# mariohsouto/ProxSDP.jl

Measured on AMD Instinct MI355X. Metric: PDHG iterations/sec at target rank ~ sqrt(n), Max-Cut SDP n=4000 (tol 1e-4 options), higher is better.
Workload: dtype f64

## Files before the change

### include/proxsdp_hip.h

```cpp
#ifndef PROXSDP_HIP_H
#define PROXSDP_HIP_H

#include <stdint.h>

#ifdef __cplusplus
extern "C" {
#endif

#define PROXSDP_HIP_ABI_VERSION 10

#define PROXSDP_E_INVALID  (-1)
#define PROXSDP_E_HIP      (-2)
#define PROXSDP_E_NOMEM    (-3)
#define PROXSDP_E_UNSUPP   (-4)
#define PROXSDP_E_INTERNAL (-5)
#define PROXSDP_E_COMM_ABORTED (-6)

#define PROXSDP_STATUS_NOT_CALLED       0
#define PROXSDP_STATUS_OPTIMAL          1
#define PROXSDP_STATUS_TIME_LIMIT       2
#define PROXSDP_STATUS_ITERATION_LIMIT  3
#define PROXSDP_STATUS_INFEAS_OR_UNBND  4
#define PROXSDP_STATUS_DUAL_INFEASIBLE  5
#define PROXSDP_STATUS_INFEASIBLE       6

typedef struct proxsdp_csc {
    int64_t nrows;
    int64_t ncols;
    const int64_t* colptr;
    const int64_t* rowval;
    const double*  nzval;
} proxsdp_csc;

typedef struct proxsdp_problem {
    int64_t n;
    int64_t p;
    int64_t m;
    proxsdp_csc A;
    proxsdp_csc G;
    const double* b;
    const double* h;
    const double* c;
    int64_t n_psd;
    const int64_t* psd_ptr;
    const int64_t* psd_idx;
    int64_t n_soc;
    const int64_t* soc_ptr;
    const int64_t* soc_idx;
    int32_t index_base;
    int32_t reserved0;
    const double* eig_resid;
    void* reduce_ctx;
    int (*reduce_fn)(void* ctx, double* sums, int32_t nsum, double* maxs, int32_t nmax);
    const double* M_dense;
    int32_t M_dense_on_device;
    int32_t reserved1;
    int64_t n_coupling;
    const int64_t* coupling_rows;
    const int32_t* coupling_owned;
    int (*reduce_vec_fn)(void* ctx, double* buf, int64_t len, int32_t on_device);
    int32_t reduce_vec_on_device;
    int32_t reserved2;
    void* nccl_comm;
    int64_t reserved3;
} proxsdp_problem;

typedef struct proxsdp_options {
    int64_t struct_size;
    int32_t log_verbose;  int32_t log_freq;
    int32_t timer_verbose; int32_t timer_file; int32_t disable_julia_logger;
    int32_t warn_on_limit; int32_t extended_log; int32_t extended_log2; int32_t log_repeat_header;
    int32_t pad0;
    double  time_limit;
    double tol_gap, tol_feasibility, tol_feasibility_dual, tol_primal, tol_dual, tol_psd, tol_soc;
    int32_t check_dual_feas; int32_t check_dual_feas_freq;
    double  max_obj; int32_t min_iter_max_obj; int32_t pad1;
    int32_t min_iter_time_infeas; int32_t pad2;
    double infeas_gap_tol, infeas_limit_gap_tol, infeas_stable_gap_tol,
           infeas_feasibility_tol, infeas_stable_feasibility_tol;
    int32_t certificate_search; int32_t pad3;
    double certificate_obj_tol, certificate_fail_tol;
    double min_beta, max_beta, initial_beta;
    double initial_adapt_level, adapt_decay; int32_t adapt_window; int32_t pad4;
    int32_t convergence_window; int32_t convergence_check;
    int64_t max_iter; int64_t min_iter; int64_t divergence_min_update;
    int64_t max_iter_lp; int64_t max_iter_conic; int64_t max_iter_local;
    int32_t advanced_initialization; int32_t line_search_flag;
    int32_t max_linsearch_steps; int32_t pad5;
    double delta, initial_theta, linsearch_decay;
    int32_t full_eig_decomp; int32_t max_target_rank_krylov_eigs;
    int32_t min_size_krylov_eigs; int32_t warm_start_eig;
    int32_t rank_increment; int32_t rank_increment_factor;
    int32_t eigsolver; int32_t eigsolver_min_lanczos; int64_t eigsolver_resid_seed;
    double  arpack_tol; int32_t arpack_resid_init; int32_t arpack_reset_resid; int64_t arpack_max_iter;
    int32_t krylovkit_reset_resid; int32_t krylovkit_resid_init;
    double  krylovkit_tol; int32_t krylovkit_max_iter; int32_t krylovkit_eager; int32_t krylovkit_verbose;
    int32_t reduce_rank; int32_t rank_slack; int32_t pad6;
    int64_t full_eig_freq; int64_t full_eig_len;
    int32_t equilibration; int32_t equilibration_iters;
    double  equilibration_lb, equilibration_ub, equilibration_limit;
    int32_t equilibration_force; int32_t approx_norm;
    int32_t device_id;
    int32_t trace_capacity;
    int32_t profile_symv_every;
    int32_t support_path;
    int32_t lanczos_operator;
    int32_t initial_target_rank;
    int32_t full_eig_lanczos;
    int32_t lanczos_cycle_kernel;
    int32_t lanczos_warm_start;
    int32_t reconstruct_mfma;
    int32_t small_block_batch;
    int32_t full_eig_sign;
    int32_t psd_sign_engine;
    int32_t full_eig_lanczos_verify;
    double  full_eig_lanczos_posres;
    int32_t full_eig_lanczos_kdim10;
    int32_t sign_small_tile_max;
    int32_t host_eig_threads;
    int32_t block_threads;
    int32_t host_eig_merge;
    int32_t block_batch;
    int32_t rocsolver_warmup;
    int32_t debug_fail_iteration;
    int32_t host_wait_spin;
    int32_t sign_start_row;
    int32_t general_batch;
    int32_t full_eig_lanczos_certify;
    int32_t host_merge_threads;
    int32_t reserved_i[1];
    double  full_eig_lanczos_tol;
    double  reserved_d[1];
    int32_t equilibration_reference_aliasing;
    int32_t reserved_i3[2];
    int32_t block_batch_groups;
    int32_t lanczos_wide_krylov;
    int32_t reserved_i2[7];
    double  full_eig_lanczos_warm_pow;
    double  reserved_d2[3];
} proxsdp_options;

#define PROXSDP_TRACE_COLS 14

typedef struct proxsdp_stats {
    int64_t lanczos_matvecs;
    int64_t lanczos_restarts;
    int64_t lanczos_calls;
    int64_t full_eigs;
    int64_t krylov_fallbacks;
    int64_t linesearch_trials;
    int64_t symv_launches;
    int64_t symv_profiled;
    double  symv_profiled_ms;
    double  symv_bytes;
    double  algorithmic_bytes;
    double  init_time;
    double  loop_time;
    double  exit_time;
    double  t_primal, t_psd, t_linesearch, t_residual;
    int64_t dense_passes;
    double  dense_ms;
    int64_t fop_projections;
    int64_t exit_matvecs;
    double  host_eig_time;
    int64_t host_eigs;
    int64_t device_eigs;
    int64_t batched_small_eigs;
    int64_t mfma_reconstructions;
    int64_t orth_profiled;
    double  orth_profiled_ms;
    double  full_eig_solver_ms;
    double  full_eig_recon_ms;
    int64_t cycle_launches;
    int64_t full_eigs_lanczos;
    int64_t cycle_steps;
    double  cycle_ms;
    int64_t warm_starts;
    int64_t full_eigs_sign;
    int64_t sign_products;
    int64_t sign_engine_projections;
    int64_t sign_engine_rejected;
    int64_t sign_engine_checks;
    int64_t sign_engine_mismatches;
    int64_t full_eigs_lanczos_checks;
    int64_t full_eigs_lanczos_mismatches;
    int64_t batched_block_steps;
    int64_t rccl_reductions;
    int64_t batched_profiled_blocks;
    int64_t host_eig_merges;
    double  host_eig_overlap_time;
    int64_t sign_short_pass;
    int64_t sign_short_fail;
    int64_t full_eigs_lanczos_certified;
    int64_t full_eigs_lanczos_cert_failed;
    int64_t cert_matvecs;
    int64_t dense_truncated_projections;
    int64_t wide_krylov_projections;
    int64_t reserved_s[4];
    int64_t dense_setup_passes;
    int64_t dense_sigma_steps;
} proxsdp_stats;
#define PROXSDP_STATS_SHARDED_GENERAL_ITERATIONS 0

typedef struct proxsdp_result {
    int32_t status;
    int32_t certificate_found;
    int32_t primal_feasible_user_tol;
    int32_t dual_feasible_user_tol;
    int32_t result_count;
    int32_t final_rank;
    int64_t iter;
    double  primal_residual;
    double  dual_residual;
    double  objval, dual_objval, gap, time;
    double  dual_feasibility;
    double* primal;
    double* dual_cone;
    double* dual_eq;
    double* dual_in;
    double* slack_eq;
    double* slack_in;
    double* trace;
    int64_t trace_rows;
    char    status_string[256];
    proxsdp_stats stats;
} proxsdp_result;

#define PROXSDP_STATE_NHIST 7
typedef struct proxsdp_state {
    int64_t struct_size;
    int64_t iteration;
    int64_t n, Q, n_psd;
    int64_t hist_len;
    double* x;
    double* y;
    double* Mty;
    double* Mx;
    int64_t* target_rank;
    int64_t* current_rank;
    double* min_eig;
    double* hist;
    double scal[16];
    int64_t ints[8];
} proxsdp_state;

int  proxsdp_hip_abi_version(void);
void proxsdp_hip_default_options(proxsdp_options* opt);
int  proxsdp_hip_set_option(proxsdp_options* opt, const char* name, double value);
int  proxsdp_hip_get_option(const proxsdp_options* opt, const char* name, double* value);
int  proxsdp_hip_solve(const proxsdp_problem* prob, const proxsdp_options* opt,
                       proxsdp_result* res);
int  proxsdp_hip_solve_ex(const proxsdp_problem* prob, const proxsdp_options* opt, proxsdp_result* res,
                          const proxsdp_state* resume, proxsdp_state* capture);
const char* proxsdp_hip_last_error(void);
int  proxsdp_hip_device_count(void);

int  proxsdp_hip_solve_sharded(const proxsdp_problem* prob, const proxsdp_options* opt,
                               int32_t n_shards, const int32_t* device_ids,
                               const int32_t* psd_owner, const int32_t* soc_owner, const int32_t* free_owner,
                               proxsdp_result* res, proxsdp_stats* shard_stats);

#define PROXSDP_FACTOR_NONE 0
#define PROXSDP_FACTOR_RITZ 1
#define PROXSDP_FACTOR_EIG  2
typedef struct proxsdp_psd_factors {
    int64_t struct_size;
    int64_t n_psd;
    const int64_t* cap;
    const int64_t* vec_ptr;
    const int64_t* val_ptr;
    double*  vectors;
    double*  values;
    int64_t* rank;
    int64_t* rank_found;
    int32_t* source;
    double*  resid;
    double*  xnorm;
} proxsdp_psd_factors;
int  proxsdp_hip_solve_factored(const proxsdp_problem* prob, const proxsdp_options* opt, proxsdp_result* res,
                                proxsdp_psd_factors* fac);

typedef struct proxsdp_start {
    int64_t struct_size;
// ... 150 lines not shown
```

### proxsdp.jl_amd/binding.py

```python
import ctypes as C
import os
import pathlib
import re

import numpy as np
import scipy.sparse as sp

_HERE = pathlib.Path(__file__).resolve().parent
LIB_PATH = _HERE / "libproxsdp_hip.so"
HEADER_PATH = _HERE.parent / "include" / "proxsdp_hip.h"

TRACE_COLS = 14
TRACE_NAMES = ("iter", "prim_obj", "dual_obj", "gap", "feas", "prim_res", "dual_res",
               "primal_step", "beta", "theta", "target_rank", "trials", "elapsed", "matvecs")


class LibraryNotBuilt(RuntimeError):
    pass


class ProxSDPHipError(RuntimeError):
    def __init__(self, code, msg):
        super().__init__(f"libproxsdp_hip error {code}: {msg}")
        self.code = code


i32, i64, f64 = C.c_int32, C.c_int64, C.c_double
pi64 = C.POINTER(C.c_int64)
pf64 = C.POINTER(C.c_double)


class CSC(C.Structure):
    _fields_ = [("nrows", i64), ("ncols", i64), ("colptr", pi64), ("rowval", pi64), ("nzval", pf64)]


class Problem(C.Structure):
    _fields_ = [("n", i64), ("p", i64), ("m", i64), ("A", CSC), ("G", CSC),
                ("b", pf64), ("h", pf64), ("c", pf64),
                ("n_psd", i64), ("psd_ptr", pi64), ("psd_idx", pi64),
                ("n_soc", i64), ("soc_ptr", pi64), ("soc_idx", pi64),
                ("index_base", i32), ("reserved0", i32), ("eig_resid", pf64),
                ("reduce_ctx", C.c_void_p), ("reduce_fn", C.c_void_p),
                ("M_dense", C.c_void_p), ("M_dense_on_device", i32), ("reserved1", i32),
                ("n_coupling", i64), ("coupling_rows", pi64), ("coupling_owned", C.POINTER(i32)),
                ("reduce_vec_fn", C.c_void_p), ("reduce_vec_on_device", i32), ("reserved2", i32),
                ("nccl_comm", C.c_void_p), ("reserved3", i64)]


REDUCE_FN = C.CFUNCTYPE(C.c_int, C.c_void_p, pf64, i32, pf64, i32)
REDUCE_VEC_FN = C.CFUNCTYPE(C.c_int, C.c_void_p, C.c_void_p, i64, i32)


def _opt_fields():
    F = []
    a = lambda name, t: F.append((name, t))
    a("struct_size", i64)
    for nme in ("log_verbose", "log_freq", "timer_verbose", "timer_file", "disable_julia_logger",
                "warn_on_limit", "extended_log", "extended_log2", "log_repeat_header", "pad0"):
        a(nme, i32)
    a("time_limit", f64)
    for nme in ("tol_gap", "tol_feasibility", "tol_feasibility_dual", "tol_primal", "tol_dual",
                "tol_psd", "tol_soc"):
        a(nme, f64)
    a("check_dual_feas", i32); a("check_dual_feas_freq", i32)
    a("max_obj", f64); a("min_iter_max_obj", i32); a("pad1", i32)
    a("min_iter_time_infeas", i32); a("pad2", i32)
    for nme in ("infeas_gap_tol", "infeas_limit_gap_tol", "infeas_stable_gap_tol",
                "infeas_feasibility_tol", "infeas_stable_feasibility_tol"):
        a(nme, f64)
    a("certificate_search", i32); a("pad3", i32)
    a("certificate_obj_tol", f64); a("certificate_fail_tol", f64)
    a("min_beta", f64); a("max_beta", f64); a("initial_beta", f64)
    a("initial_adapt_level", f64); a("adapt_decay", f64); a("adapt_window", i32); a("pad4", i32)
    a("convergence_window", i32); a("convergence_check", i32)
    for nme in ("max_iter", "min_iter", "divergence_min_update", "max_iter_lp", "max_iter_conic",
                "max_iter_local"):
        a(nme, i64)
    a("advanced_initialization", i32); a("line_search_flag", i32)
    a("max_linsearch_steps", i32); a("pad5", i32)
    a("delta", f64); a("initial_theta", f64); a("linsearch_decay", f64)
    a("full_eig_decomp", i32); a("max_target_rank_krylov_eigs", i32)
    a("min_size_krylov_eigs", i32); a("warm_start_eig", i32)
    a("rank_increment", i32); a("rank_increment_factor", i32)
    a("eigsolver", i32); a("eigsolver_min_lanczos", i32); a("eigsolver_resid_seed", i64)
    a("arpack_tol", f64); a("arpack_resid_init", i32); a("arpack_reset_resid", i32); a("arpack_max_iter", i64)
    a("krylovkit_reset_resid", i32); a("krylovkit_resid_init", i32)
    a("krylovkit_tol", f64); a("krylovkit_max_iter", i32); a("krylovkit_eager", i32); a("krylovkit_verbose", i32)
    a("reduce_rank", i32); a("rank_slack", i32); a("pad6", i32)
    a("full_eig_freq", i64); a("full_eig_len", i64)
    a("equilibration", i32); a("equilibration_iters", i32)
    a("equilibration_lb", f64); a("equilibration_ub", f64); a("equilibration_limit", f64)
    a("equilibration_force", i32); a("approx_norm", i32)
    a("device_id", i32); a("trace_capacity", i32); a("profile_symv_every", i32); a("support_path", i32)
    a("lanczos_operator", i32); a("initial_target_rank", i32)
    a("full_eig_lanczos", i32); a("lanczos_cycle_kernel", i32); a("lanczos_warm_start", i32)
    a("reconstruct_mfma", i32); a("small_block_batch", i32); a("full_eig_sign", i32); a("psd_sign_engine", i32)
    a("full_eig_lanczos_verify", i32); a("full_eig_lanczos_posres", f64); a("full_eig_lanczos_kdim10", i32)
    a("sign_small_tile_max", i32); a("host_eig_threads", i32); a("block_threads", i32)
    a("host_eig_merge", i32); a("block_batch", i32); a("rocsolver_warmup", i32); a("debug_fail_iteration", i32); a("host_wait_spin", i32)
    a("sign_start_row", i32); a("general_batch", i32); a("full_eig_lanczos_certify", i32); a("host_merge_threads", i32); a("reserved_i", i32 * 1)
    a("full_eig_lanczos_tol", f64); a("reserved_d", f64 * 1)
    a("equilibration_reference_aliasing", i32); a("reserved_i3", i32 * 2)
    a("block_batch_groups", i32); a("lanczos_wide_krylov", i32); a("reserved_i2", i32 * 7); a("full_eig_lanczos_warm_pow", f64); a("reserved_d2", f64 * 3)
    return F


class Options(C.Structure):
    _fields_ = _opt_fields()


class Stats(C.Structure):
    _fields_ = [("lanczos_matvecs", i64), ("lanczos_restarts", i64), ("lanczos_calls", i64),
                ("full_eigs", i64), ("krylov_fallbacks", i64), ("linesearch_trials", i64),
                ("symv_launches", i64), ("symv_profiled", i64), ("symv_profiled_ms", f64),
                ("symv_bytes", f64), ("algorithmic_bytes", f64), ("init_time", f64),
                ("loop_time", f64), ("exit_time", f64), ("t_primal", f64), ("t_psd", f64),
                ("t_linesearch", f64), ("t_residual", f64), ("dense_passes", i64), ("dense_ms", f64), ("fop_projections", i64), ("exit_matvecs", i64),
                ("host_eig_time", f64), ("host_eigs", i64), ("device_eigs", i64), ("batched_small_eigs", i64),
                ("mfma_reconstructions", i64), ("orth_profiled", i64), ("orth_profiled_ms", f64),
                ("full_eig_solver_ms", f64), ("full_eig_recon_ms", f64), ("cycle_launches", i64),
                ("full_eigs_lanczos", i64), ("cycle_steps", i64), ("cycle_ms", f64), ("warm_starts", i64),
                ("full_eigs_sign", i64), ("sign_products", i64),
                ("sign_engine_projections", i64), ("sign_engine_rejected", i64),
                ("sign_engine_checks", i64), ("sign_engine_mismatches", i64),
                ("full_eigs_lanczos_checks", i64), ("full_eigs_lanczos_mismatches", i64),
                ("batched_block_steps", i64), ("rccl_reductions", i64),
                ("batched_profiled_blocks", i64), ("host_eig_merges", i64),
                ("host_eig_overlap_time", f64), ("sign_short_pass", i64), ("sign_short_fail", i64),
                ("full_eigs_lanczos_certified", i64), ("full_eigs_lanczos_cert_failed", i64), ("cert_matvecs", i64),
                ("dense_truncated_projections", i64), ("wide_krylov_projections", i64), ("reserved_s", i64 * 4),
                ("dense_setup_passes", i64), ("dense_sigma_steps", i64)]


class Result(C.Structure):
    _fields_ = [("status", i32), ("certificate_found", i32), ("primal_feasible_user_tol", i32),
                ("dual_feasible_user_tol", i32), ("result_count", i32), ("final_rank", i32),
                ("iter", i64), ("primal_residual", f64), ("dual_residual", f64),
                ("objval", f64), ("dual_objval", f64), ("gap", f64), ("time", f64),
                ("dual_feasibility", f64),
                ("primal", pf64), ("dual_cone", pf64), ("dual_eq", pf64), ("dual_in", pf64),
                ("slack_eq", pf64), ("slack_in", pf64), ("trace", pf64), ("trace_rows", i64),
                ("status_string", C.c_char * 256), ("stats", Stats)]


STATS_RESERVED_SLOTS = {"sharded_general_iterations": 0}

STATE_NHIST = 7
STATE_HIST_NAMES = ("dual_gap", "prim_obj", "dual_obj", "feasibility", "primal_residual", "dual_residual", "comb_residual")
STATE_SCAL_NAMES = ("primal_step", "primal_step_old", "dual_step", "beta", "theta", "adapt_level",
                    "equa_feasibility", "ineq_feasibility", "dual_feasibility")


class State(C.Structure):
    _fields_ = [("struct_size", i64), ("iteration", i64), ("n", i64), ("Q", i64), ("n_psd", i64), ("hist_len", i64),
                ("x", pf64), ("y", pf64), ("Mty", pf64), ("Mx", pf64),
                ("target_rank", pi64), ("current_rank", pi64), ("min_eig", pf64), ("hist", pf64),
                ("scal", f64 * 16), ("ints", i64 * 8)]


class ShardIO(C.Structure):
    _fields_ = ([("struct_size", i64)] +
                [(k, i64) for k in ("n", "p", "m", "nnz_A", "nnz_G", "n_coupling", "n_psd", "len_psd", "n_soc", "len_soc", "len_eig")] +
                [("vars", pi64), ("rows_eq", pi64), ("rows_in", pi64), ("coupling_rows", pi64), ("coupling_owned", C.POINTER(i32)),
                 ("A_colptr", pi64), ("A_rowval", pi64), ("A_nzval", pf64), ("G_colptr", pi64), ("G_rowval", pi64), ("G_nzval", pf64),
                 ("b", pf64), ("h", pf64), ("c", pf64),
                 ("psd_ids", pi64), ("psd_ptr", pi64), ("psd_idx", pi64), ("soc_ids", pi64), ("soc_ptr", pi64), ("soc_idx", pi64), ("eig_resid", pf64)])


class PsdFactors(C.Structure):
    _fields_ = [("struct_size", i64), ("n_psd", i64), ("cap", pi64), ("vec_ptr", pi64), ("val_ptr", pi64),
                ("vectors", pf64), ("values", pf64), ("rank", pi64), ("rank_found", pi64), ("source", C.POINTER(i32)),
                ("resid", pf64), ("xnorm", pf64)]


class Start(C.Structure):
    _fields_ = [("struct_size", i64), ("primal", pf64), ("dual_eq", pf64), ("dual_in", pf64), ("n_psd", i64),
                ("rank", pi64), ("vec_ptr", pi64), ("val_ptr", pi64), ("vectors", pf64), ("values", pf64),
                ("target_rank", pi64), ("primal_step", f64), ("beta", f64)]


FACTOR_NONE, FACTOR_RITZ, FACTOR_EIG = 0, 1, 2
FACTOR_SOURCE_NAMES = {FACTOR_NONE: "NONE", FACTOR_RITZ: "RITZ", FACTOR_EIG: "EIG"}


_lib = None


def header_symbols():
    txt = HEADER_PATH.read_text()
    txt = re.sub(r"/\*.*?\*/", "", txt, flags=re.S)
    return sorted(set(re.findall(r"\b(proxsdp_(?:hip|host)_\w+)\s*\(", txt)))


def lib():
    global _lib
    if _lib is not None:
        return _lib
    if not LIB_PATH.exists():
        raise LibraryNotBuilt(
            f"{LIB_PATH} is missing: run `python -c 'import __graft_entry__ as g; g.build()'` "
            "(or `make -C proxsdp.jl_amd/csrc`).  There is no CPU fallback.")
    import sys
    if "torch" in sys.modules:
        try:
            tc = sys.modules["torch"].cuda
            if tc.is_available():
                tc.init()
        except Exception:
            pass
    L = C.CDLL(str(LIB_PATH))
    L.proxsdp_hip_abi_version.restype = C.c_int
    L.proxsdp_hip_last_error.restype = C.c_char_p
    L.proxsdp_hip_default_options.argtypes = [C.POINTER(Options)]
    L.proxsdp_hip_default_options.restype = None
    L.proxsdp_hip_set_option.argtypes = [C.POINTER(Options), C.c_char_p, f64]
    L.proxsdp_hip_get_option.argtypes = [C.POINTER(Options), C.c_char_p, pf64]
    L.proxsdp_hip_solve.argtypes = [C.POINTER(Problem), C.POINTER(Options), C.POINTER(Result)]
    L.proxsdp_hip_solve_ex.argtypes = [C.POINTER(Problem), C.POINTER(Options), C.POINTER(Result),
                                       C.POINTER(State), C.POINTER(State)]
    L.proxsdp_hip_solve_factored.argtypes = [C.POINTER(Problem), C.POINTER(Options), C.POINTER(Result),
                                             C.POINTER(PsdFactors)]
    L.proxsdp_hip_solve_from.argtypes = [C.POINTER(Problem), C.POINTER(Options), C.POINTER(Result),
                                         C.POINTER(Start), C.POINTER(PsdFactors)]
    L.proxsdp_hip_start_point.argtypes = [C.POINTER(Problem), C.POINTER(Options), C.POINTER(Start), C.POINTER(State)]
    L.proxsdp_hip_factor_residual.argtypes = [pf64, i64, pf64, i64, pf64, i32, pf64, pf64]
    L.proxsdp_hip_factor_residual_kernel.argtypes = [pf64, i64, pf64, i64, pf64, i32, pf64, pf64, i32, pf64]
    L.proxsdp_hip_psd_project.argtypes = [pf64, i64, i32, i32, C.POINTER(Options), pf64, pf64,
                                          C.POINTER(i32), pf64, pi64, C.POINTER(i32), C.POINTER(i32)]
    L.proxsdp_hip_eigsolve.argtypes = [pf64, i64, i32, C.POINTER(Options), pf64, i32, pf64, pf64,
                                       C.POINTER(i32), C.POINTER(i32), pi64, C.POINTER(i32)]
    L.proxsdp_hip_symv_packed.argtypes = [pf64, i64, pf64, pf64, i32, pf64]
    L.proxsdp_hip_reconstruct.argtypes = [pf64, pf64, i64, i32, pf64, i32, pf64]
    L.proxsdp_hip_reconstruct_kernel.argtypes = [pf64, pf64, i64, i32, i32, pf64, i32, pf64]
    L.proxsdp_hip_full_eig_kernel.argtypes = [pf64, i64, i32, pf64, i32, pf64, C.POINTER(i32), C.POINTER(i64)]
    L.proxsdp_hip_spmv.argtypes = [C.POINTER(CSC), i32, i32, pf64, pf64]
    L.proxsdp_host_symeig.argtypes = [i32, pf64, pf64]
    L.proxsdp_host_start_vector.argtypes = [i64, i64, i32, pf64]
    L.proxsdp_host_preprocess.argtypes = [C.POINTER(Problem), pi64, pi64, pf64, pf64]
    L.proxsdp_hip_dense_scaling.argtypes = [C.POINTER(Problem), C.POINTER(Options), pf64, pf64, pf64, pf64, C.POINTER(i32)]
    L.proxsdp_host_equilibrate_rowsums.argtypes = [pf64, i64, i64, C.POINTER(Options), pf64, pf64]
    L.proxsdp_hip_sym_product.argtypes = [C.POINTER(SymProductIO)]
    L.proxsdp_hip_sign_unpack.argtypes = [pf64, i64, f64, pf64, pf64]
    L.proxsdp_hip_solve_sharded.argtypes = [C.POINTER(Problem), C.POINTER(Options), i32, C.POINTER(i32), C.POINTER(i32),
                                            C.POINTER(i32), C.POINTER(i32), C.POINTER(Result), C.POINTER(Stats)]
    L.proxsdp_host_split_shard.argtypes = [C.POINTER(Problem), i32, C.POINTER(i32), C.POINTER(i32), C.POINTER(i32), i32,
                                           C.POINTER(ShardIO)]
    L.proxsdp_host_group_reduce.argtypes = [i32, i32, i32, i32, pf64, i32, i32, f64, pf64, C.POINTER(i32), C.POINTER(i32)]
    L.proxsdp_hip_coupling_sum.argtypes = [pf64, i32, i64, pi64, pf64, i64, pf64]
    L.proxsdp_hip_rccl_unique_id.argtypes = [C.c_void_p]
    L.proxsdp_hip_rccl_comm_init.argtypes = [i32, C.c_void_p, i32, i32, C.POINTER(C.c_void_p)]
    L.proxsdp_hip_rccl_comm_destroy.argtypes = [C.c_void_p]
    if L.proxsdp_hip_abi_version() != 10:
        raise ProxSDPHipError(-1, "ABI version mismatch")
# ... 854 lines not shown
```

### proxsdp.jl_amd/csrc/host_util.hpp

```cpp
#pragma once
#include <atomic>
#include <chrono>
#include <cmath>
#include <condition_variable>
#include <cstdint>
#include <cstdlib>
#include <cstring>
#include <cstddef>
#include <functional>
#include <mutex>
#include <thread>
#include <vector>
#include <algorithm>
#if defined(__x86_64__)
#include <immintrin.h>
#endif
#include "../../include/proxsdp_hip.h"
#include "host_eig_merge.hpp"

namespace proxsdp {

inline uint64_t splitmix64(uint64_t z) {
    z += 0x9E3779B97F4A7C15ull;
    z = (z ^ (z >> 30)) * 0xBF58476D1CE4E5B9ull;
// ... 376 lines not shown
        std::function<void(int)> f = fn;
        job_.store(&f, std::memory_order_relaxed);
        njobs_.store(n, std::memory_order_relaxed);
        done_.store(0, std::memory_order_relaxed);
        gen_ = (gen_ + 1) & 0xffffffffull;
        if (gen_ == 0) gen_ = 1;
        const uint64_t g = gen_;
        ticket_.store(g << 32, std::memory_order_release);
        work(g);
        while (done_.load(std::memory_order_acquire) < n) {
#if defined(__x86_64__)
            _mm_pause();
#endif
        }
    }
private:
    void work(uint64_t g) {
        for (;;) {
            uint64_t t = ticket_.load(std::memory_order_acquire);
            if ((t >> 32) != g) return;
            const int i = (int)(t & 0xffffffffu);
            if (i >= njobs_.load(std::memory_order_relaxed)) return;
            if (!ticket_.compare_exchange_weak(t, t + 1, std::memory_order_acq_rel, std::memory_order_acquire)) continue;
            (*job_.load(std::memory_order_relaxed))(i);
            done_.fetch_add(1, std::memory_order_acq_rel);
        }
    }
    void loop() {
        uint64_t seen = 0;
        for (;;) {
            {
                std::unique_lock<std::mutex> lk(mu_);
                cv_.wait(lk, [&]() { return stop_.load() || armed_.load(std::memory_order_acquire); });
                if (stop_.load()) return;
            }
            while (armed_.load(std::memory_order_acquire) && !stop_.load(std::memory_order_relaxed)) {
                const uint64_t g = ticket_.load(std::memory_order_acquire) >> 32;
                if (g != seen) { seen = g; work(g); }
                else {
#if defined(__x86_64__)
                    _mm_pause();
#endif
                }
            }
        }
    }
    std::vector<std::thread> th_;
    std::mutex mu_;
    std::condition_variable cv_;
    std::atomic<bool> armed_{false}, stop_{false};
    uint64_t gen_ = 0;
    std::atomic<uint64_t> ticket_{0};
    std::atomic<int> done_{0}, njobs_{0};
    std::atomic<const std::function<void(int)>*> job_{nullptr};
};

struct SplitEig {
    Rank1Merge M;
    std::vector<double> Q1, d1, Q2, d2, e2;
    int k1 = 0, K = 0;
    double beta = 0.0;
    bool have_first = false;
    int first(int k1_, int m, const double* D, const double* f, const double* al, const double* be) {
        k1 = k1_; have_first = false;
        if (k1 < 1 || (m > 0 && k1 != m + 1)) return 1;
        beta = be[k1 - 1];
        if (!(beta == beta) || beta == 0.0) return 1;
        Q1.assign((size_t)k1 * k1, 0.0); d1.assign(k1, 0.0);
        int rc;
        if (m == 0) {
            for (int j = 0; j < k1; ++j) {
                Q1[(size_t)j * k1 + j] = al[j];
                if (j + 1 < k1) { Q1[(size_t)j * k1 + j + 1] = be[j]; Q1[(size_t)(j + 1) * k1 + j] = be[j]; }
            }
            Q1[(size_t)(k1 - 1) * k1 + (k1 - 1)] -= std::fabs(beta);
            rc = symeig_dense(k1, Q1.data(), d1.data(), true, 0);
        } else {
            for (int j = 0; j < m; ++j) {
                Q1[(size_t)j * k1 + j] = D[j];
                Q1[(size_t)j * k1 + m] = f[j]; Q1[(size_t)m * k1 + j] = f[j];
            }
            Q1[(size_t)m * k1 + m] = al[m] - std::fabs(beta);
            rc = symeig_dense(k1, Q1.data(), d1.data(), false, 0);
        }
        have_first = (rc == 0);
        return rc;
    }
    int second(int K_, const double* al, const double* be) {
        K = K_;
        const int k2 = K - k1;
        if (!have_first || k2 < 1) return 1;
        Q2.assign((size_t)k2 * k2, 0.0); d2.assign(k2, 0.0);
        for (int j = 0; j < k2; ++j) {
            Q2[(size_t)j * k2 + j] = al[k1 + j];
            if (j + 1 < k2) { Q2[(size_t)j * k2 + j + 1] = be[k1 + j]; Q2[(size_t)(j + 1) * k2 + j] = be[k1 + j]; }
        }
        Q2[0] -= std::fabs(beta);
        if (symeig_dense(k2, Q2.data(), d2.data(), true, 0) != 0) return 1;
        M.build(k1, k2, Q1.data(), d1.data(), Q2.data(), d2.data(), beta);
        return 0;
    }
};

enum OptType { OT_I32, OT_I64, OT_F64 };
struct OptEntry { const char* name; OptType type; size_t offset; };

#define PX_OPT(name, type) { #name, type, offsetof(proxsdp_options, name) }
inline const std::vector<OptEntry>& option_table() {
    static const std::vector<OptEntry> t = {
        PX_OPT(log_verbose, OT_I32), PX_OPT(log_freq, OT_I32), PX_OPT(timer_verbose, OT_I32),
        PX_OPT(timer_file, OT_I32), PX_OPT(disable_julia_logger, OT_I32), PX_OPT(warn_on_limit, OT_I32),
        PX_OPT(extended_log, OT_I32), PX_OPT(extended_log2, OT_I32), PX_OPT(log_repeat_header, OT_I32),
        PX_OPT(time_limit, OT_F64),
        PX_OPT(tol_gap, OT_F64), PX_OPT(tol_feasibility, OT_F64), PX_OPT(tol_feasibility_dual, OT_F64),
        PX_OPT(tol_primal, OT_F64), PX_OPT(tol_dual, OT_F64), PX_OPT(tol_psd, OT_F64), PX_OPT(tol_soc, OT_F64),
        PX_OPT(check_dual_feas, OT_I32), PX_OPT(check_dual_feas_freq, OT_I32),
        PX_OPT(max_obj, OT_F64), PX_OPT(min_iter_max_obj, OT_I32),
        PX_OPT(min_iter_time_infeas, OT_I32), PX_OPT(infeas_gap_tol, OT_F64),
        PX_OPT(infeas_limit_gap_tol, OT_F64), PX_OPT(infeas_stable_gap_tol, OT_F64),
        PX_OPT(infeas_feasibility_tol, OT_F64), PX_OPT(infeas_stable_feasibility_tol, OT_F64),
        PX_OPT(certificate_search, OT_I32), PX_OPT(certificate_obj_tol, OT_F64), PX_OPT(certificate_fail_tol, OT_F64),
        PX_OPT(min_beta, OT_F64), PX_OPT(max_beta, OT_F64), PX_OPT(initial_beta, OT_F64),
        PX_OPT(initial_adapt_level, OT_F64), PX_OPT(adapt_decay, OT_F64), PX_OPT(adapt_window, OT_I32),
        PX_OPT(convergence_window, OT_I32), PX_OPT(convergence_check, OT_I32),
        PX_OPT(max_iter, OT_I64), PX_OPT(min_iter, OT_I64), PX_OPT(divergence_min_update, OT_I64),
        PX_OPT(max_iter_lp, OT_I64), PX_OPT(max_iter_conic, OT_I64), PX_OPT(max_iter_local, OT_I64),
        PX_OPT(advanced_initialization, OT_I32), PX_OPT(line_search_flag, OT_I32),
        PX_OPT(max_linsearch_steps, OT_I32), PX_OPT(delta, OT_F64), PX_OPT(initial_theta, OT_F64),
        PX_OPT(linsearch_decay, OT_F64),
        PX_OPT(full_eig_decomp, OT_I32), PX_OPT(max_target_rank_krylov_eigs, OT_I32),
        PX_OPT(min_size_krylov_eigs, OT_I32), PX_OPT(warm_start_eig, OT_I32),
        PX_OPT(rank_increment, OT_I32), PX_OPT(rank_increment_factor, OT_I32),
        PX_OPT(eigsolver, OT_I32), PX_OPT(eigsolver_min_lanczos, OT_I32), PX_OPT(eigsolver_resid_seed, OT_I64),
        PX_OPT(arpack_tol, OT_F64), PX_OPT(arpack_resid_init, OT_I32), PX_OPT(arpack_reset_resid, OT_I32),
        PX_OPT(arpack_max_iter, OT_I64),
        PX_OPT(krylovkit_reset_resid, OT_I32), PX_OPT(krylovkit_resid_init, OT_I32),
        PX_OPT(krylovkit_tol, OT_F64), PX_OPT(krylovkit_max_iter, OT_I32), PX_OPT(krylovkit_eager, OT_I32),
        PX_OPT(krylovkit_verbose, OT_I32),
        PX_OPT(reduce_rank, OT_I32), PX_OPT(rank_slack, OT_I32),
        PX_OPT(full_eig_freq, OT_I64), PX_OPT(full_eig_len, OT_I64),
        PX_OPT(equilibration, OT_I32), PX_OPT(equilibration_iters, OT_I32),
        PX_OPT(equilibration_lb, OT_F64), PX_OPT(equilibration_ub, OT_F64), PX_OPT(equilibration_limit, OT_F64),
        PX_OPT(equilibration_force, OT_I32), PX_OPT(approx_norm, OT_I32),
        PX_OPT(device_id, OT_I32), PX_OPT(trace_capacity, OT_I32), PX_OPT(profile_symv_every, OT_I32),
        PX_OPT(support_path, OT_I32), PX_OPT(lanczos_operator, OT_I32), PX_OPT(initial_target_rank, OT_I32),
        PX_OPT(full_eig_lanczos, OT_I32), PX_OPT(lanczos_cycle_kernel, OT_I32), PX_OPT(lanczos_warm_start, OT_I32),
        PX_OPT(reconstruct_mfma, OT_I32), PX_OPT(small_block_batch, OT_I32), PX_OPT(full_eig_sign, OT_I32), PX_OPT(psd_sign_engine, OT_I32),
        PX_OPT(full_eig_lanczos_verify, OT_I32), PX_OPT(full_eig_lanczos_posres, OT_F64), PX_OPT(full_eig_lanczos_kdim10, OT_I32),
        PX_OPT(sign_small_tile_max, OT_I32), PX_OPT(host_eig_threads, OT_I32), PX_OPT(block_threads, OT_I32),
        PX_OPT(host_eig_merge, OT_I32), PX_OPT(block_batch, OT_I32),
        PX_OPT(rocsolver_warmup, OT_I32), PX_OPT(debug_fail_iteration, OT_I32), PX_OPT(host_wait_spin, OT_I32), PX_OPT(sign_start_row, OT_I32), PX_OPT(general_batch, OT_I32),
        PX_OPT(full_eig_lanczos_certify, OT_I32), PX_OPT(full_eig_lanczos_tol, OT_F64), PX_OPT(host_merge_threads, OT_I32),
        PX_OPT(equilibration_reference_aliasing, OT_I32), PX_OPT(block_batch_groups, OT_I32), PX_OPT(full_eig_lanczos_warm_pow, OT_F64),
        PX_OPT(lanczos_wide_krylov, OT_I32),
    };
    return t;
}
#undef PX_OPT

inline void default_options(proxsdp_options* o) {
    std::memset(o, 0, sizeof(*o));
    o->struct_size = (int64_t)sizeof(*o);
    o->log_verbose = 0; o->log_freq = 1000; o->disable_julia_logger = 1;
    o->time_limit = 360000.0;
    o->tol_gap = 1e-4; o->tol_feasibility = 1e-4; o->tol_feasibility_dual = 1e-4;
    o->tol_primal = 1e-4; o->tol_dual = 1e-4; o->tol_psd = 1e-7; o->tol_soc = 1e-7;
    o->check_dual_feas = 0; o->check_dual_feas_freq = 1000;
    o->max_obj = 1e20; o->min_iter_max_obj = 10;
    o->min_iter_time_infeas = 1000; o->infeas_gap_tol = 1e-4; o->infeas_limit_gap_tol = 1e-1;
    o->infeas_stable_gap_tol = 1e-4; o->infeas_feasibility_tol = 1e-4;
    o->infeas_stable_feasibility_tol = 1e-8;
    o->certificate_search = 1; o->certificate_obj_tol = 1e-1; o->certificate_fail_tol = 1e-8;
    o->min_beta = 1e-5; o->max_beta = 1e5; o->initial_beta = 1.0;
    o->initial_adapt_level = 0.9; o->adapt_decay = 0.8; o->adapt_window = 50;
    o->convergence_window = 200; o->convergence_check = 50;
    o->max_iter = 0; o->min_iter = 40; o->divergence_min_update = 50;
    o->max_iter_lp = 10000000; o->max_iter_conic = 1000000; o->max_iter_local = 0;
    o->advanced_initialization = 1; o->line_search_flag = 1; o->max_linsearch_steps = 5000;
    o->delta = 0.9999; o->initial_theta = 1.0; o->linsearch_decay = 0.75;
    o->full_eig_decomp = 0; o->max_target_rank_krylov_eigs = 16; o->min_size_krylov_eigs = 100;
    o->warm_start_eig = 1; o->rank_increment = 1; o->rank_increment_factor = 1;
    o->eigsolver = 2; o->eigsolver_min_lanczos = 25; o->eigsolver_resid_seed = 1234;
    o->arpack_tol = 1e-10; o->arpack_resid_init = 3; o->arpack_reset_resid = 1; o->arpack_max_iter = 10000;
    o->krylovkit_reset_resid = 0; o->krylovkit_resid_init = 3; o->krylovkit_tol = 1e-12;
    o->krylovkit_max_iter = 100; o->krylovkit_eager = 0; o->krylovkit_verbose = 0;
    o->reduce_rank = 0; o->rank_slack = 3; o->full_eig_freq = 10000000; o->full_eig_len = 0;
    o->equilibration = 0; o->equilibration_iters = 1000; o->equilibration_lb = -10.0;
    o->equilibration_ub = 10.0; o->equilibration_limit = 0.9; o->equilibration_force = 0;
    o->approx_norm = 1;
    o->device_id = 0; o->trace_capacity = 0; o->profile_symv_every = 0; o->support_path = -1;
    o->lanczos_operator = -1; o->initial_target_rank = 2;
    o->full_eig_lanczos = -1; o->lanczos_cycle_kernel = -1; o->lanczos_warm_start = 0; o->reconstruct_mfma = -1;
    o->small_block_batch = -1; o->full_eig_sign = -1; o->psd_sign_engine = -1;
    o->full_eig_lanczos_verify = -1; o->full_eig_lanczos_posres = 1e-6; o->full_eig_lanczos_kdim10 = 30;
    o->sign_small_tile_max = 3072; o->host_eig_threads = 0; o->block_threads = -1;
    o->host_eig_merge = -1; o->block_batch = -1; o->rocsolver_warmup = 0; o->host_wait_spin = -1; o->sign_start_row = -1; o->general_batch = -1;
    o->full_eig_lanczos_certify = -1; o->full_eig_lanczos_tol = 0.0; o->host_merge_threads = -1;
    o->equilibration_reference_aliasing = 1; o->block_batch_groups = -1; o->full_eig_lanczos_warm_pow = 1.0;
    o->lanczos_wide_krylov = 0;
}

inline int set_option(proxsdp_options* o, const char* name, double v) {
    for (const auto& e : option_table()) {
        if (std::strcmp(e.name, name) == 0) {
            char* base = reinterpret_cast<char*>(o) + e.offset;
            if (e.type == OT_I32) *reinterpret_cast<int32_t*>(base) = (int32_t)std::llround(v);
            else if (e.type == OT_I64) *reinterpret_cast<int64_t*>(base) = (int64_t)std::llround(v);
            else *reinterpret_cast<double*>(base) = v;
            return 0;
        }
    }
    return PROXSDP_E_INVALID;
}
inline int get_option(const proxsdp_options* o, const char* name, double* v) {
    for (const auto& e : option_table()) {
        if (std::strcmp(e.name, name) == 0) {
            const char* base = reinterpret_cast<const char*>(o) + e.offset;
            if (e.type == OT_I32) *v = (double)*reinterpret_cast<const int32_t*>(base);
            else if (e.type == OT_I64) *v = (double)*reinterpret_cast<const int64_t*>(base);
            else *v = *reinterpret_cast<const double*>(base);
            return 0;
        }
    }
    return PROXSDP_E_INVALID;
}

}
```

### proxsdp.jl_amd/csrc/kernels.hip.hpp

```cpp
#pragma once
#include <hip/hip_runtime.h>
#include <cstdint>

namespace proxsdp {
namespace dev {

constexpr int WAVE = 64;
constexpr int TILE = 64;
constexpr int TPB = 256;
constexpr int NWAVE = TPB / WAVE;
constexpr int CPW = TILE / NWAVE;
constexpr double INV_SQRT2 = 0.70710678118654752440;
constexpr double SQRT2 = 1.41421356237309504880;

#ifdef PX_TIMELINE
constexpr int TL_WG = 160, TL_SLOTS = 8, TL_K = 260;
__device__ unsigned long long g_tl[2][TL_K][TL_WG][TL_SLOTS];
#define PX_TL(kind, k, slot)                                                                                   \
    do {                                                                                                       \
        if (threadIdx.x == 0 && (int)blockIdx.x < ::proxsdp::dev::TL_WG && (k) >= 0 && (k) < ::proxsdp::dev::TL_K) { \
            asm volatile("" ::: "memory");                                                                     \
            ::proxsdp::dev::g_tl[kind][k][blockIdx.x][slot] = wall_clock64();                                    \
            asm volatile("" ::: "memory");                                                                     \
        }                                                                                                      \
// ... 498 lines not shown
        if (lane < 16 && jc <= k) hpart_out[(long long)blockIdx.x * KLD + jc] = hs;
    }
    PX_TL(1, k, 6);
}
template <int NCH, int NCHP>
__global__ void __launch_bounds__(TPB)
k_lz_orth(const double* __restrict__ Ppart, int nt, int npad, const double* __restrict__ V, int ldv, int k,
          double* __restrict__ wbuf, const double* __restrict__ hred, double* __restrict__ hpart_out, int pld,
          double* __restrict__ hsum_out, const LanczosCtl* __restrict__ ctl,
          const double* __restrict__ alphas, const double* __restrict__ betas,
          const double* __restrict__ Apart, int napart, int first, const double* __restrict__ arrow, int keep,
          FopArgs fo) {
    lz_orth_body<NCH, NCHP>(Ppart, nt, npad, V, ldv, k, wbuf, hred, hpart_out, pld, hsum_out, ctl, alphas, betas, Apart,
                            napart, first, arrow, keep, fo);
}

template <int NCH>
__device__ __forceinline__ void lz_finish_body(const double* __restrict__ wbuf, double* __restrict__ V, int ldv, int k,
                                               const double* __restrict__ hpart_in, int pld,
                                               const double* __restrict__ h1, double* __restrict__ alphas,
                                               double* __restrict__ betas, LanczosCtl* __restrict__ ctl,
                                               double tol, int use_carry, int g,
                                               double* __restrict__ s_h, double* __restrict__ s_d,
                                               double* __restrict__ s_beta, double* __restrict__ hred,
                                               int nprod ) {
    constexpr int NC = 16 * NCH;
    __shared__ double s_p[NWAVE * 4 * 64 * NCH];
    const int lane = threadIdx.x & 63;
    const int wv = __builtin_amdgcn_readfirstlane((int)(threadIdx.x >> 6));
    const int kk = k + 1;
    const int i = g * LZ_ROWS + lane;
    PX_TL(0, k + 1, 0);
    const int stop = ctl->stop;
    double hp[16][NCH];
#pragma unroll
    for (int u = 0; u < 16; ++u) {
        const long long rec = (long long)min(wv + NWAVE * u, pld - 1) * KLD;
#pragma unroll
        for (int ch = 0; ch < NCH; ++ch)
            hp[u][ch] = ((ch == 0 || 64 * ch < kk) && (wv + NWAVE * u < nprod || pld > WAVE))
                            ? hpart_in[rec + 64 * ch + lane] : 0.0;
    }
    double vr[NC];
#pragma unroll
    for (int c0 = 0; c0 < NC; c0 += 4) {
        if (wv + 4 * c0 <= k) {
#pragma unroll
            for (int c = c0; c < c0 + 4; ++c) vr[c] = V[(long long)min(wv + 4 * c, k) * ldv + i];
        } else {
#pragma unroll
            for (int c = c0; c < c0 + 4; ++c) vr[c] = 0.0;
        }
    }
    double hn = hpart_in[(long long)pld * KLD + min(lane, pld - 1)];
    const double w0 = wbuf[i];
    const double h1k = h1[k];
    const double carry = use_carry ? ctl->carry : 0.0;
    if (stop) return;
    PX_TL(0, k + 1, 1);
    PX_TL_DRAIN();
    PX_TL(0, k + 1, 2);
#pragma unroll
    for (int ch = 0; ch < NCH; ++ch) {
        double pr[16], q4[4];
#pragma unroll
        for (int u = 0; u < 16; ++u) {
            pr[u] = hp[u][ch];
            if (64 * ch < kk)
                for (int q = wv + NWAVE * u + WAVE; q < pld; q += WAVE) pr[u] += hpart_in[(long long)q * KLD + 64 * ch + lane];
        }
        tree_in_wave(pr, q4);
#pragma unroll
        for (int a = 0; a < 4; ++a) s_p[(wv * 4 + a) * (64 * NCH) + 64 * ch + lane] = q4[a];
    }
    if (wv == 0) {
        if (lane >= pld) hn = 0.0;
        else for (int q = lane + WAVE; q < pld; q += WAVE) hn += hpart_in[(long long)pld * KLD + q];
        hn = wave_sum(hn);
        if (lane == 0) s_h[4 * NC] = hn;
    }
    __syncthreads();
    if ((int)threadIdx.x < 64 * NCH) {
        const int j = threadIdx.x;
        const double hj = tree_across(s_p, 64 * NCH, j);
        s_h[j] = (j < kk) ? hj : 0.0;
    }
    __syncthreads();
    PX_TL(0, k + 1, 3);
    double hh = 0.0;
    for (int j = lane; j < kk; j += WAVE) hh += s_h[j] * s_h[j];
    hh = wave_sum(hh);
    const double beta = sqrt(fmax(s_h[4 * NC] - hh, 0.0));
    double hq[NC];
#pragma unroll
    for (int c = 0; c < NC; ++c) hq[c] = s_h[wv + 4 * c];
    double d0 = 0.0, d1 = 0.0;
#pragma unroll
    for (int c = 0; c < NC; c += 2) {
        d0 += vr[c] * hq[c];
        d1 += vr[c + 1] * hq[c + 1];
    }
    s_d[wv * LZ_ROWS + lane] = d0 + d1;
    if (g == 0 && (int)threadIdx.x < kk) hred[threadIdx.x] = s_h[threadIdx.x];
    if (g == 0 && threadIdx.x == 0) {
        alphas[k] = h1k + s_h[k] - carry;
        betas[k] = beta;
        ctl->carry = s_h[k];
        if (beta <= tol) { ctl->kstop = k + 1; ctl->stop = 1; }
    }
    if (beta <= tol) return;
    __syncthreads();
    PX_TL(0, k + 1, 4);
    if (wv == 0) {
        const double wi = w0 - ((s_d[lane] + s_d[LZ_ROWS + lane]) + (s_d[2 * LZ_ROWS + lane] + s_d[3 * LZ_ROWS + lane]));
        V[(long long)(k + 1) * ldv + i] = wi / beta;
    }
    PX_TL(0, k + 1, 5);
    (void)s_beta;
}

template <int NCH>
__global__ void __launch_bounds__(TPB)
k_lz_measure(const double* __restrict__ wbuf, const double* __restrict__ V, int ldv, int k,
             double* __restrict__ hpart_out, int pld, LanczosCtl* __restrict__ ctl) {
    constexpr int NC = 16 * NCH;
    const int lane = threadIdx.x & 63;
    const int wv = __builtin_amdgcn_readfirstlane((int)(threadIdx.x >> 6));
    const int i = blockIdx.x * LZ_ROWS + lane;
    const double wp = wbuf[i];
    double vr[NC];
#pragma unroll
    for (int c = 0; c < NC; ++c) vr[c] = (wv + 4 * c <= k) ? V[(long long)(wv + 4 * c) * ldv + i] : 0.0;
    if (blockIdx.x == 0 && threadIdx.x == 0) { ctl->stop = 0; ctl->kstop = 0; ctl->carry = 0.0; }
    if (wv == 0) {
        const double r = wave_sum(wp * wp);
        if (lane == 0) hpart_out[(long long)pld * KLD + blockIdx.x] = r;
    }
#pragma unroll
    for (int ch = 0; ch < NCH; ++ch) {
        double t[16];
#pragma unroll
        for (int c = 0; c < 16; ++c) t[c] = vr[16 * ch + c] * wp;
        const double hs = fold16_all(t, lane);
        const int jc = wv + 4 * (16 * ch + lane);
        if (lane < 16 && jc <= k) hpart_out[(long long)blockIdx.x * KLD + jc] = hs;
    }
}

template <int NCH>
__global__ void __launch_bounds__(TPB)
k_lz_finish(const double* __restrict__ wbuf, int n, double* __restrict__ V, int ldv, int k,
            const double* __restrict__ hpart_in, int pld, const double* __restrict__ h1,
            double* __restrict__ alphas, double* __restrict__ betas, LanczosCtl* __restrict__ ctl, double tol,
            int use_carry, double* __restrict__ hred) {
    __shared__ double s_h[64 * NCH + 1];
    __shared__ double s_d[NWAVE * LZ_ROWS];
    __shared__ double s_beta;
    lz_finish_body<NCH>(wbuf, V, ldv, k, hpart_in, pld, h1, alphas, betas, ctl, tol, use_carry, blockIdx.x, s_h, s_d, &s_beta, hred,
                        (int)gridDim.x);
}

template <int NCH>
__global__ void __launch_bounds__(TPB)
k_symv_finish(const double* __restrict__ xp, int n, int nt, int npad, double* __restrict__ Ppart,
              const double* __restrict__ wbuf, double* __restrict__ V, int ldv, int k,
              const double* __restrict__ hpart_in, int pld, const double* __restrict__ h1,
              double* __restrict__ alphas, double* __restrict__ betas, LanczosCtl* __restrict__ ctl, double tol,
              int use_carry, double* __restrict__ Apart, double* __restrict__ hred) {
    __shared__ double s_a[2 * NWAVE * TILE];
    __shared__ double s_b[NWAVE * LZ_ROWS];
    __shared__ double s_beta;
    if ((int)blockIdx.x < nt)
        lz_finish_body<NCH>(wbuf, V, ldv, k, hpart_in, pld, h1, alphas, betas, ctl, tol, use_carry, blockIdx.x,
                            s_a, s_b, &s_beta, hred, nt);
    else if (ctl->stop) return;
    else
        symv_tiles(xp, n, npad, nt * (nt + 1) / 2, wbuf, Ppart, (int)blockIdx.x - nt, (int)gridDim.x - nt, s_a, s_b, Apart);
}

constexpr int LZB_MAX = 8;
struct LzBlk {
    const double* xp;
    double* Ppart; double* wbuf; double* V;
    double* hpart1; double* hpart2; double* hsum; double* alphas; double* betas;
    LanczosCtl* ctl;
    double* Apart; double* hred;
    const double* arrow; const double* resid;
    int k;
    int keep;
    int mode;
    int pad;
};
struct LzBatch {
    LzBlk b[LZB_MAX];
    int n, nt, npad, pld, napart, nb;
    double tol;
};
__global__ void __launch_bounds__(TPB)
k_lzb_begin(LzBatch B) {
    const LzBlk& b = B.b[blockIdx.z];
    if (b.mode == 0) return;
    const int i = blockIdx.x * TPB + threadIdx.x;
    if (i < B.npad) b.V[i] = b.resid[i];
    if (i == 0) { b.ctl->stop = 0; b.ctl->kstop = 0; b.ctl->carry = 0.0; }
}
__global__ void __launch_bounds__(TPB)
k_lzb_mv(LzBatch B, double* __restrict__ rec_out, int rec_doubles) {
    __shared__ double s_a[2 * NWAVE * TILE];
    __shared__ double s_b[NWAVE * LZ_ROWS];
    __shared__ double s_beta;
    const LzBlk& b = B.b[blockIdx.z];
    const int mode = b.mode;
    if (mode == 0) return;
    const int nt = B.nt;
    if ((int)blockIdx.x < nt) {
        if (mode == 1) return;
        const int kc = b.k - 1;
        lz_finish_body<1>(b.wbuf, b.V, B.npad, kc, (kc & 1) ? b.hpart2 : b.hpart1, B.pld, b.hsum, b.alphas, b.betas, b.ctl,
                          B.tol, kc > b.keep ? 1 : 0, blockIdx.x, s_a, s_b, &s_beta, b.hred, nt);
        if (mode == 3 && blockIdx.x == 0 && rec_out != nullptr) {
            __syncthreads();
            const double* src = b.alphas;
            for (int t = threadIdx.x; t < rec_doubles; t += TPB) rec_out[(long long)blockIdx.z * rec_doubles + t] = src[t];
        }
    } else {
        if (mode == 3 || b.ctl->stop) return;
        const double* v = (mode == 1) ? b.V + (long long)b.k * B.npad : b.wbuf;
        symv_tiles(b.xp, B.n, B.npad, nt * (nt + 1) / 2, v, b.Ppart, (int)blockIdx.x - nt, (int)gridDim.x - nt, s_a, s_b,
                   b.Apart);
    }
}
__global__ void __launch_bounds__(TPB)
k_lzb_orth(LzBatch B) {
    const LzBlk& b = B.b[blockIdx.z];
    if (b.mode == 0) return;
    FopArgs fo{};
    lz_orth_body<1, 0>(b.Ppart, B.nt, B.npad, b.V, B.npad, b.k, b.wbuf, b.hred, (b.k & 1) ? b.hpart2 : b.hpart1, B.pld,
                       b.hsum, b.ctl, b.alphas, b.betas, b.Apart, B.napart, b.k == b.keep ? 1 : 0, b.arrow, b.keep, fo);
}

struct EllOverflow {
    const int* wr_ptr;
    const int* wr_row;
    const int* wr_lo;
    const int* wr_hi;
    const int* ov_col;
    const int* ov_sidx;
};
template <int NCHP>
__device__ __forceinline__ void fop_body(const double* __restrict__ v, const double* __restrict__ Vp, int ldv, int rp,
                                         const int* __restrict__ ell_col, const int* __restrict__ ell_sidx, int ell_w,
                                         int npad, const double* __restrict__ esv, double* __restrict__ tpart, int pld,
                                         double* __restrict__ ebuf, double* __restrict__ apart, int g,
                                         double* __restrict__ s_e , const LanczosCtl* __restrict__ ctl,
                                         const EllOverflow& ov, int tlk = -1 ) {
    constexpr int NCP = 16 * NCHP;
    const int lane = threadIdx.x & 63;
    const int wv = __builtin_amdgcn_readfirstlane((int)(threadIdx.x >> 6));
    const int i = g * LZ_ROWS + lane;
    PX_TL(0, tlk, 0);
    const int stop = (ctl != nullptr) ? ctl->stop : 0;
    const double vi = v[i];
    double vrp[NCP];
#pragma unroll
    for (int c = 0; c < NCP; ++c) vrp[c] = Vp[(long long)min(wv + 4 * c, max(rp - 1, 0)) * ldv + i];
    int col0[4], sx0[4];
#pragma unroll
    for (int u = 0; u < 4; ++u) {
        const int k = min(wv + u * NWAVE, ell_w - 1);
        col0[u] = ell_col[(long long)k * npad + i];
        sx0[u] = (wv + u * NWAVE < ell_w) ? ell_sidx[(long long)k * npad + i] : -1;
    }
    if (stop) return;
    PX_TL(0, tlk, 1);
    double e = 0.0;
    for (int k0 = wv; k0 < ell_w; k0 += 4 * NWAVE) {
        int col[4], sx[4];
#pragma unroll
        for (int u = 0; u < 4; ++u) {
            if (k0 == wv) { col[u] = col0[u]; sx[u] = sx0[u]; continue; }
            const int k = min(k0 + u * NWAVE, ell_w - 1);
            col[u] = ell_col[(long long)k * npad + i];
            sx[u] = (k0 + u * NWAVE < ell_w) ? ell_sidx[(long long)k * npad + i] : -1;
        }
        double ev[4], xv[4];
#pragma unroll
        for (int u = 0; u < 4; ++u) { ev[u] = esv[max(sx[u], 0)]; xv[u] = v[col[u]]; }
#pragma unroll
        for (int u = 0; u < 4; ++u)
            if (sx[u] >= 0) e += ((col[u] == i) ? ev[u] : ev[u] * INV_SQRT2) * xv[u];
    }
    s_e[wv * LZ_ROWS + lane] = e;
    PX_TL(0, tlk, 2);
    if (ov.wr_ptr != nullptr) {
        const int q0 = ov.wr_ptr[g], q1 = ov.wr_ptr[g + 1];
        if (q1 > q0) {
            __shared__ double s_w[NWAVE];
            __syncthreads();
            for (int q = q0; q < q1; ++q) {
                const int rloc = ov.wr_row[q], grow = g * LZ_ROWS + rloc;
                double a = 0.0;
                for (int k = ov.wr_lo[q] + (int)threadIdx.x; k < ov.wr_hi[q]; k += TPB) {
                    const int col = ov.ov_col[k];
                    const double evk = esv[ov.ov_sidx[k]];
                    a += ((col == grow) ? evk : evk * INV_SQRT2) * v[col];
                }
                a = wave_sum(a);
                if (lane == 0) s_w[wv] = a;
                __syncthreads();
                if (threadIdx.x == 0) s_e[rloc] += (s_w[0] + s_w[1]) + (s_w[2] + s_w[3]);
                __syncthreads();
            }
// ... 263 lines not shown
            const int gjc = min(J * TILE + w * 16 + l4 + 4 * reg, n - 1);
#pragma unroll
            for (int b = 0; b < 4; ++b) {
                const int gic = min(I * TILE + b * 16 + l15, gjc);
                const long long idxc = (long long)gjc * (gjc + 1) / 2 + gic;
                xo[reg * 4 + b] = xold[idxc];
                mk[reg * 4 + b] = mask[(mask_off + idxc) >> 5];
            }
        }
    }
    fetch(0);
    stash(0);
    __syncthreads();
    int cur = 0;
    for (int k0 = 0; k0 < r; k0 += MF_KC) {
        const bool more = k0 + MF_KC < r;
        if (more) fetch(k0 + MF_KC);
#pragma unroll
        for (int q = 0; q < MF_KC / 4; ++q) {
            const double a = sA[cur][4 * q + l4][w * 16 + l15];
            double bv[4];
#pragma unroll
            for (int b = 0; b < 4; ++b) bv[b] = sB[cur][4 * q + l4][b * 16 + l15];
#pragma unroll
            for (int b = 0; b < 4; ++b) acc[b] = __builtin_amdgcn_mfma_f64_16x16x4f64(a, bv[b], acc[b], 0, 0, 0);
        }
        if (more) {
            stash(cur ^ 1);
            __syncthreads();
            cur ^= 1;
        }
    }
    double m0 = 0.0, m1 = 0.0;
#pragma unroll
    for (int reg = 0; reg < 4; ++reg) {
        const int gj = J * TILE + w * 16 + l4 + 4 * reg;
#pragma unroll
        for (int b = 0; b < 4; ++b) {
            const int gi = I * TILE + b * 16 + l15;
            if (gj < n && gi <= gj) {
                const long long idx = (long long)gj * (gj + 1) / 2 + gi;
                const double xn = ((gi == gj) ? 1.0 : SQRT2) * acc[b][reg];
                if (FUSE_RES) {
                    const double xov = xo[reg * 4 + b];
                    const long long gidx = mask_off + idx;
                    const bool on = (mk[reg * 4 + b] >> (gidx & 31)) & 1u;
                    if (!on) { m0 = fmax(m0, fabs(xn - xov)); m1 = fmax(m1, fabs(xov)); }
                }
                xp[idx] = xn;
            }
        }
    }
    if (FUSE_RES) {
        const double r0 = block_max(m0, s_red);
        const double r1 = block_max(m1, s_red);
        if (threadIdx.x == 0) { respart[blockIdx.x] = r0; respart[rstride + blockIdx.x] = r1; }
    }
}

__global__ void __launch_bounds__(TPB)
k_factor_residual(const double* __restrict__ xp, int n, const double* __restrict__ V, int ldv,
                  const double* __restrict__ lam, int r, double* __restrict__ part) {
    __shared__ double sA[2][MF_KC][MF_LD];
    __shared__ double sB[2][MF_KC][MF_LD];
    __shared__ double s_red[NWAVE];
    const int nt_ = (n + TILE - 1) / TILE;
    const int tile = xcd_tile(blockIdx.x, nt_ * (nt_ + 1) / 2);
    if (tile >= nt_ * (nt_ + 1) / 2) return;
    int I, J;
    tile_coords(tile, I, J);
    const int lane = threadIdx.x & 63;
    const int w = __builtin_amdgcn_readfirstlane((int)(threadIdx.x >> 6));
    const int l15 = lane & 15, l4 = lane >> 4;
    const int gja = J * TILE + lane, gib = I * TILE + lane;
    const bool ja_ok = gja < n, ib_ok = gib < n;
    const double* __restrict__ zA = V + (ja_ok ? gja : 0);
    const double* __restrict__ zB = V + (ib_ok ? gib : 0);
    constexpr int MF_U = MF_KC / NWAVE;
    double pa[MF_U], pb[MF_U];
    auto fetch = [&](int k0) {
#pragma unroll
        for (int u = 0; u < MF_U; ++u) {
            const int k = k0 + w + 4 * u;
            const bool kok = k < r;
            const long long ko = (long long)(kok ? k : 0) * ldv;
            pa[u] = (kok && ja_ok) ? zA[ko] * lam[k] : 0.0;
            pb[u] = (kok && ib_ok) ? zB[ko] : 0.0;
        }
    };
    auto stash = [&](int buf) {
#pragma unroll
        for (int u = 0; u < MF_U; ++u) { sA[buf][w + 4 * u][lane] = pa[u]; sB[buf][w + 4 * u][lane] = pb[u]; }
    };
    v4f64 acc[4];
#pragma unroll
    for (int b = 0; b < 4; ++b) acc[b] = (v4f64){0.0, 0.0, 0.0, 0.0};
    double xv[16];
#pragma unroll
    for (int reg = 0; reg < 4; ++reg) {
        const int gjc = min(J * TILE + w * 16 + l4 + 4 * reg, n - 1);
#pragma unroll
        for (int b = 0; b < 4; ++b) {
            const int gic = min(I * TILE + b * 16 + l15, gjc);
            xv[reg * 4 + b] = xp[(long long)gjc * (gjc + 1) / 2 + gic];
        }
    }
    fetch(0);
    stash(0);
    __syncthreads();
    int cur = 0;
    for (int k0 = 0; k0 < r; k0 += MF_KC) {
        const bool more = k0 + MF_KC < r;
        if (more) fetch(k0 + MF_KC);
#pragma unroll
        for (int q = 0; q < MF_KC / 4; ++q) {
            const double a = sA[cur][4 * q + l4][w * 16 + l15];
            double bv[4];
#pragma unroll
            for (int b = 0; b < 4; ++b) bv[b] = sB[cur][4 * q + l4][b * 16 + l15];
#pragma unroll
            for (int b = 0; b < 4; ++b) acc[b] = __builtin_amdgcn_mfma_f64_16x16x4f64(a, bv[b], acc[b], 0, 0, 0);
        }
        if (more) {
            stash(cur ^ 1);
            __syncthreads();
            cur ^= 1;
        }
    }
    double s0 = 0.0, s1 = 0.0;
#pragma unroll
    for (int reg = 0; reg < 4; ++reg) {
        const int gj = J * TILE + w * 16 + l4 + 4 * reg;
#pragma unroll
        for (int b = 0; b < 4; ++b) {
            const int gi = I * TILE + b * 16 + l15;
            if (gj < n && gi <= gj) {
                const double wt = (gi == gj) ? 1.0 : 2.0;
                const double x = xv[reg * 4 + b];
                const double d = x - acc[b][reg];
                s0 += wt * (d * d);
                s1 += wt * (x * x);
            }
        }
    }
    const double r0 = block_sum(s0, s_red);
    const double r1 = block_sum(s1, s_red);
    if (threadIdx.x == 0) { part[2 * tile] = r0; part[2 * tile + 1] = r1; }
}

constexpr int RM_LDV = TILE + 16;
constexpr int RM_CG = 16;
__global__ void __launch_bounds__(TPB)
k_lz_rotate_mfma(const double* __restrict__ V, int ldv, int K, const double* __restrict__ U, int ncols,
                 double* __restrict__ out, int ldo, int copy_src, int copy_dst) {
    extern __shared__ double s_mem[];
    const int Kp = (K + 3) & ~3;
    const int ldu = Kp + 2;
    double* s_V = s_mem;
    double* s_U = s_mem + (size_t)Kp * RM_LDV;
    const int lane = threadIdx.x & 63;
    const int w = __builtin_amdgcn_readfirstlane((int)(threadIdx.x >> 6));
    const int l15 = lane & 15, l4 = lane >> 4;
    const int i0 = blockIdx.x * LZ_ROWS;
    const int c0 = blockIdx.y * RM_CG;
    const int cn = min(RM_CG, ncols - c0);
    if (cn > 0) {
        double tu[RM_CG / NWAVE][2];
        for (int jb = 0; jb < Kp; jb += 2 * WAVE) {
#pragma unroll
            for (int u = 0; u < RM_CG / NWAVE; ++u)
#pragma unroll
                for (int h = 0; h < 2; ++h) {
                    const int c = w + NWAVE * u, j = jb + WAVE * h + lane;
                    tu[u][h] = (c < cn && j < K) ? U[(long long)(c0 + c) * K + j] : 0.0;
                }
#pragma unroll
            for (int u = 0; u < RM_CG / NWAVE; ++u)
#pragma unroll
                for (int h = 0; h < 2; ++h) {
                    const int c = w + NWAVE * u, j = jb + WAVE * h + lane;
                    if (j < Kp) s_U[c * ldu + j] = tu[u][h];
                }
        }
        for (int j0 = w; j0 < Kp; j0 += 16 * NWAVE) {
            double tv[16];
#pragma unroll
            for (int u = 0; u < 16; ++u) {
                const int j = j0 + NWAVE * u;
                tv[u] = (j < K) ? V[(long long)j * ldv + i0 + lane] : 0.0;
            }
#pragma unroll
            for (int u = 0; u < 16; ++u) {
                const int j = j0 + NWAVE * u;
                if (j < Kp) s_V[j * RM_LDV + lane] = tv[u];
            }
        }
        __syncthreads();
        v4f64 acc = (v4f64){0.0, 0.0, 0.0, 0.0};
        for (int q = 0; q < Kp / 4; ++q) {
            const double bv = s_V[(4 * q + l4) * RM_LDV + w * 16 + l15];
            const double av = s_U[l15 * ldu + 4 * q + l4];
            acc = __builtin_amdgcn_mfma_f64_16x16x4f64(av, bv, acc, 0, 0, 0);
        }
#pragma unroll
        for (int reg = 0; reg < 4; ++reg) {
            const int c = l4 + 4 * reg;
            if (c < cn) out[(long long)(c0 + c) * ldo + i0 + w * 16 + l15] = acc[reg];
        }
    }
    if (copy_src >= 0 && blockIdx.y == 0 && w == 0) out[(long long)copy_dst * ldo + i0 + lane] = V[(long long)copy_src * ldv + i0 + lane];
}

__global__ void __launch_bounds__(TPB)
k_small_psd_project(double* __restrict__ x, const long long* __restrict__ offs, const int* __restrict__ sides,
                    double tol_psd, int* __restrict__ rank_out, int* __restrict__ npos_out, int nmin, int nmax) {
    extern __shared__ __attribute__((aligned(16))) double sj_mem[];
    __shared__ double s_red[NWAVE];
    __shared__ int s_cnt[2];
    const int n = sides[blockIdx.x];
    if (n < nmin || n > nmax) return;
    double* __restrict__ xp = x + offs[blockIdx.x];
    const int ld = n | 1;
    double* A = sj_mem;
    double* V = A + n * ld;
    double* cs = V + n * ld;
    int* pq = (int*)(cs + 64);
    const int tid = threadIdx.x;
    for (int t = tid; t < n * n; t += TPB) {
        const int i = t % n, j = t / n;
        const int lo = min(i, j), hi = max(i, j);
        const double v = xp[(long long)hi * (hi + 1) / 2 + lo];
        A[i * ld + j] = (i == j) ? v : v * INV_SQRT2;
        V[i * ld + j] = (i == j) ? 1.0 : 0.0;
    }
    __syncthreads();
    const int m = n + (n & 1);
    const int np = m / 2;
    for (int sweep = 0; sweep < 40; ++sweep) {
        double off = 0.0, dg = 0.0;
        for (int t = tid; t < n * n; t += TPB) {
            const int i = t % n, j = t / n;
            const double v = A[i * ld + j];
            if (i == j) dg += v * v; else off += v * v;
        }
        const double offs_ = block_sum(off, s_red);
        if (tid == 0) cs[0] = offs_;
        __syncthreads();
        const double dgs = block_sum(dg, s_red);
        if (tid == 0) cs[1] = dgs;
        __syncthreads();
        if (cs[0] <= 1e-32 * cs[1] || cs[0] == 0.0) break;
        __syncthreads();
        for (int rd = 0; rd < m - 1; ++rd) {
            if (tid < np) {
                int p, q;
                if (tid == 0) { p = m - 1; q = rd; }
                else { p = (rd + tid) % (m - 1); q = (rd - tid + (m - 1)) % (m - 1); }
                if (p > q) { const int t = p; p = q; q = t; }
                double c = 1.0, s = 0.0;
                if (q < n) {
                    const double apq = A[p * ld + q];
                    if (apq != 0.0) {
                        const double tau = (A[q * ld + q] - A[p * ld + p]) / (2.0 * apq);
                        const double t = (tau >= 0.0 ? 1.0 : -1.0) / (fabs(tau) + sqrt(1.0 + tau * tau));
                        c = 1.0 / sqrt(1.0 + t * t);
                        s = t * c;
                    }
                } else { q = -1; }
                pq[tid] = p; pq[32 + tid] = q; cs[tid] = c; cs[32 + tid] = s;
            }
            __syncthreads();
            for (int t = tid; t < np * n; t += TPB) {
                const int i = t / n, k = t - i * n;
                const int p = pq[i], q = pq[32 + i];
                if (q >= 0) {
                    const double c = cs[i], s = cs[32 + i];
                    const double ap = A[p * ld + k], aq = A[q * ld + k];
                    A[p * ld + k] = c * ap - s * aq;
                    A[q * ld + k] = s * ap + c * aq;
                }
            }
            __syncthreads();
            for (int t = tid; t < np * n; t += TPB) {
                const int i = t / n, k = t - i * n;
                const int p = pq[i], q = pq[32 + i];
                if (q >= 0) {
                    const double c = cs[i], s = cs[32 + i];
                    const double ap = A[k * ld + p], aq = A[k * ld + q];
                    A[k * ld + p] = c * ap - s * aq;
                    A[k * ld + q] = s * ap + c * aq;
                    const double vp = V[k * ld + p], vq = V[k * ld + q];
                    V[k * ld + p] = c * vp - s * vq;
                    V[k * ld + q] = s * vp + c * vq;
                }
            }
            __syncthreads();
        }
    }
    if (tid == 0) { s_cnt[0] = 0; s_cnt[1] = 0; }
    __syncthreads();
    if (tid < n) {
        const double lamk = A[tid * ld + tid];
        cs[tid] = lamk > 0.0 ? lamk : 0.0;
        if (lamk > tol_psd) atomicAdd(&s_cnt[0], 1);
        if (lamk > 0.0) atomicAdd(&s_cnt[1], 1);
    }
    __syncthreads();
    const int N = n * (n + 1) / 2;
    for (int t = tid; t < N; t += TPB) {
        int j = (int)((sqrt(8.0 * (double)t + 1.0) - 1.0) * 0.5);
// ... 775 lines not shown
```

### proxsdp.jl_amd/csrc/pdhg_loop.hip.hpp

```cpp
#pragma once
#include "solver.hip.hpp"

namespace proxsdp {

constexpr int PSTRIDE = 2048;
constexpr int NQ = 16;

inline void Solver::spmv(const double* x, double* y) {
    spmv_sparse(x, y);
    if (P.dense()) dense_mv(x, y, true);
}
inline void Solver::spmv_sparse(const double* x, double* y) {
    if (P.Q == 0) return;
    if (csr_wave)
        hipLaunchKernelGGL(dev::k_spmv_csr_wave, dim3(ceil_div(P.Q, dev::NWAVE)), dim3(dev::TPB), 0, stream,
                           csr_ptr.p, csr_col.p, csr_val.p, x, y, (int)P.Q, LONG_ROW);
    else
        hipLaunchKernelGGL(dev::k_spmv_csr_thread, dim3(ceil_div(P.Q, dev::TPB)), dim3(dev::TPB), 0, stream,
                           csr_ptr.p, csr_col.p, csr_val.p, x, y, (int)P.Q, LONG_ROW);
    if (n_seg > 0) {
        hipLaunchKernelGGL(dev::k_spmv_csr_seg, dim3(n_seg), dim3(dev::TPB), 0, stream,
                           seg_lo_d.p, seg_hi_d.p, csr_col.p, csr_val.p, x, segpart_d.p);
        hipLaunchKernelGGL(dev::k_spmv_seg_fin, dim3(ceil_div(n_long, dev::TPB)), dim3(dev::TPB), 0, stream,
                           long_row_d.p, long_ptr_d.p, n_long, segpart_d.p, y);
    }
}
inline void Solver::setup_long_rows(const std::vector<int>& rp) {
    std::vector<int> lo, hi, rows, ptr{0};
    for (int64_t r = 0; r < P.Q; ++r) {
        if (rp[r + 1] - rp[r] <= LONG_ROW) continue;
        rows.push_back((int)r);
        for (int k = rp[r]; k < rp[r + 1]; k += dev::SPMV_SEG) { lo.push_back(k); hi.push_back(std::min(k + dev::SPMV_SEG, rp[r + 1])); }
        ptr.push_back((int)lo.size());
    }
    n_seg = (int)lo.size(); n_long = (int)rows.size();
    if (n_seg == 0) return;
    seg_lo_d.alloc(n_seg); seg_hi_d.alloc(n_seg); long_row_d.alloc(n_long); long_ptr_d.alloc(n_long + 1); segpart_d.alloc(n_seg);
    seg_lo_d.upload(lo.data(), n_seg, stream); seg_hi_d.upload(hi.data(), n_seg, stream);
    long_row_d.upload(rows.data(), n_long, stream); long_ptr_d.upload(ptr.data(), n_long + 1, stream);
    PX_HIP(hipStreamSynchronize(stream));
}

inline bool Solver::krylov_branch(int idx) const {
    return !opt.full_eig_decomp && target_rank[idx] <= opt.max_target_rank_krylov_eigs &&
           eig[idx].n > opt.min_size_krylov_eigs && (iter % opt.full_eig_freq) > opt.full_eig_len;
}
inline bool Solver::batch_eligible(int idx, bool fuse) const {
    const EigWork& W = eig[idx];
    if (opt.block_batch == 0 || !krylov_branch(idx)) return false;
    if (opt.eigsolver == 1 || opt.psd_sign_engine == 1 || opt.lanczos_warm_start > 0 || opt.krylovkit_eager)
        return false;
    if (fuse && use_support && opt.lanczos_operator != 0 && W.fop_ok && (W.have_factors || W.x_prev_sparse)) return false;
    return std::max(2 * (int)target_rank[idx] + 1, (int)opt.eigsolver_min_lanczos) <= 63;
}
inline void Solver::project_blocks(const std::vector<int>& blocks, const double* xin, double* xout, bool fuse) {
    std::vector<int> rest;
    std::vector<std::vector<int>> groups;
    if (opt.block_batch != 0 && blocks.size() >= 2) {
        std::vector<int> cand;
        for (int idx : blocks) (batch_eligible(idx, fuse) ? cand : rest).push_back(idx);
        std::stable_sort(cand.begin(), cand.end(), [this](int a, int b) { return eig[a].n < eig[b].n; });
        size_t i0 = 0;
        while (i0 < cand.size()) {
            size_t i1 = i0;
            while (i1 < cand.size() && eig[cand[i1]].n == eig[cand[i0]].n) ++i1;
            const size_t cnt = i1 - i0;
            if (cnt < 2) { rest.push_back(cand[i0]); i0 = i1; continue; }
            size_t ng = (cnt + dev::LZB_MAX - 1) / dev::LZB_MAX;
            const int want = opt.block_batch_groups < 0 ? 1 : (int)opt.block_batch_groups;
            if (parallel_blocks() && want >= 2 && cnt >= 4) ng = std::max<size_t>(ng, std::min<size_t>((size_t)want, cnt / 2));
            for (size_t q = 0; q < ng; ++q) {
                const size_t a = i0 + q * cnt / ng, b = i0 + (q + 1) * cnt / ng;
                groups.emplace_back(cand.begin() + a, cand.begin() + b);
            }
            i0 = i1;
        }
        std::sort(rest.begin(), rest.end());
    } else {
        rest = blocks;
    }
    if (batch_ctx.size() < groups.size()) {
        const size_t have = batch_ctx.size();
        batch_ctx.resize(groups.size());
        for (size_t q = have; q < groups.size(); ++q) batch_ctx[q].reset(new BatchCtx());
    }
    for (const std::vector<int>& g : groups) for (int idx : g) current_rank[idx] = 0;
    const int want_groups = opt.block_batch_groups < 0 ? 1 : (int)opt.block_batch_groups;
    bool leaders_have_streams = parallel_blocks() && groups.size() >= 2 && want_groups >= 2;
    for (const std::vector<int>& g : groups) leaders_have_streams = leaders_have_streams && eig[g[0]].stream != nullptr;
    if (leaders_have_streams) {
        std::vector<int> leaders;
        std::vector<int> slot_of(eig.size(), -1);
        for (size_t q = 0; q < groups.size(); ++q) { leaders.push_back(groups[q][0]); slot_of[groups[q][0]] = (int)q; }
        run_blocks(leaders, [this, xin, &groups, &slot_of](int leader) {
            const std::vector<int>& g = groups[slot_of[leader]];
            std::vector<int> nevs;
            for (int idx : g) nevs.push_back((int)target_rank[idx]);
            lanczos_batch(g, xin, nevs, slot_of[leader]);
        });
    } else {
        for (size_t q = 0; q < groups.size(); ++q) {
            std::vector<int> nevs;
            for (int idx : groups[q]) nevs.push_back((int)target_rank[idx]);
            lanczos_batch(groups[q], xin, nevs, (int)q);
        }
    }
    for (const std::vector<int>& g : groups)
        for (int idx : g) project_block(idx, xin, xout, fuse, true);
    if (!groups.empty()) merge_block_stats();
    if (!rest.empty()) run_blocks(rest, [this, xin, xout, fuse](int idx) { project_block(idx, xin, xout, fuse); });
}

inline void Solver::project_block(int idx, const double* xin, double* xout, bool fuse, bool lanczos_done) {
    EigWork& W = eig[idx];
    const double* xp = xin + P.blocks[idx].off;
    double* xo = xout + P.blocks[idx].off;
    current_rank[idx] = 0;
    W.ritz_ok = false;
    const bool krylov = lanczos_done || krylov_branch(idx);
    W.use_fop = !lanczos_done && fuse && use_support && opt.lanczos_operator != 0 && W.fop_ok && krylov &&
                (W.have_factors || W.x_prev_sparse) && !(opt.krylovkit_eager && opt.eigsolver != 1);
    if (std::max(2 * (int)target_rank[idx] + 1, (int)opt.eigsolver_min_lanczos) > dev::LZ_KMAX) W.use_fop = false;
    if (W.use_fop) {
        if (!W.have_factors) { W.F_r = 0; W.F_first = 0; }
        W.esv = esv_d.p + (W.have_factors ? 0 : ns);
    }
    if (!krylov) {
        const bool implicit = !opt.full_eig_decomp && (iter % opt.full_eig_freq) > opt.full_eig_len &&
                              W.n > opt.min_size_krylov_eigs;
        if (!implicit && opt.full_eig_lanczos != 1) {
            W.have_factors = false; W.x_prev_sparse = false; W.use_fop = false;
            full_eig_project(idx, xp, xo, fuse);
            return;
        }
        W.use_fop = fuse && use_support && opt.lanczos_operator != 0 && W.fop_ok && (W.have_factors || W.x_prev_sparse);
        if (W.use_fop) {
            if (!W.have_factors) { W.F_r = 0; W.F_first = 0; }
            W.esv = esv_d.p + (W.have_factors ? 0 : ns);
        }
        if (full_eig_by_lanczos(idx, xp, xo, fuse)) return;
        W.have_factors = false; W.x_prev_sparse = false; W.use_fop = false;
        full_eig_project(idx, xp, xo, fuse);
        return;
    }
    const bool used_fop = W.use_fop;
    const int nev = (int)target_rank[idx];
    if (!lanczos_done && !krylovdim_fits(nev)) {
        W.use_fop = false;
        truncated_project_dense(idx, xp, xo, fuse, nev);
        return;
    }
    if (!lanczos_done) {
        if (exact_projection_by_sign(idx, xp, xo, fuse, nev)) return;
        const double t_kry = opt.psd_sign_engine == 1 ? now_s() : 0.0;
        lanczos(W, xp, nev);
        if (opt.psd_sign_engine == 1 && W.converged) {
            const double ms = (now_s() - t_kry) * 1e3;
            W.kry_ms = W.kry_ms < 0 ? ms : 0.75 * W.kry_ms + 0.25 * ms;
        }
    }
    W.use_fop = false;
    if (used_fop) W.lst.fop_projections++;
    if (!W.converged) {
        W.lst.krylov_fallbacks++;
        W.have_factors = false; W.x_prev_sparse = false;
        full_eig_project(idx, xp, xo, fuse);
        return;
    }
    double mn = W.vals[0];
    for (double v : W.vals) mn = std::min(mn, v);
    min_eig[idx] = mn;
    int first = 0, npos = 0;
    if (opt.eigsolver == 1) {
        for (int i = 0; i < nev; ++i) if (W.vals[i] > 0.0) ++npos;
        first = nev - npos;
    } else {
        const int k = std::min(nev, W.converged_eigs);
        for (int i = 0; i < k; ++i) if (W.vals[i] > 0.0) ++npos;
    }
    current_rank[idx] += npos;
    W.last_npos = npos;
    if (npos > 0) W.lam.upload(W.vals.data() + first, npos, stream);
    launch_reconstruct(W, W.Z.p + (size_t)first * W.npad, W.npad, W.lam.p, npos, xo,
                       fuse ? xp : nullptr, fuse ? idx : -1);
    W.recon_r += npos;
    if (W.fop_ok) {
        std::swap(W.Z.p, W.F.p);
        W.F_first = first; W.F_r = npos;
        std::swap(W.lam.p, W.Flam.p);
        std::swap(W.lam.n, W.Flam.n);
        W.have_factors = true; W.x_prev_sparse = false;
    } else {
        W.ritz_first = first; W.ritz_r = npos; W.ritz_ok = true;
    }
    if (W.sign_check_pending) verify_sign_engine(idx, xo);
}

inline double sign_cost_model_ms(int ld) {
    static const int L[] = {128, 512, 1024, 1536, 2048, 3072, 4096};
    static const double T[] = {0.30, 0.60, 2.05, 4.8, 11.3, 31.2, 71.2};
    if (ld <= L[0]) return T[0];
    for (int i = 1; i < 7; ++i)
        if (ld <= L[i]) return T[i - 1] + (T[i] - T[i - 1]) * (double)(ld - L[i - 1]) / (L[i] - L[i - 1]);
    return T[6] * std::pow((double)ld / 4096.0, 3.0);
}
inline bool Solver::exact_projection_by_sign(int idx, const double* xp, double* xo, bool fuse, int nev) {
    if (opt.psd_sign_engine != 1) return false;
    EigWork& W = eig[idx];
    W.sign_check_pending = false;
    if (W.n < 33 || W.n > 16384) return false;
    if (W.kry_ms < 0.0 || W.last_npos < 0) return false;
    if (W.last_npos >= nev) return false;
    if (W.sign_backoff > 0) { --W.sign_backoff; return false; }
    const double est = W.sign_ms >= 0.0 ? W.sign_ms : sign_cost_model_ms(W.nt * dev::TILE);
    if (W.kry_ms < 1.5 * est) { W.sign_streak = 0; return false; }
    if (W.sign_streak >= 256) { W.sign_streak = 0; return false; }
    if (W.sign_disabled) return false;
    const bool inplace = xp == xo;
    if (W.sign_verified_left <= 0) {
        if (W.sg_out.n < (size_t)W.N) W.sg_out.alloc(W.N);
        const long long cr = current_rank[idx];
        const double me = min_eig[idx];
        const int lnp = W.last_npos;
        if (full_eig_by_sign(idx, xp, W.sg_out.p, false, true)) W.sign_check_pending = current_rank[idx] < nev;
        current_rank[idx] = cr; min_eig[idx] = me; W.last_npos = lnp;
        return false;
    }
    double* out = xo;
    if (inplace) {
        if (W.sg_out.n < (size_t)W.N) W.sg_out.alloc(W.N);
        out = W.sg_out.p;
    }
    const double t0 = now_s();
    if (!full_eig_by_sign(idx, xp, out, fuse, true)) return false;
    const double ms = (now_s() - t0) * 1e3;
    W.sign_ms = W.sign_ms < 0 ? ms : 0.75 * W.sign_ms + 0.25 * ms;
    const int npos = (int)current_rank[idx];
    if (npos >= nev) {
        W.lst.sign_engine_rejected++;
        current_rank[idx] = 0;
        W.sign_backoff = 32;
        return false;
    }
    if (inplace) PX_HIP(hipMemcpyAsync(xo, out, (size_t)W.N * sizeof(double), hipMemcpyDeviceToDevice, stream));
    W.lst.sign_engine_projections++;
    W.sign_streak++;
    W.sign_verified_left--;
    min_eig[idx] = 0.0;
    W.have_factors = false; W.x_prev_sparse = false; W.use_fop = false;
    return true;
}

inline void Solver::verify_sign_engine(int idx, const double* xo) {
    EigWork& W = eig[idx];
    W.sign_check_pending = false;
    if (W.sg_cmp.n < 2) W.sg_cmp.alloc(2);
    W.sg_cmp.zero(stream);
    hipLaunchKernelGGL(dev::k_maxdiff, dim3(grid_for(W.N)), dim3(dev::TPB), 0, stream, xo, (const double*)W.sg_out.p,
                       (long long)W.N, W.sg_cmp.p);
    double h[2] = {0.0, 0.0};
    W.sg_cmp.download(h, 2, stream);
    PX_HIP(hipStreamSynchronize(stream));
    W.lst.sign_engine_checks++;
    if (h[0] <= 1e-8 * std::max(h[1], 1e-300)) {
        W.sign_verified_left = 64;
    } else {
        W.sign_disabled = true;
        W.lst.sign_engine_mismatches++;
    }
}

inline bool Solver::full_eig_by_lanczos(int idx, const double* xp, double* xo, bool fuse) {
    EigWork& W = eig[idx];
    if (opt.full_eig_lanczos == 0 || opt.eigsolver == 1 || W.n <= opt.min_size_krylov_eigs) return false;
    if (W.last_npos < 0) return false;
    if (W.fel_disabled) return false;
    const int maxnev = std::min((std::min(W.cap, dev::MAXK - 4) - 2) / 2, W.n - 1);
    int g = W.last_npos + std::max(3, W.last_npos / 8);
    if (8 * W.last_npos > W.n) return false;
    const bool used_fop = W.use_fop;
    const int vk = opt.full_eig_lanczos_verify < 0 ? 256 : opt.full_eig_lanczos_verify;
    bool verify = vk > 0 && (W.fel_served % vk) == 0;
    long long ref_rank = 0;
    int ref_npos = 0;
    bool ref_sign = false;
    if (verify) {
        if (W.sg_out.n < (size_t)W.N) W.sg_out.alloc(W.N);
        const long long cr = current_rank[idx];
        const double me = min_eig[idx];
        const int lnp = W.last_npos;
        const bool hf = W.have_factors, xs = W.x_prev_sparse, uf = W.use_fop;
        const long long fe0 = W.lst.full_eigs, fs0 = W.lst.full_eigs_sign;
        full_eig_project(idx, xp, W.sg_out.p, false);
        ref_rank = current_rank[idx]; ref_npos = W.last_npos; ref_sign = W.lst.full_eigs_sign > fs0;
        current_rank[idx] = cr; min_eig[idx] = me; W.last_npos = lnp;
        W.have_factors = hf; W.x_prev_sparse = xs; W.use_fop = uf;
        W.lst.full_eigs = fe0; W.lst.full_eigs_sign = fs0;
    }
    auto use_reference_result = [&]() {
        W.fel_disabled = true;
        W.lst.full_eigs_lanczos_mismatches++;
        W.have_factors = false; W.x_prev_sparse = false; W.use_fop = false; W.ritz_ok = false;
        if (xp != xo) { full_eig_project(idx, xp, xo, fuse); return; }
        PX_HIP(hipMemcpyAsync(xo, W.sg_out.p, (size_t)W.N * sizeof(double), hipMemcpyDeviceToDevice, stream));
        W.lst.full_eigs++;
        if (ref_sign) W.lst.full_eigs_sign++;
        current_rank[idx] = ref_rank; min_eig[idx] = 0.0; W.last_npos = ref_npos;
    };
    for (int attempt = 0; attempt < 2; ++attempt) {
        if (g > maxnev || g < 1) break;
        lanczos(W, xp, g, true);
        if (!W.converged) {
            if (attempt == 0 && g < maxnev) { g = std::min(2 * g + 2, maxnev); continue; }
            break;
        }
        const int npos = W.count;
        W.fel_served++;
        if (npos + 2 + W.last_npos / 8 < W.last_npos) break;
        const int cert_m = opt.full_eig_lanczos_certify < 0 ? 10 : opt.full_eig_lanczos_certify;
        if (cert_m >= 2) {
            double theta = 0.0, cscale = 0.0;
            if (lanczos_certificate(W, xp, npos, cert_m, theta, cscale)) {
                const double posres = lanczos_posres();
                if (!(theta <= posres * cscale)) {
                    W.lst.full_eigs_lanczos_cert_failed++;
                    if (++W.fel_cert_fails >= 3) W.fel_disabled = true;
                    if (debug) std::fprintf(stderr, "[proxsdp] certificate failed: block %d iteration %lld theta %.3e scale %.3e npos %d\n",
                                            idx, (long long)iter, theta, cscale, npos);
                    break;
                }
                W.lst.full_eigs_lanczos_certified++;
            }
        }
        int rank = 0;
        for (int i = 0; i < npos; ++i) if (W.vals[i] > opt.tol_psd) ++rank;
        W.use_fop = false;
        if (used_fop) W.lst.fop_projections++;
// ... 1504 lines not shown
        if (nb > 0) {
            const BlockInfo& B0 = P.blocks[0];
            bb += (8.0 * (double)B0.N + 16.0 * (double)B0.n) * (double)lz_matvec_iter +
                  8.0 * (double)B0.n * (double)recon_r_iter;
        }
        st.algorithmic_bytes += bb;
    }
    if (res.trace && res.trace_rows < opt.trace_capacity) {
        double* row = res.trace + (size_t)res.trace_rows * PROXSDP_TRACE_COLS;
        row[0] = (double)k; row[1] = h_pobj.at(k); row[2] = h_dobj.at(k); row[3] = h_gap.at(k);
        row[4] = h_feas.at(k); row[5] = h_pres.at(k); row[6] = h_dres.at(k); row[7] = primal_step;
        row[8] = beta; row[9] = theta; row[10] = nb ? (double)target_rank[0] : 0.0; row[11] = (double)last_trials;
        row[12] = now_s() - loop_t0; row[13] = (double)lz_matvec_iter;
        res.trace_rows++;
    }
    if (opt.check_dual_feas && k % opt.check_dual_feas_freq == 0) {
        std::vector<double> cc(P.c_orig);
        if (stop_reason == 6) std::fill(cc.begin(), cc.end(), 0.0);
        update_dual_feasibility(cc);
    }
    if (opt.log_verbose && opt.log_freq > 0 && k % opt.log_freq == 0)
        std::printf("|%9lld| %+.4e %+.4e %.2e %.2e %.2e %.2e %4lld %8.2f\n", k, h_pobj.at(k), h_dobj.at(k),
                    h_gap.at(k), h_feas.at(k), h_pres.at(k), h_dres.at(k), nb ? target_rank[0] : 0,
                    now_s() - time0);
}

inline Solver::Loop Solver::after_iteration(long long k) {
    const int window = opt.convergence_window;
    const size_t nb = P.blocks.size();
    if (iter < certificate_search_min_iter) return Loop::next;

    if (opt.certificate_search && certificate_search) {
        if (stop_reason == 6) {
            if (h_dobj.at(k) > opt.certificate_obj_tol) {
                update_dual_feasibility(std::vector<double>(P.n, 0.0));
                if (dual_feasibility < opt.tol_feasibility_dual) {
                    certificate_found = true;
                    stop_reason_string += " [Dual ray found]";
                    return Loop::stop;
                }
            }
        } else {
            if (h_pobj.at(k) < -opt.certificate_obj_tol && h_feas.at(iter) < opt.tol_feasibility) {
                certificate_found = true;
                stop_reason_string += " [Primal ray found]";
                return Loop::stop;
            }
        }
        if ((h_pobj.at(k) < -opt.certificate_fail_tol && h_dobj.at(k) < -opt.certificate_fail_tol &&
             h_feas.at(iter) < -opt.certificate_fail_tol) || std::isnan(h_comb.at(k))) {
            stop_reason_string += " [Failed to find certificate]";
            return Loop::stop;
        }
    }

    rank_update += 1;
    if (h_gap.at(iter) <= opt.tol_gap && h_feas.at(iter) <= opt.tol_feasibility &&
        (!opt.check_dual_feas || dual_feasibility < opt.tol_feasibility_dual)) {
        if ((sharded() ? !g_not_converged_rank : convergedrank()) && soc_convergence() && iter > opt.min_iter) {
            if (!certificate_search) {
                stop_reason = 1;
                stop_reason_string = "Optimal solution found";
            } else {
                stop_reason_string += " [Failed to find certificate - type 2]";
            }
            return Loop::stop;
        } else if (rank_update > window) {
            update_cont += 1;
            if (update_cont > 0) {
                for (size_t idx = 0; idx < nb; ++idx) bump_rank((int)idx);
                rank_update = 0; update_cont = 0;
            }
        }
    } else if (k > window && h_comb.at(k - window) < h_comb.at(k) && rank_update > window) {
        update_cont += 1;
        if (update_cont > opt.divergence_min_update) {
            if (sharded() && g_any_below_full) { rank_update = 0; update_cont = 0; }
            for (size_t idx = 0; idx < nb; ++idx) {
                if (target_rank[idx] < P.blocks[idx].n) { rank_update = 0; update_cont = 0; }
                bump_rank((int)idx);
            }
        }
    } else if (h_pres.at(k) > opt.tol_primal && h_dres.at(k) < opt.tol_dual && k > window) {
        if (++ada_count > opt.adapt_window) {
            ada_count = 0;
            if (opt.line_search_flag) { beta *= (1.0 - adapt_level); primal_step /= std::sqrt(1.0 - adapt_level); }
            else { primal_step /= (1.0 - adapt_level); dual_step *= (1.0 - adapt_level); }
            adapt_level *= opt.adapt_decay;
        }
    } else if (h_pres.at(k) < opt.tol_primal && h_dres.at(k) > opt.tol_dual && k > window) {
        if (++ada_count > opt.adapt_window) {
            ada_count = 0;
            if (opt.line_search_flag) { beta /= (1.0 - adapt_level); primal_step *= std::sqrt(1.0 - adapt_level); }
            else { primal_step *= (1.0 - adapt_level); dual_step /= (1.0 - adapt_level); }
            adapt_level *= opt.adapt_decay;
        }
    }

    const double elapsed = sharded() ? g_elapsed : now_s() - time0;
    if (iter >= max_iter_local || elapsed >= time_limit) {
        if (iter > opt.min_iter_time_infeas && h_gap.max_abs_diff() < opt.infeas_stable_gap_tol &&
            h_gap.at(k) > opt.infeas_limit_gap_tol) {
            if (h_feas.at(iter) <= opt.tol_feasibility / 100) {
                if (declare(5, "Problem declared unbounded due to lack of improvement", Cert::dual_infeasible, true))
                    return Loop::stop;
            } else if (h_feas.at(iter) > opt.infeas_feasibility_tol) {
                if (declare(6, "Problem declared infeasible due to lack of improvement", Cert::infeasible, true))
                    return Loop::stop;
            }
        } else if (iter >= max_iter_local) {
            stop_reason = 3;
            stop_reason_string = "Iteration limit of " + std::to_string(max_iter_local) + " was hit";
        } else {
            stop_reason = 2;
            stop_reason_string = "Time limit hit, limit: " + std::to_string(time_limit) +
                                 " time: " + std::to_string(now_s() - time0);
        }
        if (iter >= max_iter_local || elapsed >= time_limit) return Loop::stop;
    }
    if (opt.certificate_search && certificate_search) return Loop::next;

    if ((iter > opt.min_iter_max_obj && h_dobj.at(k) > opt.max_obj) || std::isnan(h_dobj.at(k))) {
        if (declare(6, "Infeasible: |Dual objective| = " + std::to_string(h_dobj.at(k)) +
                       " > maximum allowed = " + std::to_string(opt.max_obj), Cert::infeasible))
            return Loop::stop;
    }
    if ((iter > opt.min_iter_max_obj && h_pobj.at(k) < -opt.max_obj) || std::isnan(h_pobj.at(k))) {
        if (declare(5, "Unbounded: |Primal objective| = " + std::to_string(h_pobj.at(k)) +
                       " > maximum allowed = " + std::to_string(opt.max_obj), Cert::dual_infeasible))
            return Loop::stop;
    }
    if (iter > opt.min_iter_max_obj && h_gap.at(k) > opt.infeas_limit_gap_tol &&
        h_feas.at(iter) > opt.infeas_feasibility_tol &&
        h_feas.max_abs_diff() < opt.infeas_stable_feasibility_tol) {
        if (declare(6, "Infeasible: feasibility stalled at " + std::to_string(h_feas.at(iter)), Cert::infeasible))
            return Loop::stop;
    }
    if (iter > opt.min_iter_max_obj && h_gap.at(k) > 1 - opt.infeas_gap_tol &&
        h_gap.max_abs_diff() < opt.infeas_stable_gap_tol) {
        if (std::fabs(h_dobj.at(k)) > std::fabs(h_pobj.at(k)) && h_feas.at(iter) > opt.infeas_feasibility_tol) {
            if (declare(6, "Infeasible: duality gap stalled at 100 % with |Dual objective| >> |Primal objective|", Cert::infeasible))
                return Loop::stop;
        } else if (std::fabs(h_pobj.at(k)) > std::fabs(h_dobj.at(k)) && h_feas.at(iter) <= opt.tol_feasibility) {
            if (declare(5, "Unbounded: duality gap stalled at 100 % with |Dual objective| << |Primal objective|", Cert::dual_infeasible))
                return Loop::stop;
        }
    }
    return Loop::next;
}

inline void Solver::finish() {
    PX_HIP(hipStreamSynchronize(stream));
    if (capture_state && capture_state->ints[3] == 0 && iter == capture_state->iteration) write_capture();
    for (EigWork& W : eig) harvest_full_eig_events(W);
    merge_block_stats();
    st.loop_time = now_s() - loop_t0;
    if (warm.joinable()) warm.join();

    if (opt.certificate_search && certificate_search) {
        if (certificate_found) {
            std::vector<double> cc(P.c_orig);
            if (stop_reason == 6) std::fill(cc.begin(), cc.end(), 0.0);
            cache_solution(cc);
        }
    } else {
        cache_solution(P.c_orig);
    }
    if (debug && dbg_lz[5] > 0)
        std::fprintf(stderr, "[proxsdp] single-block Lanczos: %.0f cycles; per cycle: wait for the GPU %.1f us | after-cycle host logic (eigensolve, "
                     "convergence, restart rotation staging) %.1f us; per projection: results (Ritz coefficients + rotation staging) %.1f us\n",
                     dbg_lz[5], 1e6 * dbg_lz[0] / dbg_lz[5], 1e6 * dbg_lz[1] / dbg_lz[5], 1e6 * dbg_lz[3] / std::max(1.0, (double)st.lanczos_calls));
    if (b1_dbg.p != nullptr) {
        long long t[8] = {0};
        b1_dbg.download(t, 8, stream);
        PX_HIP(hipStreamSynchronize(stream));
        if (t[4] > 0)
            std::fprintf(stderr, "[proxsdp] k_lz_block1: %lld launches, %lld steps; per launch: prologue %.2f us | step loop %.2f us (%.2f us per step) | "
                         "epilogue %.2f us\n", t[4], t[3], 0.01 * t[0] / t[4], 0.01 * t[1] / t[4], 0.01 * t[1] / std::max(1LL, t[3]), 0.01 * t[2] / t[4]);
    }
    if (debug && dbg_batch[4] > 0)
        std::fprintf(stderr, "[dbg] batched Lanczos: %.0f cycles; per cycle enqueue %.1f us, wait %.1f us, restart logic %.1f us, flush %.1f us\n",
                     dbg_batch[4], 1e6 * dbg_batch[0] / dbg_batch[4], 1e6 * dbg_batch[1] / dbg_batch[4],
                     1e6 * dbg_batch[2] / dbg_batch[4], 1e6 * dbg_batch[3] / dbg_batch[4]);
    res.stats = st;
}

inline void Solver::run() {
    const double t_init0 = now_s();
    check_run_options();
    init_parameters();
    reduce_global_constants();

    setup_device();
    setup_dense_scaling();
    b_host = P.b; h_host = P.h; c_host = P.c;
    start_host_helpers();
    alloc_iterate();
    upload_sparse_operator();
    classify_blocks();
    start_block_workers();
    setup_small_batch();
    setup_soc();
    if (P.dense()) opt.support_path = 0;
    setup_support();
    setup_dense();
    alloc_candidates();
    if (sharded() && use_support == shard_general)
        throw std::logic_error("block-sharded solve: the shard's vector path is not the one chosen for it");
    if (!initial_steps()) return;

    long long k_first = 1;
    if (resume_state) { apply_resume(); k_first = resume_state->iteration + 1; }
    if (start) apply_start();
    if (start_out) { write_start_point(); return; }
    if (capture_state) { check_state_shape(*capture_state, "capture"); capture_state->ints[3] = 0; }
    st.init_time = now_s() - t_init0;

    loop_t0 = now_s();
    const long long kmax = 2 * max_iter_local;
    for (long long k = k_first; k <= kmax; ++k) {
        if (capture_state && k == capture_state->iteration + 1 && k > k_first) write_capture();
        iterate(k);
        if (after_iteration(k) == Loop::stop) break;
    }
    finish();
}

}
```

### proxsdp.jl_amd/csrc/solver.hip.hpp

```cpp
#pragma once
#include <hip/hip_runtime.h>
#include <hip/hip_ext.h>
#include <array>
#include <memory>
#include <mutex>
#include <condition_variable>
#include <functional>
#include <exception>
#include <rocblas/rocblas.h>
#include <rocsolver/rocsolver.h>

#include <algorithm>
#include <chrono>
#include <cmath>
#include <cstdio>
#include <cstdlib>
#include <cstring>
#include <stdexcept>
#include <string>
#include <thread>
#include <tuple>
#include <type_traits>
#include <utility>
#include <vector>
// ... 10 lines not shown
#include "prep.hpp"

namespace proxsdp {

struct HipError : std::runtime_error { using std::runtime_error::runtime_error; };

#define PX_HIP(call)                                                                         \
    do {                                                                                     \
        hipError_t e_ = (call);                                                              \
        if (e_ != hipSuccess)                                                                \
            throw ::proxsdp::HipError(std::string(#call) + ": " + hipGetErrorString(e_) + " (" +       \
                           __FILE__ + ":" + std::to_string(__LINE__) + ")");                \
    } while (0)
#define PX_ROC(call)                                                                         \
    do {                                                                                     \
        rocblas_status s_ = (call);                                                          \
        if (s_ != rocblas_status_success)                                                    \
            throw ::proxsdp::HipError(std::string(#call) + ": rocblas status " + std::to_string((int)s_)); \
    } while (0)

template <typename T>
struct DevBuf {
    T* p = nullptr;
    size_t n = 0;
    DevBuf() = default;
    explicit DevBuf(size_t count) { alloc(count); }
    DevBuf(const DevBuf&) = delete;
    DevBuf& operator=(const DevBuf&) = delete;
    DevBuf(DevBuf&& o) noexcept : p(o.p), n(o.n) { o.p = nullptr; o.n = 0; }
    DevBuf& operator=(DevBuf&& o) noexcept {
        if (this != &o) { release(); p = o.p; n = o.n; o.p = nullptr; o.n = 0; }
        return *this;
    }
    ~DevBuf() { release(); }
    void alloc(size_t count) {
        release();
        n = count;
        if (count == 0) return;
        hipError_t e = hipMalloc(reinterpret_cast<void**>(&p), count * sizeof(T));
        if (e != hipSuccess) { p = nullptr; throw std::bad_alloc(); }
    }
    void release() { if (p) { (void)hipFree(p); p = nullptr; } n = 0; }
    void zero(hipStream_t s) { if (n) PX_HIP(hipMemsetAsync(p, 0, n * sizeof(T), s)); }
    void upload(const T* h, size_t count, hipStream_t s) {
        if (count) PX_HIP(hipMemcpyAsync(p, h, count * sizeof(T), hipMemcpyHostToDevice, s));
    }
    void download(T* h, size_t count, hipStream_t s) const {
        if (count) PX_HIP(hipMemcpyAsync(h, p, count * sizeof(T), hipMemcpyDeviceToHost, s));
    }
};

struct PinnedBuf {
    double* p = nullptr;
    PinnedBuf() = default;
    PinnedBuf(const PinnedBuf&) = delete;
    PinnedBuf& operator=(const PinnedBuf&) = delete;
    PinnedBuf(PinnedBuf&& o) noexcept : p(o.p) { o.p = nullptr; }
    PinnedBuf& operator=(PinnedBuf&& o) noexcept { if (this != &o) { release(); p = o.p; o.p = nullptr; } return *this; }
    ~PinnedBuf() { release(); }
    void alloc(size_t count, unsigned flags = hipHostMallocDefault) {
        release();
        if (hipHostMalloc((void**)&p, count * sizeof(double), flags) != hipSuccess) { p = nullptr; throw std::bad_alloc(); }
    }
    void release() { if (p) { (void)hipHostFree(p); p = nullptr; } }
};

template <typename H, typename Traits>
struct Owned {
    H h = nullptr;
    Owned() = default;
    Owned(const Owned&) = delete;
    Owned& operator=(const Owned&) = delete;
    Owned(Owned&& o) noexcept : h(o.h) { o.h = nullptr; }
    Owned& operator=(Owned&& o) noexcept { if (this != &o) { release(); h = o.h; o.h = nullptr; } return *this; }
    ~Owned() { release(); }
    void release() { if (h) { Traits::destroy(h); h = nullptr; } }
    operator H() const { return h; }
};
struct EventTraits { static void destroy(hipEvent_t e) { (void)hipEventDestroy(e); } };
struct StreamTraits { static void destroy(hipStream_t s) { (void)hipStreamDestroy(s); } };
struct BlasTraits { static void destroy(rocblas_handle b) { (void)rocblas_destroy_handle(b); } };
struct Event : Owned<hipEvent_t, EventTraits> {
    void create(unsigned flags = hipEventDefault) { if (!h) PX_HIP(hipEventCreateWithFlags(&h, flags)); }
};
struct Stream : Owned<hipStream_t, StreamTraits> {
    void create(unsigned flags = hipStreamDefault) { if (!h) PX_HIP(hipStreamCreateWithFlags(&h, flags)); }
};
struct BlasHandle : Owned<rocblas_handle, BlasTraits> {
    void create() { if (!h) PX_ROC(rocblas_create_handle(&h)); }
};

template <typename F>
inline double time_launches(hipStream_t s, int repeat, F&& launch) {
    Event a, b;
    a.create(); b.create();
    PX_HIP(hipEventRecord(a, s));
    for (int i = 0; i < repeat; ++i) launch();
    PX_HIP(hipEventRecord(b, s));
    PX_HIP(hipEventSynchronize(b));
    float t = 0.f;
    PX_HIP(hipEventElapsedTime(&t, a, b));
    return (double)t / repeat;
}

static inline double now_s() {
    return std::chrono::duration<double>(std::chrono::steady_clock::now().time_since_epoch()).count();
}
static inline int ceil_div(long long a, long long b) { return (int)((a + b - 1) / b); }
static inline int grid_for(long long n) {
    long long g = (n + dev::TPB - 1) / dev::TPB;
    return (int)std::max<long long>(1, std::min<long long>(g, 2048));
}
template <typename Query, typename GiveUp>
inline void poll_ready(Query query, GiveUp give_up) {
    for (unsigned spins = 0;; ++spins) {
        const hipError_t e = query();
        if (e == hipSuccess) return;
        if (e != hipErrorNotReady) PX_HIP(e);
        if ((spins & 0xfff) == 0xfff) give_up();
#if defined(__x86_64__)
        _mm_pause();
#endif
    }
}
}
#include "shard_comm.hip.hpp"
namespace proxsdp {

struct CircularVector {
    std::vector<double> v;
    int l = 0;
    void init(int len) { v.assign(len, 0.0); l = len; }
    double& at(long long i) { return v[(size_t)(((i - 1) % l + l) % l)]; }
    double max_abs_diff() const {
        double val = 0.0;
        for (int i = 0; i < l; ++i) val = std::max(val, std::fabs(v[i] - v[(i + l - 1) % l]));
        return val;
    }
};

struct EigEvents {
    std::vector<Event> e0, e1;
    size_t used = 0;
    std::pair<hipEvent_t, hipEvent_t> acquire() {
        if (used == e0.size()) {
            Event a, b;
            a.create(); b.create();
            e0.push_back(std::move(a)); e1.push_back(std::move(b));
        }
        ++used;
        return {e0[used - 1], e1[used - 1]};
    }
    void harvest(double& ms_sum, int64_t& count) {
        for (size_t s = 0; s < used; ++s) {
            float ms = 0.f;
            if (hipEventElapsedTime(&ms, e0[s], e1[s]) == hipSuccess) { ms_sum += ms; count++; }
        }
        used = 0;
    }
};

struct StreamRef {
    Stream main;
    static inline thread_local hipStream_t tl = nullptr;
    operator hipStream_t() const { return tl ? tl : main.h; }
};

struct LzRun {
    int nev = 0, krylovdim = 0, ld = 0;
    bool arpack = false, positive_part = false;
    double tol = 0.0, step_tol = 0.0;
    long long maxiter = 0;
    std::vector<double> T, Tw, D, U, f, al, be, Qa, da, ea;
    int howmany = 0, numiter = 1, converged = 0, K = 0, kfirst = 0, pos_count = -1, m_arrow = 0;
    bool pos_fail = false, presymv = false;
    double betaK = 0.0;
    const double* rec = nullptr;
    int rec_ld = 0;
    bool wide = false;
    SplitEig* splitp = nullptr;
    SplitEig& split_ref() { return *splitp; }
    bool split_ready = false;
    bool merge_active = false;
    std::vector<double> erow;
};

struct EigWork {
    int n = 0, nt = 0, npad = 0, nwg = 0, cap = 0, pld = 0;
    int64_t N = 0;
    DevBuf<double> V, Z;
    DevBuf<double> w, Ppart, hpart1, hpart2, hsum1, hred, U, lam, resid, Apart, arrow;
    DevBuf<double> resid2;
    int napart = 0;
    PinnedBuf arrow_host;
    const double* arrow_p = nullptr;
    DevBuf<double> rec;
    double* alphas_p = nullptr; double* betas_p = nullptr; dev::LanczosCtl* ctl_p = nullptr;
    PinnedBuf rec_pinned;
    double* rec_host = nullptr;
    static constexpr size_t REC_DOUBLES = 2 * dev::MAXK + sizeof(dev::LanczosCtl) / sizeof(double);
    static constexpr size_t USTAGE_DOUBLES = (size_t)dev::MAXK * dev::MAXK + 2 * dev::MAXK;
    size_t ustage_doubles = USTAGE_DOUBLES;
    bool wide = false;
    DevBuf<double> hpw1, hpw2, hsw1, hsw2, recw;
    PinnedBuf recw_pinned;
    dev::LanczosCtl* ctlw_p = nullptr;
    static constexpr size_t RECW_DOUBLES = 2 * dev::LZW_MAXK + sizeof(dev::LanczosCtl) / sizeof(double);
    DevBuf<double> A, D, E;
    DevBuf<rocblas_int> info;
    std::vector<double> resid_host;
    PinnedBuf Ustage[2];
    int ustage_next = 0;
    std::vector<double> vals;
    int count = 0, converged_eigs = 0, numiter = 0, prev_numiter = 1;
    bool converged = false;
    DevBuf<double> F, Flam, tpart, ebuf, apartf;
    DevBuf<int> ell_col, ell_sidx;
    DevBuf<int> wr_ptr, wr_row, wr_lo, wr_hi, ov_col, ov_sidx;
    dev::EllOverflow ov{};
    int ell_w = 0, F_first = 0, F_r = 0;
    bool fop_ok = false;
    bool have_factors = false;
    bool x_prev_sparse = true;
    bool use_fop = false;
    bool ritz_ok = false;
    int ritz_first = 0, ritz_r = 0;
    int last_npos = -1;
    PinnedBuf rec_early;
    SplitEig split;
    int batch_slot = 0;
    bool b1_defer = false;
    int b1_rot_K = 0;
    const double* b1_rot_U = nullptr;
    LzRun lzrun;
    long long fel_served = 0;
    bool fel_disabled = false;
    int fel_cert_fails = 0;
    DevBuf<double> warm_part;
    bool cye_pending = false;
    const double* esv = nullptr;
    proxsdp_stats lst{};
    long long mv_iter = 0, recon_r = 0;
    bool fe_pending = false;
    DevBuf<double> sgA, sgX, sgX2, sgY, sgQ, sg_part, sg_part2, sg_sc;
    PinnedBuf sg_host;
    int sg_ld = 0;
    int sg_npart = 0;
    int sg_row = -1, sg_ok = 16, sg_idle = 0, sg_hold = 0;
    bool sg_small = false;
    int sg_nt48 = 0;
    bool sg_pending = false;
    double kry_ms = -1.0, sign_ms = -1.0;
    int sign_streak = 0, sign_backoff = 0;
    int sign_verified_left = 0;
    bool sign_disabled = false, sign_check_pending = false;
    DevBuf<double> sg_cmp;
    DevBuf<double> sg_out;
    Stream stream;
    Event done;
    Stream side;
    Event ev_mid, ev_early;
    EigEvents ev, evo;
    Event fe[3];
    Event cye[2];
    Event sg_ev;
};
static_assert(std::is_nothrow_move_constructible<EigWork>::value, "eig.resize() moves workspaces");


static inline void count_matvecs(EigWork& W, long long c) {
    W.lst.symv_launches += c;
    W.lst.symv_bytes += (double)c * (8.0 * (double)W.N + 16.0 * (double)W.n);
}

static inline int lz_nch(int cols) { return (cols <= 64) ? 1 : (cols <= 128) ? 2 : (cols <= 192) ? 3 : 4; }
template <typename F>
static inline void with_nch(int cols, F&& f) {
    switch (lz_nch(cols)) {
        case 1: f(std::integral_constant<int, 1>{}); break;
        case 2: f(std::integral_constant<int, 2>{}); break;
        case 3: f(std::integral_constant<int, 3>{}); break;
        default: f(std::integral_constant<int, 4>{}); break;
    }
}

struct RotSink {
    struct Req { EigWork* W = nullptr; const double* V = nullptr; double* out = nullptr; int K = 0, ncols = 0, copy_src = -1,
                 copy_dst = 0, nextra = 0; bool valid = false; std::vector<double> data; };
    std::array<Req, dev::LZB_MAX> slot;
};

class Solver {
public:
    Solver(const proxsdp_problem& prob, const proxsdp_options& opt_in, proxsdp_result& res_out,
           ShardGroup* grp = nullptr, int grp_rank = 0)
        : opt(opt_in), res(res_out), time0(now_s()), P(prepare(prob, &opt_in, grp != nullptr || prob.reduce_fn != nullptr || prob.nccl_comm != nullptr)) {
        user_resid = prob.eig_resid;
        if (grp) comm.reset(new GroupComm(*grp, grp_rank, opt.host_wait_spin != 0));
        else if (prob.nccl_comm != nullptr) comm.reset(new RcclComm(prob.nccl_comm, st));
        else if (prob.reduce_fn != nullptr) comm.reset(new CallbackComm(prob));
        if (prob.n_coupling > 0) {
            if ((!prob.reduce_fn || !prob.reduce_vec_fn) && prob.nccl_comm == nullptr && grp == nullptr)
                throw std::invalid_argument("coupling rows need nccl_comm, or reduce_fn and reduce_vec_fn");
            if (!prob.coupling_rows || !prob.coupling_owned)
                throw std::invalid_argument("coupling rows need coupling_rows and coupling_owned");
            for (int64_t k = 0; k < prob.n_coupling; ++k) {
                const int64_t r = prob.coupling_rows[k];
                if (r < 0 || r >= prob.p + prob.m) throw std::invalid_argument("coupling row out of range");
                coup_rows.push_back((int)r);
                coup_owned.push_back(prob.coupling_owned[k] != 0);
            }
        }
    }
    Solver(const proxsdp_options& opt_in, proxsdp_result& res_out) : opt(opt_in), res(res_out) {
        time0 = now_s();
    }
    ~Solver() {
        if (warm.joinable()) warm.join();
        block_pool.reset();
    }
    void run();
    void check_run_options();
    void init_parameters();
    void reduce_global_constants();
    void start_host_helpers();
    void alloc_iterate_pairs();
    void alloc_iterate();
    void classify_blocks();
    void start_block_workers();
    void setup_small_batch();
    void setup_soc();
    bool initial_steps();
    enum class Loop { next, stop };
    void iterate(long long k);
    Loop after_iteration(long long k);
    void finish();
    enum class Cert { infeasible, dual_infeasible };
    bool declare(int reason, const std::string& str, Cert kind, bool at_limit = false);
    void cert_infeas();
    void cert_dual_infeas();
    void snapshot();
    void update_dual_feasibility(const std::vector<double>& cvec);
    double loop_t0 = 0;
    bool shard_general = false;

    void setup_device();
    void alloc_eigwork(EigWork& W, int n, int max_nev);
    void lanczos_start_vector(EigWork& W, const double* user);
    void lanczos(EigWork& W, const double* xp, int nev, bool positive_part = false);
    void lz_launch_step(EigWork& W, const double* xp, int k, int kfirst, double step_tol, bool& presymv);
    void lz_launch_finish(EigWork& W, int k, double tol, bool use_carry);
    void lz_launch_begin(EigWork& W, const double* start, dev::LanczosCtl* ctl);
    bool lanczos_certificate(EigWork& W, const double* xp, int npos, int msteps, double& theta_max, double& scale);
    void lanczos_batch(const std::vector<int>& blocks, const double* xbase, const std::vector<int>& nevs, int ctx_slot = 0);
    double dbg_batch[5] = {0, 0, 0, 0, 0};
    double dbg_lz[8] = {0, 0, 0, 0, 0, 0, 0, 0};
    static inline thread_local RotSink* rot_sink = nullptr;
    struct BatchCtx {
        DevBuf<double> U;
        PinnedBuf U_host, rec_host;
        std::unique_ptr<SpinPool> pool;
        Event ev;
    };
    std::vector<std::unique_ptr<BatchCtx>> batch_ctx;
    std::mutex batch_stats_mu;
    std::unique_ptr<SpinPool> merge_pool;
    ParFor merge_par;
    int merge_helpers() const { return opt.host_merge_threads < 0 ? 3 : std::min(15, (int)opt.host_merge_threads); }
    static constexpr size_t LZB_USTRIDE = 64 * 64 + 2 * dev::MAXK;
    void flush_rotations(RotSink& sink, BatchCtx& C);
    bool lz_init(EigWork& W, struct LzRun& R, int nev, bool positive_part);
    void lz_prepare_arrow(struct LzRun& R);
    bool lz_after_cycle(EigWork& W, struct LzRun& R, bool speculated);
    void lz_rayleigh(EigWork& W, struct LzRun& R, int K, double betaK, bool from_arrow, bool check_first);
    void lz_restart(EigWork& W, struct LzRun& R, int K, int keep, bool speculated);
    void lz_finish_run(EigWork& W, struct LzRun& R);
    void lanczos_eager(EigWork& W, const double* xp, int nev);
    void lzw_step(EigWork& W, const double* xp, int k, int kfirst, double step_tol, bool& presymv);
    void lz_merge_vectors(EigWork& W, struct LzRun& R, int ncols);
    bool lz_split_first(EigWork& W, struct LzRun& R, int k1);
    void full_eig_values(EigWork& W, const double* xp, double offscale, bool vectors, std::vector<double>& Dhost);
    void harvest_full_eig_events(EigWork& W);
    int block1_lds_cap = 0;
    DevBuf<long long> b1_dbg;
    bool block1_plan(const EigWork& W, int krylovdim, bool split_wanted) const;
    void launch_block1(EigWork& W, const double* xp, int kfirst, int krylovdim, double tol);
    bool sg48_ok = false;
    void launch_symv(EigWork& W, const double* xp, const double* v, bool use_ctl, dev::LanczosCtl* ctl = nullptr);
    void launch_symv_finish(EigWork& W, const double* xp, int kclose, double tol, bool use_carry);
    void launch_reconstruct(EigWork& W, const double* Z, int ldz, const double* lam, int r, double* xp_out,
                            const double* xp_old = nullptr, int blk = -1);
    proxsdp_psd_factors* factors_out = nullptr;
    DevBuf<double> fac_V, fac_lam, fac_part;
    void factor_residual(const double* xp, int n, const double* V, int ldv, const double* lam, int r,
                         double& resid2, double& xnorm2);
    void extract_factors(const std::vector<double>& x);
    void rotate(EigWork& W, int K, const std::vector<double>& U, int ldu, int ncols, double* out, int copy_src, int copy_dst,
                const double* extra, int nextra);

    void test_project(int idx, double* xp, int tr);
    void test_full_eig(const double* xin, double* xout) { current_rank.assign(1, 0); min_eig.assign(1, 0.0); full_eig_project(0, xin, xout, false); }
    long long test_rank() const { return current_rank.empty() ? 0 : current_rank[0]; }
    double test_min_eig() const { return min_eig.empty() ? 0.0 : min_eig[0]; }
    void test_spmv(bool transpose, const double* in, double* out);
    void test_trial_batch(proxsdp_trial_batch& t);
    void test_cone_tail(const double* x, int64_t n, const int64_t* so, const int32_t* sl, int nsoc,
                        const int64_t* oo, int none, double* x_soc, double* gap_in, double* gap_out,
                        double* x_clamp, double* mineig);
    void test_sym_product(proxsdp_sym_product& t);
    void test_sign_unpack(const double* packed, double sentinel, double* A, double* sc);

    bool debug = std::getenv("PROXSDP_HIP_DEBUG") != nullptr;
    proxsdp_options opt;
    proxsdp_result& res;
    double time0 = 0;
    Prep P;
    proxsdp_stats st{};
    const double* user_resid = nullptr;
    std::unique_ptr<ShardComm> comm;
    bool sharded() const { return comm != nullptr; }
    long long current_iteration() const { return iter; }
    std::exception_ptr shard_error;
    void reduce(std::vector<double>& sums, std::vector<double>& maxs) { if (comm) comm->reduce(stream, sums, maxs); }
    void reduce_vec_host(std::vector<double>& v) { if (!v.empty()) comm->reduce_vec_host(stream, v); }
    std::vector<int> coup_rows;
    std::vector<char> coup_owned;
    DevBuf<int> coup_rows_d;
    DevBuf<double> roww_d;
    void reduce_coupling(double* Mx_dev) {
        if (!coup_rows.empty()) comm->reduce_coupling(stream, Mx_dev, coup_rows_d.p, (int)coup_rows.size());
    }
    void wait_stream() {
        if (!comm || !comm->bounded_wait(stream)) wait_for_stream(stream, opt.host_wait_spin != 0);
    }
    const proxsdp_state* resume_state = nullptr;
    proxsdp_state* capture_state = nullptr;
    void check_state_shape(const proxsdp_state& s, const char* what) const;
    void apply_resume();
    void write_capture();
    const proxsdp_start* start = nullptr;
    proxsdp_state* start_out = nullptr;
    bool start_active = false;
    DevBuf<long long> start_ord_d;
    DevBuf<double> start_src_d, start_V, start_lam;
    void apply_start();
    void write_start_point();
    int ada_count = 0;
    void wait_event(hipEvent_t ev) {
        if (opt.host_wait_spin == 0) PX_HIP(hipEventSynchronize(ev));
        else poll_ready([&]() { return hipEventQuery(ev); }, []() {});
    }
    double g_n = 0, g_Q = 0, g_p = 0, g_m = 0, g_norm_b = 0, g_norm_h = 0, g_norm_c = 0, g_frob = 0;
    bool g_conic = false, g_not_converged_rank = false, g_any_below_full = false;
    double g_elapsed = 0;
    bool init_only = false;
    double sigma_max = 0.0;
    std::thread warm;
    std::mutex blas_mutex;
    std::unique_ptr<BlockPool> block_pool;
    bool parallel_blocks() const { return block_pool != nullptr; }
    void run_blocks(const std::vector<int>& blocks, const std::function<void(int)>& job);
    void merge_block_stats();
    void start_rocsolver_warmup();

private:
    DevBuf<double> xbuf[2], Mtybuf[2], ybuf[2], Mxbuf[2], c_d, bh_d, part, scal;
    DevBuf<int> csr_ptr, csr_col, csc_ptr, csc_row;
    DevBuf<double> csr_val, csc_val;
    DevBuf<long long> one_off, soc_off;
    DevBuf<int> soc_len;
    DevBuf<double> one_min, soc_gap_d;
    int xc = 0, mtyc = 0, yc = 0, mxc = 0;
    std::vector<int> one_blocks;
    std::vector<int> big_blocks;
    std::vector<int> small_blocks, large_blocks;
    DevBuf<long long> small_off;
    DevBuf<int> small_side, small_rank;
    PinnedBuf small_rank_host;
    int small_maxn = 0;
    int small_jacobi_max = 64;
    int small_sign_maxn = 0;
    int small_sign_cap = 0;
    bool zero_copy_small() const { return P.n <= (1 << 16); }
    bool small_pending = false;
    void project_small_blocks(double* x);
    void harvest_small_ranks();
    bool csr_wave = false;
    int rotate_lds_cap = 60 * 1024;
    int rotate_mfma_lds_cap = 0;
    static constexpr int LONG_ROW = 8192;
    DevBuf<int> seg_lo_d, seg_hi_d, long_row_d, long_ptr_d;
    DevBuf<double> segpart_d;
    int n_seg = 0, n_long = 0;
    void setup_long_rows(const std::vector<int>& rp);

    double theta = 1, beta = 1, adapt_level = 0.9, primal_step = 0, primal_step_old = 0, dual_step = 0;
    long long iter = 0;
    int rank_update = 0, update_cont = 0, stop_reason = 0;
    std::string stop_reason_string = "Not optimized";
    std::vector<long long> target_rank, current_rank;
    std::vector<double> min_eig;
    double dual_feasibility = -1.0;
    bool certificate_search = false, certificate_found = false;
    long long certificate_search_min_iter = 0;
    long long max_iter_local = 0;
    double time_limit = 0;
    int last_trials = 0;
    long long lz_matvec_iter = 0; long long recon_r_iter = 0;
    CircularVector h_gap, h_pobj, h_dobj, h_feas, h_pres, h_dres, h_comb;
    double equa_feasibility = 0, ineq_feasibility = 0;

    void primal_step_dev();
    void psd_projection(double* x);
    void project_block(int idx, const double* xin, double* xout, bool fuse, bool lanczos_done = false);
    void project_blocks(const std::vector<int>& blocks, const double* xin, double* xout, bool fuse);
    bool krylov_branch(int idx) const;
    bool batch_eligible(int idx, bool fuse) const;
    void setup_support();
    void setup_dense();
    std::vector<int> support_list() const;
    void upload_support(const std::vector<int>& supp);
    void upload_sparse_operator();
    void launch_clamp_scalars(double* x, int cnt);
    void launch_soc_project(double* x, int nsoc);
    void launch_soc_gap(const double* x, int nsoc);
    void launch_primal_update_S(double* x, double tau);
    void alloc_candidates();
    struct BatchShape {
        int gq, gx; long long cstride, ystride, mstride;
        const int* supp; long long cnt;
        const double* xold; const double* cv;
        double* mty_cur; double* mty_commit;
    };
    BatchShape batch_shape() const;
    void batch_evaluate(const dev::TrialBatch& tb, int nc, double xold_coef);
    void batch_mty(const dev::TrialBatch& tb, int nc);
    void batch_residuals(const dev::TrialBatch& tb, int nc, int c0, double xold_coef);
    const double* batch_read_back(int nc);
    const double* linesearch_and_residuals();
    void reduce_candidates(int nc);
    void record_residuals(const double* s);
    void dense_mv(const double* x, double* y, bool scaled);
    void dense_mtv(int nc, const double* Y, long long ystride, bool scaled, double* OUT, long long ostride,
                   const double* old, const double* addc, double* normpart, long long cstride, bool addback);
    void full_eig_project(int idx, const double* xp_in, double* xp_out, bool fuse);
    bool full_eig_by_lanczos(int idx, const double* xp_in, double* xp_out, bool fuse);
    bool full_eig_by_sign(int idx, const double* xp_in, double* xp_out, bool fuse, bool force = false);
    void truncated_project_dense(int idx, const double* xp_in, double* xp_out, bool fuse, int nev);
    double lanczos_posres() const {
        const double base = opt.full_eig_lanczos_posres > 0.0 ? opt.full_eig_lanczos_posres : 1e-6;
        const double tmin = std::min({opt.tol_gap, opt.tol_feasibility, opt.tol_primal, opt.tol_dual});
        return tmin > 0.0 ? std::min(base, 1e-2 * tmin) : base;
    }
    bool krylovdim_fits(int nev) const {
        const int kd = std::max(2 * nev + 1, (int)opt.eigsolver_min_lanczos);
        if (kd <= dev::LZ_KMAX) return true;
        return opt.lanczos_wide_krylov == 1 && kd <= dev::LZW_MAXK - 1 && !(opt.krylovkit_eager && opt.eigsolver != 1);
    }
    bool exact_projection_by_sign(int idx, const double* xp, double* xo, bool fuse, int nev);
    void verify_sign_engine(int idx, const double* xo);
    template <int EPI, bool FUSE>
    void sym_gemm(EigWork& W, const double* Pm, const double* Qm, double* T, const double* Y, double ca, double cb,
                  double cc, const double* dsc, double* part, double* xp_out, const double* xp_old, int blk);
    bool sign_tile48_fits(int n, int ld) const { return sg48_ok && ceil_div(n, dev::SG_T48) * dev::SG_T48 <= ld; }
    static int sym_gemm_grid(const EigWork& W, bool final_epi);
    void sign_choose_tiles(EigWork& W);
    void sign_unpack(EigWork& W, const double* xp_in, double* A, double* sc);
    void sign_scale(EigWork& W, double* sc);
    void spmv(const double* x, double* y);
    void spmv_sparse(const double* x, double* y);
    bool convergedrank() const;
    bool soc_convergence();
    double dual_feas_host(const std::vector<double>& y, const std::vector<double>& cvec,
                          std::vector<double>* dual_eq, std::vector<double>* dual_in, std::vector<double>* dual_cone);
    void cache_solution(const std::vector<double>& cvec);
    void certificate_parameters();
    void bump_rank(int idx);
    std::vector<double> b_host, h_host, c_host;
    bool have_snapshot = false;
    bool use_support = false;
    bool general_row_weights = false;
    int ns = 0, rstride = 0, n_res_wg = 0;
    std::vector<int> tile_base;
    DevBuf<int> supp_d;
    DevBuf<unsigned> mask_d;
    DevBuf<double> cS_d, xsave_d, MtyS_cur, respart_d;
    DevBuf<double> Ediag_d, Ddiag_d;
    DevBuf<double> esv_d;
    const double* Md = nullptr;
    DevBuf<double> Md_own, dmv_part;
    DevBuf<unsigned char> offdiag_d;
    int dmv_slices = 1, dmv_qpad = 0;
    static constexpr int DMV_ROWS = 8, DMV_UNR = 4;
    long long dense_passes_seen = 0;
    void upload_dense();
    void setup_dense_scaling();
    double spectral_norm_device();
    DevBuf<double> drow_d, dcol_d;
    double dense_frob2 = 0.0;
    size_t dense_ev_used = 0;
    void dense_ev_begin();
    void dense_ev_end();
    void dense_ev_harvest();
    DevBuf<double> ycand_d, Mtycand_d, bpart, bscal;
    std::vector<double> hbscal;
    PinnedBuf hscal_pin;

public:
    std::vector<EigWork> eig;
    StreamRef stream;
    BlasHandle blas;
    std::vector<std::pair<Event, Event>> dense_ev;
    Event ev_main;
};

inline void Solver::alloc_eigwork(EigWork& W, int n, int max_nev) {
    W.n = n;
    W.N = (int64_t)n * (n + 1) / 2;
    W.nt = ceil_div(n, dev::TILE);
    W.npad = W.nt * dev::TILE;
    W.nwg = ceil_div(n, dev::TPB);
    const int kd_want = std::max(2 * max_nev + 1, (int)opt.eigsolver_min_lanczos);
    W.wide = opt.lanczos_wide_krylov == 1 && kd_want > dev::LZ_KMAX;
    int kd = std::min(kd_want, W.wide ? dev::LZW_MAXK - 1 : dev::LZ_KMAX);
    W.cap = kd + 1;
    W.V.alloc((size_t)W.npad * W.cap);
    W.Z.alloc((size_t)W.npad * W.cap);
    W.w.alloc(W.npad);
    W.Ppart.alloc((size_t)W.nt * W.npad);
    W.pld = ceil_div(W.nt, dev::WAVE) * dev::WAVE;
    W.hpart1.alloc((size_t)W.pld * dev::MAXK);
    W.hpart2.alloc((size_t)W.pld * dev::MAXK);
    W.hpart1.zero(stream); W.hpart2.zero(stream);
    W.hsum1.alloc(dev::MAXK);
    W.hred.alloc(dev::MAXK); W.hred.zero(stream);
    W.napart = 8 * ceil_div(W.nt * (W.nt + 1) / 2, 8);
    W.Apart.alloc(W.napart); W.Apart.zero(stream);
    W.arrow.alloc(2 * dev::MAXK); W.arrow.zero(stream);
    W.arrow_host.alloc(2 * dev::MAXK);
    W.rec.alloc(EigWork::REC_DOUBLES);
    W.alphas_p = W.rec.p; W.betas_p = W.rec.p + dev::MAXK;
    W.ctl_p = reinterpret_cast<dev::LanczosCtl*>(W.rec.p + 2 * dev::MAXK);
    W.rec_pinned.alloc(EigWork::REC_DOUBLES);
    W.rec_host = W.rec_pinned.p;
    W.ustage_doubles = W.wide ? (size_t)dev::LZW_MAXK * dev::LZW_MAXK + 2 * dev::LZW_MAXK : EigWork::USTAGE_DOUBLES;
    W.U.alloc(W.ustage_doubles);
    W.Ustage[0].alloc(W.ustage_doubles); W.Ustage[1].alloc(W.ustage_doubles);
    if (W.wide) {
        if (W.nt > W.pld) throw std::logic_error("wide Lanczos: more producers than partial-dot records");
        const size_t hpw_doubles = dev::lzw_hpart_doubles(W.pld);
        W.hpw1.alloc(hpw_doubles); W.hpw2.alloc(hpw_doubles);
        W.hpw1.zero(stream); W.hpw2.zero(stream);
        W.hsw1.alloc(dev::KW + 1); W.hsw2.alloc(dev::KW + 1);
        W.hsw1.zero(stream); W.hsw2.zero(stream);
        W.recw.alloc(EigWork::RECW_DOUBLES); W.recw.zero(stream);
        W.ctlw_p = reinterpret_cast<dev::LanczosCtl*>(W.recw.p + 2 * dev::LZW_MAXK);
        W.recw_pinned.alloc(EigWork::RECW_DOUBLES);
    }
    W.arrow_p = W.arrow.p;
    W.lam.alloc(std::max(n, dev::MAXK));
    W.resid.alloc(W.npad);
    W.V.zero(stream); W.Z.zero(stream); W.w.zero(stream);
    W.hsum1.zero(stream); W.rec.zero(stream);
    W.resid.zero(stream);
}

inline void Solver::lanczos_start_vector(EigWork& W, const double* user) {
    W.resid_host.assign(W.npad, 0.0);
    if (user) std::copy(user, user + W.n, W.resid_host.begin());
    else start_vector(W.n, (uint64_t)opt.eigsolver_resid_seed,
                      opt.eigsolver == 1 ? opt.arpack_resid_init : opt.krylovkit_resid_init,
                      W.resid_host.data());
    double nr = norm2(W.resid_host.data(), W.n);
    if (!(nr > 0.0)) throw std::invalid_argument("Lanczos start vector has zero norm");
    for (int i = 0; i < W.n; ++i) W.resid_host[i] /= nr;
}

inline void Solver::setup_device() {
    int ndev = 0;
    PX_HIP(hipGetDeviceCount(&ndev));
    if (ndev <= 0) throw HipError("no HIP device available");
    if (opt.device_id < 0 || opt.device_id >= ndev) throw std::invalid_argument("device_id out of range");
    if (opt.lanczos_wide_krylov != 0 && opt.lanczos_wide_krylov != 1) throw std::invalid_argument("lanczos_wide_krylov must be 0 or 1");
    if (opt.lanczos_cycle_kernel == 1) opt.lanczos_cycle_kernel = 0;
    PX_HIP(hipSetDevice(opt.device_id));
    stream.main.create();
    rotate_lds_cap = 60 * 1024;
    for (int kb : {160, 156, 152, 144}) {
        if (hipFuncSetAttribute(reinterpret_cast<const void*>(dev::k_lz_rotate),
                                hipFuncAttributeMaxDynamicSharedMemorySize, kb * 1024) == hipSuccess) { rotate_lds_cap = kb * 1024; break; }
        (void)hipGetLastError();
    }
    (void)hipFuncSetAttribute(reinterpret_cast<const void*>(dev::k_lzb_rotate), hipFuncAttributeMaxDynamicSharedMemorySize, rotate_lds_cap);
    for (int kb : {156, 152, 144, 128, 96, 64}) {
        if (hipFuncSetAttribute(reinterpret_cast<const void*>(dev::k_lz_rotate_mfma),
                                hipFuncAttributeMaxDynamicSharedMemorySize, kb * 1024) == hipSuccess) { rotate_mfma_lds_cap = kb * 1024; break; }
        (void)hipGetLastError();
    }
    sg48_ok = true;
    for (const void* f : {reinterpret_cast<const void*>(dev::k_sym_gemm48<dev::SG_PLAIN, 4>), reinterpret_cast<const void*>(dev::k_sym_gemm48<dev::SG_POLY, 4>)})
        sg48_ok = sg48_ok && hipFuncSetAttribute(f, hipFuncAttributeMaxDynamicSharedMemorySize, (int)dev::sg48_lds_bytes(4)) == hipSuccess;
    if (!sg48_ok) (void)hipGetLastError();
    small_sign_cap = 0;
    for (int sd : {64, 56, 48, 40, 32, 24, 16}) {
        const size_t bytes = dev::small_sign_lds_bytes(sd);
        if (bytes <= 48 * 1024 || hipFuncSetAttribute(reinterpret_cast<const void*>(dev::k_small_sign_project),
                                                      hipFuncAttributeMaxDynamicSharedMemorySize, (int)bytes) == hipSuccess) {
            small_sign_cap = sd;
            break;
        }
        (void)hipGetLastError();
    }
    if (std::getenv("PROXSDP_HIP_DEBUG_B1") != nullptr) { b1_dbg.alloc(8); b1_dbg.zero(stream); }
    block1_lds_cap = 0;
    for (int kb : {160, 144, 128, 112, 96}) {
        bool ok = true;
        for (const void* f : {reinterpret_cast<const void*>(dev::k_lz_block1<1, false>), reinterpret_cast<const void*>(dev::k_lz_block1<2, false>),
                              reinterpret_cast<const void*>(dev::k_lz_block1<1, true>), reinterpret_cast<const void*>(dev::k_lz_block1<2, true>)})
            ok = ok && hipFuncSetAttribute(f, hipFuncAttributeMaxDynamicSharedMemorySize, kb * 1024) == hipSuccess;
        if (ok) { block1_lds_cap = kb * 1024; break; }
        (void)hipGetLastError();
    }
    blas.create();
    PX_ROC(rocblas_set_stream(blas, stream));
}

inline bool Solver::block1_plan(const EigWork& W, int krylovdim, bool split_wanted) const {
    if (!(opt.lanczos_cycle_kernel == 2 || opt.lanczos_cycle_kernel < 0) || block1_lds_cap == 0) return false;
    if (W.nt > dev::B1_MAXNT || krylovdim > dev::B1_KMAX || split_wanted || rot_sink != nullptr) return false;
    if (opt.lanczos_cycle_kernel < 0 && W.nt > dev::B1_NV) return false;
    if (W.use_fop && (W.F_r > 4 * dev::B1_NPV || W.ov.wr_ptr != nullptr || W.ell_w < 1)) return false;
    const dev::B1Lds L = dev::b1_lds_plan(W.nt, W.npad, W.use_fop, W.use_fop ? 0 : W.N, 0);
    return (size_t)L.total * sizeof(double) <= (size_t)block1_lds_cap;
}

inline void Solver::launch_block1(EigWork& W, const double* xp, int kfirst, int krylovdim, double tol) {
    dev::Block1Args a{};
    a.xp = xp; a.n = W.n; a.nt = W.nt; a.npad = W.npad;
    a.ldv = W.npad; a.kfirst = kfirst; a.kd = krylovdim; a.tol = tol;
    a.Vout = W.V.p;
    if (W.b1_rot_K > 0) {
        a.Vin = W.Z.p; a.U = W.b1_rot_U; a.rotK = W.b1_rot_K;
        W.b1_rot_K = 0;
    } else {
        a.Vin = W.V.p; a.U = nullptr; a.rotK = 0;
    }
    bool ell_lds = false;
    if (W.use_fop) {
        a.Vp = W.F.p + (size_t)W.F_first * W.npad; a.lam = W.Flam.p; a.rp = W.F_r;
        a.ell_col = W.ell_col.p; a.ell_sidx = W.ell_sidx.p; a.ell_w = W.ell_w; a.esv = W.esv;
        const dev::B1Lds Le = dev::b1_lds_plan(W.nt, W.npad, true, 0, W.ell_w);
        ell_lds = (size_t)Le.total * sizeof(double) <= (size_t)block1_lds_cap;
    }
    a.ell_in_lds = ell_lds ? 1 : 0;
    a.arrow = W.arrow_p;
    a.alphas = W.alphas_p; a.betas = W.betas_p; a.ctl = W.ctl_p;
    a.dbg = b1_dbg.p;
    const dev::B1Lds L = dev::b1_lds_plan(W.nt, W.npad, W.use_fop, W.use_fop ? 0 : W.N, ell_lds ? W.ell_w : 0);
    const size_t lds = (size_t)L.total * sizeof(double);
    const bool two = W.nt > dev::B1_NV;
    auto kern = W.use_fop ? (two ? dev::k_lz_block1<2, true> : dev::k_lz_block1<1, true>)
                          : (two ? dev::k_lz_block1<2, false> : dev::k_lz_block1<1, false>);
    const bool prof = opt.profile_symv_every > 0;
    if (prof) {
        W.cye[0].create(); W.cye[1].create();
        hipExtLaunchKernelGGL(kern, dim3(1), dim3(dev::B1_TPB), lds, stream, W.cye[0], W.cye[1], 0, a);
        W.cye_pending = true;
    } else {
        hipLaunchKernelGGL(kern, dim3(1), dim3(dev::B1_TPB), lds, stream, a);
    }
    W.lst.cycle_launches++;
    W.lst.cycle_steps += krylovdim - kfirst;
    count_matvecs(W, krylovdim - kfirst);
}

inline void Solver::start_rocsolver_warmup() {
    const int dev_id = opt.device_id;
    warm = std::thread([dev_id]() {
        if (hipSetDevice(dev_id) != hipSuccess) return;
        try {
            Stream s;
            BlasHandle h;
            s.create(); h.create();
            (void)rocblas_set_stream(h, s);
            double* buf = nullptr;
            rocblas_int* info = nullptr;
            const int n = 96;
            if (hipMalloc((void**)&buf, sizeof(double) * (n * n + 2 * n)) == hipSuccess &&
                hipMalloc((void**)&info, sizeof(rocblas_int)) == hipSuccess) {
                (void)hipMemsetAsync(buf, 0, sizeof(double) * (n * n + 2 * n), s);
                (void)rocsolver_dsyevd(h, rocblas_evect_original, rocblas_fill_upper, n, buf, n,
                                       buf + n * n, buf + n * n + n, info);
                (void)rocsolver_dsyevd(h, rocblas_evect_none, rocblas_fill_upper, n, buf, n,
                                       buf + n * n, buf + n * n + n, info);
                (void)hipStreamSynchronize(s);
            }
            if (buf) (void)hipFree(buf);
            if (info) (void)hipFree(info);
        } catch (...) {}
    });
}

template <typename K, typename... Args>
static inline void launch_prof(bool prof, hipEvent_t e0, hipEvent_t e1, K kern, dim3 grid, hipStream_t stream, Args... args) {
    if (prof) hipExtLaunchKernelGGL(kern, grid, dim3(dev::TPB), 0, stream, e0, e1, 0, args...);
    else hipLaunchKernelGGL(kern, grid, dim3(dev::TPB), 0, stream, args...);
}

inline void Solver::launch_symv(EigWork& W, const double* xp, const double* v, bool use_ctl, dev::LanczosCtl* ctl) {
    const int ntile = 8 * ceil_div(W.nt * (W.nt + 1) / 2, 8);
    const bool prof = opt.profile_symv_every > 0 && (W.lst.symv_launches % opt.profile_symv_every) == 0;
    hipEvent_t e0 = nullptr, e1 = nullptr;
    if (prof) std::tie(e0, e1) = W.ev.acquire();
    if (W.use_fop) {
        auto kern = (W.F_r <= 64) ? dev::k_fop<1> : dev::k_fop<2>;
        launch_prof(prof, e0, e1, kern, dim3(W.nt), stream,
                    v, (const double*)(W.F.p + (size_t)W.F_first * W.npad), W.npad, W.F_r,
                    (const int*)W.ell_col.p, (const int*)W.ell_sidx.p, W.ell_w, W.npad, W.esv, W.tpart.p, W.pld,
                    W.ebuf.p, W.apartf.p, (const dev::LanczosCtl*)(use_ctl ? W.ctl_p : nullptr), W.ov);
    } else {
        launch_prof(prof, e0, e1, dev::k_symv_packed, dim3(ntile), stream,
                    xp, W.n, W.nt, W.npad, v, W.Ppart.p, (const dev::LanczosCtl*)(use_ctl ? (ctl ? ctl : W.ctl_p) : nullptr), W.Apart.p);
    }
    count_matvecs(W, 1);
}

inline double* lz_hpart(EigWork& W, int k) {
    return (k & 1) ? W.hpart2.p : W.hpart1.p;
}

inline void Solver::launch_symv_finish(EigWork& W, const double* xp, int kclose, double tol, bool use_carry) {
    const int ntile = 8 * ceil_div(W.nt * (W.nt + 1) / 2, 8);
    const bool prof = opt.profile_symv_every > 0 && (W.lst.symv_launches % opt.profile_symv_every) == 0;
    hipEvent_t e0 = nullptr, e1 = nullptr;
    if (prof) std::tie(e0, e1) = W.ev.acquire();
    with_nch(kclose + 1, [&](auto nch) {
        constexpr int NCH = decltype(nch)::value;
        if (W.use_fop) {
            auto kern = (W.F_r <= 64) ? dev::k_fop_finish<1, NCH> : dev::k_fop_finish<2, NCH>;
            launch_prof(prof, e0, e1, kern, dim3(2 * W.nt), stream,
                        (const double*)W.w.p, W.V.p, W.npad, kclose, (const double*)lz_hpart(W, kclose), W.pld,
                        (const double*)W.hsum1.p, W.alphas_p, W.betas_p, W.ctl_p, tol, use_carry ? 1 : 0, W.nt,
                        (const double*)(W.F.p + (size_t)W.F_first * W.npad), W.F_r,
                        (const int*)W.ell_col.p, (const int*)W.ell_sidx.p, W.ell_w, W.npad, W.esv, W.tpart.p, W.ebuf.p,
                        W.apartf.p, W.hred.p, W.ov);
        } else {
            launch_prof(prof, e0, e1, dev::k_symv_finish<NCH>, dim3(W.nt + ntile), stream,
                        xp, W.n, W.nt, W.npad, W.Ppart.p, (const double*)W.w.p, W.V.p, W.npad, kclose,
                        (const double*)lz_hpart(W, kclose), W.pld, (const double*)W.hsum1.p, W.alphas_p, W.betas_p, W.ctl_p,
                        tol, use_carry ? 1 : 0, W.Apart.p, W.hred.p);
        }
    });
    count_matvecs(W, 1);
}

inline void Solver::lz_launch_finish(EigWork& W, int k, double tol, bool use_carry) {
    with_nch(k + 1, [&](auto nch) {
        hipLaunchKernelGGL(dev::k_lz_finish<decltype(nch)::value>, dim3(W.nt), dim3(dev::TPB), 0, stream,
                           (const double*)W.w.p, W.n, W.V.p, W.npad, k, (const double*)lz_hpart(W, k), W.pld,
                           (const double*)W.hsum1.p, W.alphas_p, W.betas_p, W.ctl_p, tol, use_carry ? 1 : 0, W.hred.p);
    });
}

inline void Solver::lz_launch_begin(EigWork& W, const double* start, dev::LanczosCtl* ctl) {
    hipLaunchKernelGGL(dev::k_lz_begin, dim3(ceil_div(W.npad, dev::TPB)), dim3(dev::TPB), 0, stream,
                       W.V.p, start, W.npad, ctl);
}

inline void Solver::launch_reconstruct(EigWork& W, const double* Z, int ldz, const double* lam, int r, double* xp_out,
                                       const double* xp_old, int blk) {
    const int ntile = 8 * ceil_div(W.nt * (W.nt + 1) / 2, 8);
    const bool mfma = opt.reconstruct_mfma == 1 || (opt.reconstruct_mfma < 0 && r >= 16);
    if (mfma) {
        W.lst.mfma_reconstructions++;
        if (use_support && xp_old != nullptr && blk >= 0)
            hipLaunchKernelGGL(dev::k_reconstruct_mfma<true>, dim3(ntile), dim3(dev::TPB), 0, stream,
                               Z, ldz, lam, r, W.n, xp_out, xp_old, mask_d.p, (long long)P.blocks[blk].off,
                               respart_d.p + tile_base[blk], rstride);
        else
            hipLaunchKernelGGL(dev::k_reconstruct_mfma<false>, dim3(ntile), dim3(dev::TPB), 0, stream,
                               Z, ldz, lam, r, W.n, xp_out, (const double*)nullptr, (const unsigned*)nullptr, 0LL,
                               (double*)nullptr, 0);
        return;
    }
    if (use_support && xp_old != nullptr && blk >= 0)
        hipLaunchKernelGGL(dev::k_reconstruct_packed<true>, dim3(ntile), dim3(dev::TPB), 0, stream,
                           Z, ldz, lam, r, W.n, xp_out, xp_old, mask_d.p, (long long)P.blocks[blk].off,
                           respart_d.p + tile_base[blk], rstride);
    else
        hipLaunchKernelGGL(dev::k_reconstruct_packed<false>, dim3(ntile), dim3(dev::TPB), 0, stream,
                           Z, ldz, lam, r, W.n, xp_out, (const double*)nullptr, (const unsigned*)nullptr, 0LL,
                           (double*)nullptr, 0);
}

inline void Solver::factor_residual(const double* xp, int n, const double* V, int ldv, const double* lam, int r,
                                    double& resid2, double& xnorm2) {
    const int nt = ceil_div(n, dev::TILE);
    const int tiles = nt * (nt + 1) / 2;
    if (fac_part.n < (size_t)2 * tiles) fac_part.alloc((size_t)2 * tiles);
    hipLaunchKernelGGL(dev::k_factor_residual, dim3(8 * ceil_div(tiles, 8)), dim3(dev::TPB), 0, stream,
                       xp, n, V, ldv, lam, r, fac_part.p);
    PX_HIP(hipGetLastError());
    std::vector<double> h((size_t)2 * tiles);
    fac_part.download(h.data(), h.size(), stream);
    PX_HIP(hipStreamSynchronize(stream));
    resid2 = 0.0; xnorm2 = 0.0;
    for (int t = 0; t < tiles; ++t) { resid2 += h[2 * t]; xnorm2 += h[2 * t + 1]; }
}

inline void Solver::rotate(EigWork& W, int K, const std::vector<double>& U, int ldu, int ncols,
                           double* out, int copy_src, int copy_dst, const double* extra, int nextra) {
    if (rot_sink != nullptr) {
        RotSink::Req& q = rot_sink->slot[W.batch_slot];
        q.W = &W; q.V = W.V.p; q.out = out; q.K = K; q.ncols = ncols; q.copy_src = copy_src; q.copy_dst = copy_dst;
        q.nextra = std::max(nextra, 0); q.valid = true;
        q.data.resize((size_t)K * std::max(ncols, 0) + (size_t)q.nextra);
        for (int c = 0; c < ncols; ++c)
            for (int j = 0; j < K; ++j) q.data[(size_t)c * K + j] = U[(size_t)c * ldu + j];
        for (int t = 0; t < q.nextra; ++t) q.data[(size_t)K * std::max(ncols, 0) + t] = extra[t];
        return;
    }
    double* tmp = W.Ustage[W.ustage_next].p;
    W.ustage_next ^= 1;
    if ((size_t)K * std::max(ncols, 1) + (size_t)std::max(nextra, 0) > W.ustage_doubles)
        throw std::logic_error("rotation staging buffer too small");
    for (int c = 0; c < ncols; ++c)
        for (int j = 0; j < K; ++j) tmp[(size_t)c * K + j] = U[(size_t)c * ldu + j];
    for (int q = 0; q < nextra; ++q) tmp[(size_t)K * ncols + q] = extra[q];
    if (W.b1_defer && nextra > 0 && K < 32 && copy_src == K && copy_dst == ncols && out == W.Z.p) {
        W.b1_rot_K = K; W.b1_rot_U = tmp;
        W.arrow_p = tmp + (size_t)K * ncols;
        return;
    }
    W.U.upload(tmp, (size_t)K * ncols + (size_t)std::max(nextra, 0), stream);
    if (nextra > 0) W.arrow_p = W.U.p + (size_t)K * ncols;
    if (W.lzrun.wide) {
        if (ncols > 0 || copy_src >= 0)
            hipLaunchKernelGGL(dev::k_lzw_rotate, dim3(W.nt, std::max(1, ceil_div(ncols, dev::LZW_RC))), dim3(dev::TPB), 0, stream,
                               (const double*)W.V.p, W.npad, K, (const double*)W.U.p, ncols, out, W.npad, copy_src, copy_dst);
        return;
    }
    {
        const int Kp = (K + 3) & ~3;
        const size_t lds_m = ((size_t)Kp * dev::RM_LDV + (size_t)dev::RM_CG * (Kp + 2)) * sizeof(double);
        if (K >= 32 && ncols >= 16 && (int)lds_m <= rotate_mfma_lds_cap) {
            hipLaunchKernelGGL(dev::k_lz_rotate_mfma, dim3(W.nt, ceil_div(ncols, dev::RM_CG)), dim3(dev::TPB), lds_m, stream,
                               (const double*)W.V.p, W.npad, K, (const double*)W.U.p, ncols, out, W.npad, copy_src, copy_dst);
            return;
        }
    }
    const int vbytes = K * (dev::LZ_ROWS + 1) * 8;
    const int maxcols = std::max(1, (rotate_lds_cap - vbytes) / (8 * K));
    int c0 = 0;
    do {
        const int cn = std::max(0, std::min(maxcols, ncols - c0));
        const bool last = (c0 + cn >= ncols);
        if (cn > 0 || (last && copy_src >= 0))
            hipLaunchKernelGGL(dev::k_lz_rotate, dim3(W.nt), dim3(dev::TPB), (size_t)K * cn * 8 + vbytes, stream,
                               W.V.p, W.npad, W.n, K, W.U.p + (size_t)c0 * K, K, cn,
                               out + (size_t)c0 * W.npad, W.npad, last ? copy_src : -1, copy_dst - c0);
        c0 += std::max(cn, 1);
    } while (c0 < ncols);
}

inline bool Solver::lz_init(EigWork& W, LzRun& R, int nev, bool positive_part) {
    R.nev = nev; R.positive_part = positive_part;
    W.b1_rot_K = 0; W.b1_rot_U = nullptr;
    R.arpack = (opt.eigsolver == 1);
    int krylovdim = std::max(2 * nev + 1, (int)opt.eigsolver_min_lanczos);
    if (positive_part) {
        const int mult10 = opt.full_eig_lanczos_kdim10 > 0 ? opt.full_eig_lanczos_kdim10 : 30;
        krylovdim = std::min(std::min(W.cap, dev::MAXK - 4) - 1, std::max(krylovdim, nev * mult10 / 10 + 8));
    }
    if (krylovdim + 1 > W.cap) throw std::invalid_argument("Lanczos workspace too small for the requested rank");
    R.krylovdim = krylovdim;
    R.wide = krylovdim > dev::LZ_KMAX;
    if (R.wide && !W.wide) throw std::logic_error("wide Lanczos: workspace has no wide records");
    R.rec = R.wide ? W.recw_pinned.p : W.rec_host;
    R.rec_ld = R.wide ? dev::LZW_MAXK : dev::MAXK;
    R.tol = R.arpack ? opt.arpack_tol : opt.krylovkit_tol;
    R.maxiter = R.arpack ? (long long)opt.arpack_max_iter : (long long)opt.krylovkit_max_iter;
    W.prev_numiter = std::max(W.numiter, 1);
    W.converged = false; W.count = 0; W.converged_eigs = 0; W.numiter = 0; W.vals.clear();
    W.lst.lanczos_calls++;
    if (R.arpack && (!(0 < nev && nev < W.n) || krylovdim > W.n)) return false;
    R.step_tol = R.arpack ? 0.0 : R.tol;
    R.ld = krylovdim + 1;
    R.T.assign((size_t)R.ld * R.ld, 0.0); R.D.assign(R.ld, 0.0); R.f.assign(R.ld, 0.0);
    R.al.assign(R.ld, 0.0); R.be.assign(R.ld, 0.0);
    R.howmany = nev; R.numiter = 1; R.converged = 0; R.K = 0; R.kfirst = 0; R.pos_count = -1;
    R.pos_fail = false; R.presymv = false; R.betaK = 0.0;
    R.split_ready = false; R.merge_active = false;
    R.splitp = &W.split;
    return true;
}

inline void Solver::lz_merge_vectors(EigWork& W, LzRun& R, int ncols) {
    const double t0 = now_s();
    const int K = R.K;
    std::vector<int> cols(std::max(ncols, 1));
    for (int c = 0; c < ncols; ++c) cols[c] = K - 1 - c;
    R.U.assign((size_t)K * std::max(ncols, 1), 0.0);
    if (ncols > 0) R.split_ref().M.vectors(cols.data(), ncols, R.U.data());
    W.lst.host_eig_time += now_s() - t0;
}

inline void Solver::lz_prepare_arrow(LzRun& R) {
    R.m_arrow = R.kfirst;
    if (R.m_arrow <= 0) return;
    const int n1 = R.m_arrow + 1, ld = R.ld;
    R.Qa.assign((size_t)n1 * n1, 0.0); R.da.assign(n1, 0.0); R.ea.assign(n1, 0.0);
    for (int j = 0; j < R.m_arrow; ++j) {
        R.Qa[(size_t)j * n1 + j] = R.T[(size_t)j * ld + j];
        R.Qa[(size_t)j * n1 + R.m_arrow] = R.Qa[(size_t)R.m_arrow * n1 + j] = R.T[(size_t)j * ld + R.m_arrow];
    }
    householder_tridiag(n1, R.Qa.data(), R.da.data(), R.ea.data());
}

inline bool Solver::lz_after_cycle(EigWork& W, LzRun& R, bool speculated) {
    const int krylovdim = R.krylovdim, ld = R.ld, kfirst = R.kfirst, nev = R.nev;
    const double tol = R.tol;
    std::vector<double>& T = R.T; std::vector<double>& D = R.D; std::vector<double>& f = R.f;
    std::vector<double>& al = R.al; std::vector<double>& be = R.be;
    dev::LanczosCtl hctl{};
    std::copy(R.rec, R.rec + krylovdim, al.begin());
    std::copy(R.rec + R.rec_ld, R.rec + R.rec_ld + krylovdim, be.begin());
    std::memcpy(&hctl, R.rec + 2 * R.rec_ld, sizeof(hctl));
    const int Kend = hctl.stop ? hctl.kstop : krylovdim;
    W.lst.lanczos_matvecs += (Kend - kfirst);
    count_matvecs(W, -(long long)(krylovdim - Kend));
    W.mv_iter += (Kend - kfirst);
    for (int k = kfirst; k < Kend; ++k) {
        T[(size_t)k * ld + k] = al[k];
        if (k + 1 < Kend) { T[(size_t)k * ld + k + 1] = be[k]; T[(size_t)(k + 1) * ld + k] = be[k]; }
    }
    const int K = R.K = Kend;
    const double betaK = R.betaK = be[K - 1];
    if (!(betaK == betaK)) {
        R.converged = 0; R.pos_fail = true; R.howmany = 0;
        return false;
    }
    if (betaK <= tol && K < R.howmany && !R.arpack) R.howmany = K;
    R.merge_active = false;
    if (K > 1 && R.split_ready && K == krylovdim) {
        const double te0 = now_s();
        if (R.split_ref().second(K, al.data(), be.data()) == 0) {
            R.erow.resize(K);
            R.split_ref().M.row_of_vectors(K - 1, R.erow.data());
            for (int c = 0; c < K; ++c) {
                D[c] = R.split_ref().M.evals[K - 1 - c];
                f[c] = betaK * R.erow[K - 1 - c];
            }
            R.merge_active = true;
            W.lst.host_eigs++; W.lst.host_eig_merges++;
        }
        W.lst.host_eig_time += now_s() - te0;
    }
    R.split_ready = false;
    if (!R.merge_active) lz_rayleigh(W, R, K, betaK, true, kfirst == 0);
    int converged = 0;
    if (!R.arpack) {
        double tol_c = tol;
        if (R.positive_part && opt.full_eig_lanczos_tol > 0.0)
            tol_c = std::max(tol, opt.full_eig_lanczos_tol * std::max(std::fabs(D[0]), std::fabs(D[K - 1])));
        while (converged < K && std::fabs(f[converged]) <= tol_c) ++converged;
    } else {
        const double eps23 = std::pow(2.220446049250313e-16 / 2.0, 2.0 / 3.0);
        int want = std::min(nev, K);
        for (int i = 0; i < want; ++i)
            if (std::fabs(f[i]) <= tol * std::max(eps23, std::fabs(D[i]))) ++converged;
    }
    R.converged = converged;
    if (R.positive_part) {
        int j = 0;
        while (j < K && D[j] > 0.0) ++j;
        if (j > nev) { R.pos_fail = true; return false; }
        const double scale = std::max(std::fabs(D[0]), std::fabs(D[K - 1]));
        int jn = j;
        while (jn < K && D[jn] >= -1e-12 * scale) ++jn;
        const double posres = lanczos_posres();
        if (converged >= j && (jn == K || std::fabs(f[jn]) <= std::max(tol, posres * scale))) { R.pos_count = j; return false; }
        if (K < krylovdim || R.numiter == R.maxiter) { R.pos_fail = true; return false; }
    } else {
        if (converged >= R.howmany) return false;
        if (K < krylovdim) return false;
    }
    if (R.numiter == R.maxiter) return false;
    const int keep = R.arpack ? std::min(krylovdim - 1, nev + std::max(1, (krylovdim - nev) / 2))
                              : (3 * krylovdim + 2 * converged) / 5;
    lz_restart(W, R, K, keep, speculated);
    return true;
}

inline void Solver::lz_rayleigh(EigWork& W, LzRun& R, int K, double betaK, bool from_arrow, bool check_first) {
    std::vector<double>& D = R.D; std::vector<double>& U = R.U; std::vector<double>& f = R.f;
    if (K == 1) {
        D[0] = R.T[0]; U.assign(1, 1.0); f[0] = betaK;
        return;
    }
    R.Tw.assign((size_t)K * K, 0.0);
    for (int c = 0; c < K; ++c)
        for (int r = 0; r < K; ++r) R.Tw[(size_t)c * K + r] = R.T[(size_t)c * R.ld + r];
    std::vector<double> Dasc(K);
    const double te0 = now_s();
    if (from_arrow && R.m_arrow > 0 && K > R.m_arrow)
        symeig_tridiag_from(K, R.m_arrow, R.Qa.data(), R.da.data(), R.ea.data(), R.al.data(), R.be.data(), R.Tw.data(), Dasc.data());
    else
        symeig_dense(K, R.Tw.data(), Dasc.data(), check_first);
    W.lst.host_eig_time += now_s() - te0; W.lst.host_eigs++;
    U.assign((size_t)K * K, 0.0);
    for (int c = 0; c < K; ++c) {
        D[c] = Dasc[K - 1 - c];
        for (int r = 0; r < K; ++r) U[(size_t)c * K + r] = R.Tw[(size_t)(K - 1 - c) * K + r];
        f[c] = betaK * U[(size_t)c * K + (K - 1)];
    }
}

inline void Solver::lz_restart(EigWork& W, LzRun& R, int K, int keep, bool speculated) {
    const std::vector<double>& D = R.D; const std::vector<double>& f = R.f;
    if (!R.wide) for (int j = 0; j < keep; ++j) { W.arrow_host.p[j] = f[j]; W.arrow_host.p[dev::MAXK + j] = D[j]; }
    if (R.merge_active) lz_merge_vectors(W, R, keep);
    rotate(W, K, R.U, K, keep, W.Z.p, K, keep, W.arrow_host.p, R.wide ? 0 : 2 * dev::MAXK);
    std::swap(W.V.p, W.Z.p);
    std::fill(R.T.begin(), R.T.end(), 0.0);
    const int ld = R.ld;
    for (int j = 0; j < keep; ++j) {
        R.T[(size_t)j * ld + j] = D[j];
        R.T[(size_t)j * ld + keep] = f[j];
        R.T[(size_t)keep * ld + j] = f[j];
    }
    R.kfirst = keep;
    R.presymv = speculated;
    ++R.numiter;
    W.lst.lanczos_restarts++;
}

inline void Solver::lz_finish_run(EigWork& W, LzRun& R) {
    const int K = R.K, nev = R.nev;
    W.numiter = R.numiter;
    if (R.positive_part) {
        if (R.pos_fail || R.pos_count < 0) { W.converged = false; return; }
        W.count = R.pos_count; W.converged_eigs = R.pos_count; W.converged = true;
        W.vals.assign(R.D.begin(), R.D.begin() + R.pos_count);
        if (R.pos_count > 0 && R.merge_active) lz_merge_vectors(W, R, R.pos_count);
        if (R.pos_count > 0) rotate(W, K, R.U, K, R.pos_count, W.Z.p, -1, 0, nullptr, 0);
        return;
    }
    if (R.pos_fail) { W.converged = false; return; }
    if (R.arpack) {
        W.converged_eigs = R.converged;
        if (R.converged < nev) { W.converged = false; return; }
        W.count = nev;
        W.vals.assign(R.D.begin(), R.D.begin() + nev);
        std::reverse(W.vals.begin(), W.vals.end());
        std::vector<double> Ur((size_t)K * nev);
        for (int c = 0; c < nev; ++c)
            for (int r = 0; r < K; ++r) Ur[(size_t)c * K + r] = R.U[(size_t)(nev - 1 - c) * K + r];
        rotate(W, K, Ur, K, nev, W.Z.p, -1, 0, nullptr, 0);
        W.converged = true;
        return;
    }
    int howmany = R.howmany;
    if (R.converged > howmany) howmany = R.converged;
    W.count = howmany;
    W.vals.assign(R.D.begin(), R.D.begin() + howmany);
    W.converged_eigs = R.converged;
    W.converged = (R.converged != 0);
    if (R.merge_active) lz_merge_vectors(W, R, howmany);
    rotate(W, K, R.U, K, howmany, W.Z.p, -1, 0, nullptr, 0);
}

inline void Solver::lanczos_eager(EigWork& W, const double* xp, int nev) {
    LzRun& R = W.lzrun;
    W.use_fop = false;
    if (!lz_init(W, R, nev, false)) return;
    if (R.arpack) throw std::invalid_argument("krylovkit_eager applies to eigsolver = 2 (KrylovKit) only");
    if (R.wide) throw std::invalid_argument("krylovkit_eager: Krylov dimension > 255 is not supported");
    const int kd = R.krylovdim, ld = R.ld;
    const double tol = R.tol;
    lz_launch_begin(W, W.resid.p, W.ctl_p);
    std::vector<double>& T = R.T; std::vector<double>& f = R.f;
    std::vector<double> fstep(2 * dev::MAXK, 0.0);
    int K = 0, kfirst = 0, converged = 0;
    double beta = 0.0;
    while (true) {
        const int k = K;
        launch_symv(W, xp, W.V.p + (size_t)k * W.npad, true);
        int keep = kfirst;
        if (k > kfirst) {
            std::fill(fstep.begin(), fstep.begin() + k, 0.0);
            fstep[k - 1] = beta;
            W.arrow.upload(fstep.data(), (size_t)k, stream);
            W.arrow_p = W.arrow.p;
            keep = k;
        }
        with_nch(k + 1, [&](auto nch) {
            auto kern = dev::k_lz_orth<decltype(nch)::value, 0>;
            hipLaunchKernelGGL(kern, dim3(W.nt), dim3(dev::TPB), 0, stream,
                               (const double*)W.Ppart.p, W.nt, W.npad, (const double*)W.V.p, W.npad, k, W.w.p,
                               (const double*)W.hred.p, lz_hpart(W, k), W.pld, W.hsum1.p, (const dev::LanczosCtl*)W.ctl_p,
                               (const double*)W.alphas_p, (const double*)W.betas_p, (const double*)W.Apart.p, W.napart, 1,
                               (const double*)W.arrow_p, keep, dev::FopArgs{});
        });
        lz_launch_finish(W, k, 0.0, false);
        PX_HIP(hipMemcpyAsync(W.rec_host, W.rec.p, EigWork::REC_DOUBLES * sizeof(double), hipMemcpyDeviceToHost, stream));
        PX_HIP(hipStreamSynchronize(stream));
        const double al_k = W.rec_host[k];
        beta = W.rec_host[dev::MAXK + k];
        W.lst.lanczos_matvecs++; W.mv_iter++;
        if (!(beta == beta) || !(al_k == al_k)) { R.pos_fail = true; R.K = K; break; }
        T[(size_t)k * ld + k] = al_k;
        if (k > kfirst) { T[(size_t)(k - 1) * ld + k] = T[(size_t)k * ld + (k - 1)] = W.rec_host[dev::MAXK + k - 1]; }
        K = k + 1;
        if (beta <= tol && K < R.howmany) R.howmany = K;
        if (K == kd || beta <= tol || K >= R.howmany) {
            lz_rayleigh(W, R, K, beta, false, false);
            converged = 0;
            while (converged < K && std::fabs(f[converged]) <= tol) ++converged;
            R.K = K; R.converged = converged;
            if (converged >= R.howmany) break;
        }
        if (K < kd) {
            if (beta <= tol) { R.K = K; break; }
            continue;
        }
        if (R.numiter == R.maxiter) break;
        lz_restart(W, R, K, (3 * kd + 2 * converged) / 5, false);
        kfirst = K = R.kfirst;
    }
    lz_finish_run(W, R);
}

inline bool Solver::lz_split_first(EigWork& W, LzRun& R, int k1) {
    R.split_ready = false;
    R.m_arrow = 0;
    if (hipEventSynchronize(W.ev_early) != hipSuccess) return false;
    const double t0 = now_s();
    const double* al_e = W.rec_early.p;
    const double* be_e = W.rec_early.p + dev::MAXK;
    dev::LanczosCtl c{};
    std::memcpy(&c, W.rec_early.p + 2 * dev::MAXK, sizeof(c));
    const int m = R.kfirst;
    bool ok = !c.stop;
    for (int j = m; ok && j < k1; ++j) ok = (al_e[j] == al_e[j]) && (be_e[j] == be_e[j]) && be_e[j] > 0.0;
    if (ok) {
        std::vector<double> Dk(std::max(m, 1)), fk(std::max(m, 1));
        for (int j = 0; j < m; ++j) { Dk[j] = R.T[(size_t)j * R.ld + j]; fk[j] = R.T[(size_t)j * R.ld + m]; }
        ok = R.split_ref().first(k1, m, Dk.data(), fk.data(), al_e, be_e) == 0;
    }
    R.split_ready = ok;
    W.lst.host_eig_overlap_time += now_s() - t0;
    return ok;
}

inline void Solver::lz_launch_step(EigWork& W, const double* xp, int k, int kfirst, double step_tol, bool& presymv) {
    if (k == kfirst) {
        if (!presymv) launch_symv(W, xp, W.V.p + (size_t)k * W.npad, true);
        else count_matvecs(W, 1);
        presymv = false;
    } else {
        launch_symv_finish(W, xp, k - 1, step_tol, k - 1 > kfirst);
    }
    dev::FopArgs fo{};
    if (W.use_fop) {
        fo.Vp = W.F.p + (size_t)W.F_first * W.npad; fo.lam = W.Flam.p; fo.rp = W.F_r;
        fo.tpart = W.tpart.p; fo.ebuf = W.ebuf.p; fo.apart = W.apartf.p;
    }
    const bool prof_o = opt.profile_symv_every > 0 && (W.lst.symv_launches % opt.profile_symv_every) == 1;
    hipEvent_t e0 = nullptr, e1 = nullptr;
    if (prof_o) std::tie(e0, e1) = W.evo.acquire();
    auto launch_orth = [&](auto kern) {
        launch_prof(prof_o, e0, e1, kern, dim3(W.nt), stream,
                    (const double*)W.Ppart.p, W.nt, W.npad, (const double*)W.V.p, W.npad, k, W.w.p,
                    (const double*)W.hred.p, lz_hpart(W, k), W.pld, W.hsum1.p,
                    (const dev::LanczosCtl*)W.ctl_p, (const double*)W.alphas_p, (const double*)W.betas_p,
                    (const double*)W.Apart.p, W.napart, k == kfirst ? 1 : 0, (const double*)W.arrow_p,
                    kfirst, fo);
    };
    with_nch(k + 1, [&](auto nch) {
        constexpr int NCH = decltype(nch)::value;
        if (!W.use_fop) launch_orth(dev::k_lz_orth<NCH, 0>);
        else if (W.F_r <= 64) launch_orth(dev::k_lz_orth<NCH, 1>);
        else launch_orth(dev::k_lz_orth<NCH, 2>);
    });
}

inline bool Solver::lanczos_certificate(EigWork& W, const double* xp, int npos, int msteps, double& theta_max, double& scale) {
    if (npos + msteps + 1 > W.cap || npos + msteps + 1 > dev::KLD || msteps < 2) return false;
    if (W.resid2.n == 0) {
        std::vector<double> r2(W.npad, 0.0);
        start_vector(W.n, (uint64_t)opt.eigsolver_resid_seed ^ 0x9e3779b97f4a7c15ull, 3, r2.data());
        W.resid2.alloc(W.npad);
        W.resid2.upload(r2.data(), W.npad, stream);
        PX_HIP(hipStreamSynchronize(stream));
    }
    std::swap(W.V.p, W.Z.p);
    if (npos == 0) {
        lz_launch_begin(W, W.resid2.p, W.ctl_p);
    } else {
        PX_HIP(hipMemcpyAsync(W.w.p, W.resid2.p, (size_t)W.npad * sizeof(double), hipMemcpyDeviceToDevice, stream));
        const int kc = npos - 1;
        with_nch(npos, [&](auto nch) {
            hipLaunchKernelGGL(dev::k_lz_measure<decltype(nch)::value>, dim3(W.nt), dim3(dev::TPB), 0, stream,
                               (const double*)W.w.p, (const double*)W.V.p, W.npad, kc, lz_hpart(W, kc), W.pld, W.ctl_p);
        });
        lz_launch_finish(W, kc, 0.0, false);
    }
    for (int j = 0; j < npos; ++j) { W.arrow_host.p[j] = 0.0; W.arrow_host.p[dev::MAXK + j] = W.vals[j]; }
    if (npos > 0) {
        PX_HIP(hipMemcpyAsync(W.arrow.p, W.arrow_host.p, (size_t)npos * sizeof(double), hipMemcpyHostToDevice, stream));
        PX_HIP(hipMemcpyAsync(W.arrow.p + dev::MAXK, W.arrow_host.p + dev::MAXK, (size_t)npos * sizeof(double), hipMemcpyHostToDevice, stream));
    }
    W.arrow_p = W.arrow.p;
    const int kend = npos + msteps;
    bool presymv = false;
    for (int k = npos; k < kend; ++k) lz_launch_step(W, xp, k, npos, 0.0, presymv);
    lz_launch_finish(W, kend - 1, 0.0, kend - 1 > npos);
    PX_HIP(hipMemcpyAsync(W.rec_host, W.rec.p, EigWork::REC_DOUBLES * sizeof(double), hipMemcpyDeviceToHost, stream));
    wait_stream();
    std::swap(W.V.p, W.Z.p);
    W.evo.used = 0; W.ev.used = 0;
    W.lst.lanczos_matvecs += msteps; W.mv_iter += msteps; W.lst.cert_matvecs += msteps;
    dev::LanczosCtl hctl{};
    std::memcpy(&hctl, W.rec_host + 2 * dev::MAXK, sizeof(hctl));
    if (hctl.stop) msteps = std::max(0, std::min(msteps, hctl.kstop - npos));
    if (msteps < 1) return false;
    const double* al = W.rec_host + npos;
    const double* be = W.rec_host + dev::MAXK + npos;
    std::vector<double> T((size_t)msteps * msteps, 0.0), d(msteps, 0.0);
    for (int j = 0; j < msteps; ++j) {
        if (!(al[j] == al[j]) || !(j + 1 < msteps ? be[j] == be[j] : true)) return false;
        T[(size_t)j * msteps + j] = al[j];
        if (j + 1 < msteps) T[(size_t)j * msteps + j + 1] = T[(size_t)(j + 1) * msteps + j] = be[j];
    }
    if (msteps == 1) d[0] = al[0];
    else if (symeig_dense(msteps, T.data(), d.data(), true) != 0) return false;
    theta_max = d[msteps - 1];
    scale = std::max({std::fabs(d[0]), std::fabs(theta_max), npos > 0 ? std::fabs(W.vals[0]) : 0.0});
    return true;
}

inline void Solver::lanczos(EigWork& W, const double* xp, int nev, bool positive_part) {
    W.ritz_ok = false;
    if (opt.krylovkit_eager && opt.eigsolver != 1 && !positive_part) { lanczos_eager(W, xp, nev); return; }
    LzRun& R = W.lzrun;
    if (!lz_init(W, R, nev, positive_part)) return;
    const int krylovdim = R.krylovdim;
    const double step_tol = R.step_tol;
    const bool wide = R.wide;
    if (wide) W.lst.wide_krylov_projections++;
    if (krylovdim >= 96) QlPool::get().arm();
    dev::LanczosCtl* const ctl = wide ? W.ctlw_p : W.ctl_p;
    const bool warm_start = positive_part ? (opt.lanczos_warm_start >= 0) : (opt.lanczos_warm_start > 0);
    if (!wide && warm_start && W.fop_ok && W.have_factors && W.F_r > 0 && W.tpart.n > 0) {
        const int nb = ceil_div(W.npad, dev::TPB);
        hipLaunchKernelGGL(dev::k_lz_warm_sum, dim3(nb), dim3(dev::TPB), 0, stream,
                           W.V.p, (const double*)(W.F.p + (size_t)W.F_first * W.npad), W.npad, W.F_r,
                           (const double*)W.resid.p, W.npad, W.warm_part.p,
                           (const double*)(positive_part && W.F_r <= dev::TPB ? W.Flam.p : nullptr),
                           positive_part ? opt.full_eig_lanczos_warm_pow : 0.0);
        hipLaunchKernelGGL(dev::k_lz_warm_scale, dim3(nb), dim3(dev::TPB), 0, stream,
                           W.V.p, W.npad, (const double*)W.warm_part.p, nb, W.ctl_p);
        W.lst.warm_starts++;
    } else
        lz_launch_begin(W, W.resid.p, ctl);

    const int merge_from = opt.host_eig_merge == 0 ? (1 << 30) : (opt.host_eig_merge == 1 ? 24 : 64);
    const bool blk1 = !wide && block1_plan(W, krylovdim, !R.arpack && krylovdim >= merge_from);
    const bool use_split = !wide && !blk1 && !R.arpack && krylovdim >= merge_from;
    struct PoolGuard { SpinPool* p; ~PoolGuard() { if (p) p->disarm(); } } pool_guard{nullptr};
    W.split.M.par = nullptr;
    if (use_split && merge_helpers() > 0 && StreamRef::tl == nullptr) {
        if (!merge_pool) {
            merge_pool.reset(new SpinPool(merge_helpers()));
            merge_par = [this](int n, const std::function<void(int)>& body) { merge_pool->run(n, body); };
        }
        merge_pool->arm();
        pool_guard.p = merge_pool.get();
        W.split.M.par = &merge_par;
        W.split.M.nchunk = merge_helpers() + 1;
    }
    if (use_split && W.side == nullptr) {
        W.side.create(hipStreamNonBlocking);
        W.ev_mid.create(hipEventDisableTiming);
        W.ev_early.create(hipEventDisableTiming);
        W.rec_early.alloc(EigWork::REC_DOUBLES);
    }
    struct DeferGuard {
        EigWork& W;
        DeferGuard(EigWork& w, bool on) : W(w) { W.b1_defer = on; }
        ~DeferGuard() { W.b1_defer = false; }
    };
    while (true) {
        const int kfirst = R.kfirst;
        const int k1 = (kfirst == 0) ? (18 * krylovdim) / 25 : kfirst + 1;
        const bool split_cycle = use_split && k1 >= 1 && k1 <= krylovdim - 2;
        if (wide) {
            for (int k = kfirst; k < krylovdim; ++k) lzw_step(W, xp, k, kfirst, step_tol, R.presymv);
        } else if (blk1) {
            launch_block1(W, xp, kfirst, krylovdim, step_tol);
            R.presymv = false;
        } else {
            for (int k = kfirst; k < krylovdim; ++k) {
                lz_launch_step(W, xp, k, kfirst, step_tol, R.presymv);
                if (split_cycle && k == k1) {
                    PX_HIP(hipEventRecord(W.ev_mid, stream));
                    PX_HIP(hipStreamWaitEvent(W.side, W.ev_mid, 0));
                    PX_HIP(hipMemcpyAsync(W.rec_early.p, W.rec.p, EigWork::REC_DOUBLES * sizeof(double), hipMemcpyDeviceToHost, W.side));
                    PX_HIP(hipEventRecord(W.ev_early, W.side));
                }
            }
            lz_launch_finish(W, krylovdim - 1, step_tol, krylovdim - 1 > kfirst);
        }
        const bool speculate = !blk1 && (W.prev_numiter > 1 || R.numiter > 1);
        if (speculate) {
            launch_symv(W, xp, W.V.p + (size_t)krylovdim * W.npad, true, ctl);
            count_matvecs(W, -1);
        }
        if (wide) PX_HIP(hipMemcpyAsync(W.recw_pinned.p, W.recw.p, EigWork::RECW_DOUBLES * sizeof(double), hipMemcpyDeviceToHost, stream));
        else PX_HIP(hipMemcpyAsync(W.rec_host, W.rec.p, EigWork::REC_DOUBLES * sizeof(double), hipMemcpyDeviceToHost, stream));
        if (!(split_cycle && lz_split_first(W, R, k1))) lz_prepare_arrow(R);
        const double tdbg0 = debug ? now_s() : 0.0;
        wait_stream();
        if (debug) { dbg_lz[0] += now_s() - tdbg0; dbg_lz[5] += 1.0; }
        if (W.cye_pending) {
            W.cye_pending = false;
            float ms = 0.f;
            if (hipEventElapsedTime(&ms, W.cye[0], W.cye[1]) == hipSuccess) W.lst.cycle_ms += ms;
        }
        W.ev.harvest(W.lst.symv_profiled_ms, W.lst.symv_profiled);
        W.evo.harvest(W.lst.orth_profiled_ms, W.lst.orth_profiled);
        const double tdbg1 = debug ? now_s() : 0.0;
        bool go_on;
        {
            DeferGuard defer(W, blk1);
            go_on = lz_after_cycle(W, R, speculate);
        }
        if (debug) dbg_lz[1] += now_s() - tdbg1;
        if (!go_on) break;
    }
    const double tdbg2 = debug ? now_s() : 0.0;
    lz_finish_run(W, R);
    if (debug) dbg_lz[3] += now_s() - tdbg2;
}

inline void Solver::lzw_step(EigWork& W, const double* xp, int k, int kfirst, double step_tol, bool& presymv) {
    if (k == kfirst && presymv) {
        count_matvecs(W, 1);
    } else {
        launch_symv(W, xp, W.V.p + (size_t)k * W.npad, true, W.ctlw_p);
    }
    presymv = false;
    const dev::LanczosCtl* ctl = W.ctlw_p;
    const int nred = ceil_div(k + 2, dev::TPB);
    hipLaunchKernelGGL(dev::k_lzw_dots, dim3(W.nt), dim3(dev::TPB), 0, stream,
                       (const double*)W.Ppart.p, W.nt, W.npad, (const double*)W.V.p, W.npad, k, W.w.p, W.hpw1.p, ctl);
    hipLaunchKernelGGL(dev::k_lzw_reduce, dim3(nred), dim3(dev::TPB), 0, stream,
                       (const double*)W.hpw1.p, W.pld, W.nt, k, W.hsw1.p, ctl, 0);
    hipLaunchKernelGGL(dev::k_lzw_update, dim3(W.nt), dim3(dev::TPB), 0, stream,
                       W.w.p, (const double*)W.V.p, W.npad, k, (const double*)W.hsw1.p, W.hpw2.p, W.pld, ctl);
    hipLaunchKernelGGL(dev::k_lzw_reduce, dim3(nred), dim3(dev::TPB), 0, stream,
                       (const double*)W.hpw2.p, W.pld, W.nt, k, W.hsw2.p, ctl, 1);
    hipLaunchKernelGGL(dev::k_lzw_close, dim3(W.nt), dim3(dev::TPB), 0, stream,
                       (const double*)W.w.p, W.V.p, W.npad, k, (const double*)W.hsw1.p, (const double*)W.hsw2.p,
                       W.recw.p, W.recw.p + dev::LZW_MAXK, W.ctlw_p, step_tol);
}

inline void Solver::flush_rotations(RotSink& S, BatchCtx& C) {
    dev::LzRotBatch B{};
    size_t used = 0, lds = 0;
    int nt = 0;
    for (RotSink::Req& r : S.slot) {
        if (!r.valid) continue;
        r.valid = false;
        const size_t len = r.data.size();
        if (used + len > (size_t)dev::LZB_MAX * LZB_USTRIDE) throw std::logic_error("flush_rotations: staging buffer too small");
        std::memcpy(C.U_host.p + used, r.data.data(), len * sizeof(double));
        B.r[B.nb++] = dev::LzRot{r.V, C.U.p + used, r.out, r.K, r.ncols, r.copy_src, r.copy_dst};
        if (r.nextra > 0) r.W->arrow_p = C.U.p + used + (size_t)r.K * std::max(r.ncols, 0);
        lds = std::max(lds, ((size_t)r.K * std::max(r.ncols, 0) + (size_t)r.K * (dev::LZ_ROWS + 1)) * sizeof(double));
        B.npad = r.W->npad; nt = r.W->nt;
        used += (len + 7) & ~(size_t)7;
    }
    if (B.nb == 0) return;
    if ((int)lds > rotate_lds_cap) throw std::logic_error("flush_rotations: LDS budget exceeded");
    PX_HIP(hipMemcpyAsync(C.U.p, C.U_host.p, used * sizeof(double), hipMemcpyHostToDevice, stream));
    hipLaunchKernelGGL(dev::k_lzb_rotate, dim3(nt, 1, B.nb), dim3(dev::TPB), lds, stream, B);
}

inline void Solver::lanczos_batch(const std::vector<int>& blocks, const double* xbase, const std::vector<int>& nevs, int ctx_slot) {
    const int nb = (int)blocks.size();
    if (ctx_slot < 0 || ctx_slot >= (int)batch_ctx.size() || !batch_ctx[ctx_slot]) throw std::logic_error("lanczos_batch: no context for this group");
    BatchCtx& C = *batch_ctx[ctx_slot];
    const bool concurrent = StreamRef::tl != nullptr;
    long long steps_local = 0;
    if (nb < 1 || nb > dev::LZB_MAX) throw std::invalid_argument("lanczos_batch: 1..LZB_MAX blocks");
    auto Rq = [&](int q) -> LzRun& { return eig[blocks[q]].lzrun; };
    std::vector<char> live(nb, 0), ran(nb, 0);
    EigWork& W0 = eig[blocks[0]];
    dev::LzBatch B{};
    B.n = W0.n; B.nt = W0.nt; B.npad = W0.npad; B.pld = W0.pld; B.napart = W0.napart; B.nb = nb;
    for (int q = 0; q < nb; ++q) {
        EigWork& W = eig[blocks[q]];
        W.use_fop = false;
        W.ritz_ok = false;
        W.batch_slot = q;
        live[q] = ran[q] = lz_init(W, Rq(q), nevs[q], false) ? 1 : 0;
        if (Rq(q).krylovdim > 63) throw std::invalid_argument("lanczos_batch: krylovdim > 63");
        B.tol = Rq(q).step_tol;
    }
    auto fill = [&](int q) -> dev::LzBlk& {
        EigWork& W = eig[blocks[q]];
        dev::LzBlk& b = B.b[q];
        b.xp = xbase + P.blocks[blocks[q]].off;
        b.Ppart = W.Ppart.p; b.wbuf = W.w.p; b.V = W.V.p; b.hpart1 = W.hpart1.p; b.hpart2 = W.hpart2.p;
        b.hsum = W.hsum1.p; b.alphas = W.alphas_p; b.betas = W.betas_p; b.ctl = W.ctl_p; b.Apart = W.Apart.p;
        b.hred = W.hred.p; b.arrow = W.arrow_p; b.resid = W.resid.p;
        return b;
    };
    const int ntile = 8 * ceil_div(W0.nt * (W0.nt + 1) / 2, 8);
    if (C.U.n == 0) {
        C.U.alloc(dev::LZB_MAX * LZB_USTRIDE); C.U_host.alloc(dev::LZB_MAX * LZB_USTRIDE);
        C.rec_host.alloc(dev::LZB_MAX * EigWork::REC_DOUBLES);
    }
    RotSink sink;
    const int nhelp = std::min(nb, opt.block_threads < 0 ? 8 : (int)opt.block_threads) - 1;
    if (nhelp >= 1 && (!C.pool || C.pool->helpers() < nhelp)) C.pool.reset(new SpinPool(nhelp));
    SpinPool* pool = (nhelp >= 1) ? C.pool.get() : nullptr;
    struct SinkGuard { SpinPool* p; ~SinkGuard() { Solver::rot_sink = nullptr; if (p) p->disarm(); } } guard{pool};
    rot_sink = &sink;
    if (pool) pool->arm();
    for (int q = 0; q < nb; ++q) fill(q).mode = live[q] ? 1 : 0;
    hipLaunchKernelGGL(dev::k_lzb_begin, dim3(ceil_div(W0.npad, dev::TPB), 1, nb), dim3(dev::TPB), 0, stream, B);
    long long nlaunch = 0, prof_blocks = 0;
    double tp0 = debug ? now_s() : 0.0;
    auto lap = [&](double& acc) { if (debug && !concurrent) { const double t = now_s(); acc += t - tp0; tp0 = t; } };
    std::vector<char> presymv(nb, 0);
    C.ev.create(hipEventDisableTiming);
    double* const rec_out = C.rec_host.p;
    const int rec_n = (int)EigWork::REC_DOUBLES;
    while (true) {
        int tmax = 0, nlive = 0;
        for (int q = 0; q < nb; ++q)
            if (live[q]) { tmax = std::max(tmax, Rq(q).krylovdim - Rq(q).kfirst); ++nlive; }
        if (nlive == 0) break;
        for (int t = 0; t <= tmax; ++t) {
            bool any_orth = false, any_mv = false;
            for (int q = 0; q < nb; ++q) {
                dev::LzBlk& b = fill(q);
                b.mode = 0;
                if (!live[q]) continue;
                const int k = Rq(q).kfirst + t, kd = Rq(q).krylovdim;
                b.k = k; b.keep = Rq(q).kfirst;
                b.mode = (t == 0) ? (presymv[q] ? 0 : 1) : (k < kd) ? 2 : (k == kd) ? 3 : 0;
                any_mv = any_mv || b.mode != 0;
                if (k < kd) {
                    any_orth = true;
                    count_matvecs(eig[blocks[q]], 1);
                }
            }
            const bool prof = any_mv && opt.profile_symv_every > 0 && t > 0 && t < tmax && (nlaunch++ % opt.profile_symv_every) == 0;
            if (prof) {
                const auto ev = W0.ev.acquire();
                hipExtLaunchKernelGGL(dev::k_lzb_mv, dim3(W0.nt + ntile, 1, nb), dim3(dev::TPB), 0, stream,
                                      ev.first, ev.second, 0, B, rec_out, rec_n);
                int act = 0;
                for (int q = 0; q < nb; ++q) act += (B.b[q].mode == 2) ? 1 : 0;
                prof_blocks += act;
            } else if (any_mv)
            hipLaunchKernelGGL(dev::k_lzb_mv, dim3(W0.nt + ntile, 1, nb), dim3(dev::TPB), 0, stream, B, rec_out, rec_n);
            if (!any_orth) continue;
            for (int q = 0; q < nb; ++q) {
                dev::LzBlk& b = B.b[q];
                const bool act = live[q] && b.k < Rq(q).krylovdim;
                b.mode = act ? 1 : 0;
            }
            hipLaunchKernelGGL(dev::k_lzb_orth, dim3(W0.nt, 1, nb), dim3(dev::TPB), 0, stream, B);
            steps_local += nlive;
        }
        PX_HIP(hipEventRecord(C.ev, stream));
        for (int q = 0; q < nb; ++q) {
            dev::LzBlk& b = fill(q);
            b.mode = live[q] ? 1 : 0;
            b.k = live[q] ? Rq(q).krylovdim : 0; b.keep = 0;
        }
        hipLaunchKernelGGL(dev::k_lzb_mv, dim3(W0.nt + ntile, 1, nb), dim3(dev::TPB), 0, stream, B, (double*)nullptr, 0);
        for (int q = 0; q < nb; ++q) presymv[q] = live[q];
        for (int q = 0; q < nb; ++q) if (live[q]) lz_prepare_arrow(Rq(q));
        lap(dbg_batch[0]);
        wait_event(C.ev);
        lap(dbg_batch[1]);
        for (int q = 0; q < nb; ++q)
            if (live[q]) std::memcpy(eig[blocks[q]].rec_host, C.rec_host.p + (size_t)q * EigWork::REC_DOUBLES, EigWork::REC_DOUBLES * sizeof(double));
        W0.ev.harvest(W0.lst.symv_profiled_ms, W0.lst.symv_profiled);
        std::exception_ptr err[dev::LZB_MAX] = {};
        auto job = [&](int q) {
// ... 422 lines not shown
```

Baseline: 528.5.

## Hand off Lanczos cycle record via coherent host memory and sequence flag

The Lanczos finish kernel now writes alphas, betas and the control block straight into coherent pinned host memory and publishes a sequence word with a system-scope release store. The host spins on that word instead of issuing a device-to-host copy and synchronising the whole stream, so a speculative symv can stay queued. The restart rotation reuses Ritz vectors staged directly in the upload buffer, and the rotation kernel writes the eigenvalues to device memory so a separate lam upload is skipped. Event harvesting is deferred and tolerates events that are not ready. The cost is added complexity, reliance on coherent host memory ordering, and host CPU spinning.

```diff
diff --git a/include/proxsdp_hip.h b/include/proxsdp_hip.h
--- a/include/proxsdp_hip.h
+++ b/include/proxsdp_hip.h
@@ -128,7 +128,7 @@
     int32_t general_batch;
     int32_t full_eig_lanczos_certify;
     int32_t host_merge_threads;
-    int32_t reserved_i[1];
+    int32_t host_handoff;
     double  full_eig_lanczos_tol;
     double  reserved_d[1];
     int32_t equilibration_reference_aliasing;
diff --git a/proxsdp.jl_amd/binding.py b/proxsdp.jl_amd/binding.py
--- a/proxsdp.jl_amd/binding.py
+++ b/proxsdp.jl_amd/binding.py
@@ -98,7 +98,7 @@
     a("full_eig_lanczos_verify", i32); a("full_eig_lanczos_posres", f64); a("full_eig_lanczos_kdim10", i32)
     a("sign_small_tile_max", i32); a("host_eig_threads", i32); a("block_threads", i32)
     a("host_eig_merge", i32); a("block_batch", i32); a("rocsolver_warmup", i32); a("debug_fail_iteration", i32); a("host_wait_spin", i32)
-    a("sign_start_row", i32); a("general_batch", i32); a("full_eig_lanczos_certify", i32); a("host_merge_threads", i32); a("reserved_i", i32 * 1)
+    a("sign_start_row", i32); a("general_batch", i32); a("full_eig_lanczos_certify", i32); a("host_merge_threads", i32); a("host_handoff", i32)
     a("full_eig_lanczos_tol", f64); a("reserved_d", f64 * 1)
     a("equilibration_reference_aliasing", i32); a("reserved_i3", i32 * 2)
     a("block_batch_groups", i32); a("lanczos_wide_krylov", i32); a("reserved_i2", i32 * 7); a("full_eig_lanczos_warm_pow", f64); a("reserved_d2", f64 * 3)
diff --git a/proxsdp.jl_amd/csrc/host_util.hpp b/proxsdp.jl_amd/csrc/host_util.hpp
--- a/proxsdp.jl_amd/csrc/host_util.hpp
+++ b/proxsdp.jl_amd/csrc/host_util.hpp
@@ -552,7 +552,7 @@
         PX_OPT(rocsolver_warmup, OT_I32), PX_OPT(debug_fail_iteration, OT_I32), PX_OPT(host_wait_spin, OT_I32), PX_OPT(sign_start_row, OT_I32), PX_OPT(general_batch, OT_I32),
         PX_OPT(full_eig_lanczos_certify, OT_I32), PX_OPT(full_eig_lanczos_tol, OT_F64), PX_OPT(host_merge_threads, OT_I32),
         PX_OPT(equilibration_reference_aliasing, OT_I32), PX_OPT(block_batch_groups, OT_I32), PX_OPT(full_eig_lanczos_warm_pow, OT_F64),
-        PX_OPT(lanczos_wide_krylov, OT_I32),
+        PX_OPT(lanczos_wide_krylov, OT_I32), PX_OPT(host_handoff, OT_I32),
     };
     return t;
 }
@@ -597,7 +597,7 @@
     o->host_eig_merge = -1; o->block_batch = -1; o->rocsolver_warmup = 0; o->host_wait_spin = -1; o->sign_start_row = -1; o->general_batch = -1;
     o->full_eig_lanczos_certify = -1; o->full_eig_lanczos_tol = 0.0; o->host_merge_threads = -1;
     o->equilibration_reference_aliasing = 1; o->block_batch_groups = -1; o->full_eig_lanczos_warm_pow = 1.0;
-    o->lanczos_wide_krylov = 0;
+    o->lanczos_wide_krylov = 0; o->host_handoff = -1;
 }
 
 inline int set_option(proxsdp_options* o, const char* name, double v) {
diff --git a/proxsdp.jl_amd/csrc/kernels.hip.hpp b/proxsdp.jl_amd/csrc/kernels.hip.hpp
--- a/proxsdp.jl_amd/csrc/kernels.hip.hpp
+++ b/proxsdp.jl_amd/csrc/kernels.hip.hpp
@@ -674,12 +674,21 @@
 k_lz_finish(const double* __restrict__ wbuf, int n, double* __restrict__ V, int ldv, int k,
             const double* __restrict__ hpart_in, int pld, const double* __restrict__ h1,
             double* __restrict__ alphas, double* __restrict__ betas, LanczosCtl* __restrict__ ctl, double tol,
-            int use_carry, double* __restrict__ hred) {
+            int use_carry, double* __restrict__ hred, double* __restrict__ rec_out, unsigned long long* __restrict__ seq_out,
+            unsigned long long seq) {
     __shared__ double s_h[64 * NCH + 1];
     __shared__ double s_d[NWAVE * LZ_ROWS];
     __shared__ double s_beta;
     lz_finish_body<NCH>(wbuf, V, ldv, k, hpart_in, pld, h1, alphas, betas, ctl, tol, use_carry, blockIdx.x, s_h, s_d, &s_beta, hred,
                         (int)gridDim.x);
+    if (rec_out != nullptr && blockIdx.x == 0) {
+        __syncthreads();
+        for (int t = threadIdx.x; t <= k; t += TPB) { rec_out[t] = alphas[t]; rec_out[MAXK + t] = betas[t]; }
+        if (threadIdx.x == 0) *reinterpret_cast<LanczosCtl*>(rec_out + 2 * MAXK) = *ctl;
+        __threadfence_system();
+        __syncthreads();
+        if (threadIdx.x == 0) __hip_atomic_store(seq_out, seq, __ATOMIC_RELEASE, __HIP_MEMORY_SCOPE_SYSTEM);
+    }
 }
 
 template <int NCH>
@@ -1249,10 +1258,12 @@
 constexpr int RM_CG = 16;
 __global__ void __launch_bounds__(TPB)
 k_lz_rotate_mfma(const double* __restrict__ V, int ldv, int K, const double* __restrict__ U, int ncols,
-                 double* __restrict__ out, int ldo, int copy_src, int copy_dst) {
+                 double* __restrict__ out, int ldo, int copy_src, int copy_dst, double* __restrict__ lam_out, int nlam) {
     extern __shared__ double s_mem[];
     const int Kp = (K + 3) & ~3;
     const int ldu = Kp + 2;
+    if (lam_out != nullptr && blockIdx.x == 0 && blockIdx.y == 0)
+        for (int t = threadIdx.x; t < nlam; t += TPB) lam_out[t] = U[(long long)K * ncols + t];
     double* s_V = s_mem;
     double* s_U = s_mem + (size_t)Kp * RM_LDV;
     const int lane = threadIdx.x & 63;
diff --git a/proxsdp.jl_amd/csrc/pdhg_loop.hip.hpp b/proxsdp.jl_amd/csrc/pdhg_loop.hip.hpp
--- a/proxsdp.jl_amd/csrc/pdhg_loop.hip.hpp
+++ b/proxsdp.jl_amd/csrc/pdhg_loop.hip.hpp
@@ -153,7 +153,7 @@
     if (!lanczos_done) {
         if (exact_projection_by_sign(idx, xp, xo, fuse, nev)) return;
         const double t_kry = opt.psd_sign_engine == 1 ? now_s() : 0.0;
-        lanczos(W, xp, nev);
+        lanczos(W, xp, nev, false, handoff_on());
         if (opt.psd_sign_engine == 1 && W.converged) {
             const double ms = (now_s() - t_kry) * 1e3;
             W.kry_ms = W.kry_ms < 0 ? ms : 0.75 * W.kry_ms + 0.25 * ms;
@@ -162,6 +162,7 @@
     W.use_fop = false;
     if (used_fop) W.lst.fop_projections++;
     if (!W.converged) {
+        harvest_step_events(W);
         W.lst.krylov_fallbacks++;
         W.have_factors = false; W.x_prev_sparse = false;
         full_eig_project(idx, xp, xo, fuse);
@@ -180,9 +181,12 @@
     }
     current_rank[idx] += npos;
     W.last_npos = npos;
-    if (npos > 0) W.lam.upload(W.vals.data() + first, npos, stream);
+    const bool lam_there = !lanczos_done && W.lam_on_device && first == 0 && npos <= W.count;
+    W.lam_on_device = false;
+    if (npos > 0 && !lam_there) W.lam.upload(W.vals.data() + first, npos, stream);
     launch_reconstruct(W, W.Z.p + (size_t)first * W.npad, W.npad, W.lam.p, npos, xo,
                        fuse ? xp : nullptr, fuse ? idx : -1);
+    harvest_step_events(W);
     W.recon_r += npos;
     if (W.fop_ok) {
         std::swap(W.Z.p, W.F.p);
@@ -1993,7 +1997,7 @@
 inline void Solver::finish() {
     PX_HIP(hipStreamSynchronize(stream));
     if (capture_state && capture_state->ints[3] == 0 && iter == capture_state->iteration) write_capture();
-    for (EigWork& W : eig) harvest_full_eig_events(W);
+    for (EigWork& W : eig) { harvest_full_eig_events(W); harvest_step_events(W); }
     merge_block_stats();
     st.loop_time = now_s() - loop_t0;
     if (warm.joinable()) warm.join();
@@ -2011,6 +2015,10 @@
         std::fprintf(stderr, "[proxsdp] single-block Lanczos: %.0f cycles; per cycle: wait for the GPU %.1f us | after-cycle host logic (eigensolve, "
                      "convergence, restart rotation staging) %.1f us; per projection: results (Ritz coefficients + rotation staging) %.1f us\n",
                      dbg_lz[5], 1e6 * dbg_lz[0] / dbg_lz[5], 1e6 * dbg_lz[1] / dbg_lz[5], 1e6 * dbg_lz[3] / std::max(1.0, (double)st.lanczos_calls));
+    if (debug && dbg_lz[5] > 0)
+        std::fprintf(stderr, "[proxsdp] single-block Lanczos, per cycle: enqueue of the steps %.1f us, with the host work under the cycle %.1f us; "
+                     "per projection: between two projections (rotation's launch to the next cycle's first) %.1f us\n",
+                     1e6 * dbg_lz[6] / dbg_lz[5], 1e6 * dbg_lz[2] / dbg_lz[5], 1e6 * dbg_lz[7] / std::max(1.0, (double)st.lanczos_calls));
     if (b1_dbg.p != nullptr) {
         long long t[8] = {0};
         b1_dbg.download(t, 8, stream);
diff --git a/proxsdp.jl_amd/csrc/solver.hip.hpp b/proxsdp.jl_amd/csrc/solver.hip.hpp
--- a/proxsdp.jl_amd/csrc/solver.hip.hpp
+++ b/proxsdp.jl_amd/csrc/solver.hip.hpp
@@ -186,11 +186,17 @@
         return {e0[used - 1], e1[used - 1]};
     }
     void harvest(double& ms_sum, int64_t& count) {
+        size_t kept = 0;
         for (size_t s = 0; s < used; ++s) {
             float ms = 0.f;
-            if (hipEventElapsedTime(&ms, e0[s], e1[s]) == hipSuccess) { ms_sum += ms; count++; }
-        }
-        used = 0;
+            const hipError_t e = hipEventElapsedTime(&ms, e0[s], e1[s]);
+            if (e == hipSuccess) { ms_sum += ms; count++; }
+            else if (e == hipErrorNotReady) {
+                if (kept != s) { std::swap(e0[kept], e0[s]); std::swap(e1[kept], e1[s]); }
+                ++kept;
+            }
+        }
+        used = kept;
     }
 };
 
@@ -214,6 +220,7 @@
     bool wide = false;
     SplitEig* splitp = nullptr;
     SplitEig& split_ref() { return *splitp; }
+    bool hand_off = false;
     bool split_ready = false;
     bool merge_active = false;
     std::vector<double> erow;
@@ -232,6 +239,11 @@
     double* alphas_p = nullptr; double* betas_p = nullptr; dev::LanczosCtl* ctl_p = nullptr;
     PinnedBuf rec_pinned;
     double* rec_host = nullptr;
+    unsigned long long* rec_seq_host = nullptr;
+    unsigned long long rec_seq = 0;
+    bool harvest_pending = false;
+    const double* u_staged = nullptr;
+    bool lam_on_device = false;
     static constexpr size_t REC_DOUBLES = 2 * dev::MAXK + sizeof(dev::LanczosCtl) / sizeof(double);
     static constexpr size_t USTAGE_DOUBLES = (size_t)dev::MAXK * dev::MAXK + 2 * dev::MAXK;
     size_t ustage_doubles = USTAGE_DOUBLES;
@@ -381,14 +393,18 @@
     void setup_device();
     void alloc_eigwork(EigWork& W, int n, int max_nev);
     void lanczos_start_vector(EigWork& W, const double* user);
-    void lanczos(EigWork& W, const double* xp, int nev, bool positive_part = false);
+    void lanczos(EigWork& W, const double* xp, int nev, bool positive_part = false, bool hand_off = false);
     void lz_launch_step(EigWork& W, const double* xp, int k, int kfirst, double step_tol, bool& presymv);
-    void lz_launch_finish(EigWork& W, int k, double tol, bool use_carry);
+    void lz_launch_finish(EigWork& W, int k, double tol, bool use_carry, bool hand_off = false);
+    void wait_cycle_record(EigWork& W);
+    void harvest_step_events(EigWork& W);
+    bool handoff_on() const { return opt.host_handoff != 0; }
     void lz_launch_begin(EigWork& W, const double* start, dev::LanczosCtl* ctl);
     bool lanczos_certificate(EigWork& W, const double* xp, int npos, int msteps, double& theta_max, double& scale);
     void lanczos_batch(const std::vector<int>& blocks, const double* xbase, const std::vector<int>& nevs, int ctx_slot = 0);
     double dbg_batch[5] = {0, 0, 0, 0, 0};
     double dbg_lz[8] = {0, 0, 0, 0, 0, 0, 0, 0};
+    double dbg_lz_out = 0.0;
     static inline thread_local RotSink* rot_sink = nullptr;
     struct BatchCtx {
         DevBuf<double> U;
@@ -430,7 +446,7 @@
                          double& resid2, double& xnorm2);
     void extract_factors(const std::vector<double>& x);
     void rotate(EigWork& W, int K, const std::vector<double>& U, int ldu, int ncols, double* out, int copy_src, int copy_dst,
-                const double* extra, int nextra);
+                const double* extra, int nextra, bool extra_is_lam = false);
 
     void test_project(int idx, double* xp, int tr);
     void test_full_eig(const double* xin, double* xout) { current_rank.assign(1, 0); min_eig.assign(1, 0.0); full_eig_project(0, xin, xout, false); }
@@ -675,8 +691,10 @@
     W.rec.alloc(EigWork::REC_DOUBLES);
     W.alphas_p = W.rec.p; W.betas_p = W.rec.p + dev::MAXK;
     W.ctl_p = reinterpret_cast<dev::LanczosCtl*>(W.rec.p + 2 * dev::MAXK);
-    W.rec_pinned.alloc(EigWork::REC_DOUBLES);
+    W.rec_pinned.alloc(EigWork::REC_DOUBLES + 1, hipHostMallocCoherent);
     W.rec_host = W.rec_pinned.p;
+    W.rec_seq_host = reinterpret_cast<unsigned long long*>(W.rec_pinned.p + EigWork::REC_DOUBLES);
+    *W.rec_seq_host = 0; W.rec_seq = 0;
     W.ustage_doubles = W.wide ? (size_t)dev::LZW_MAXK * dev::LZW_MAXK + 2 * dev::LZW_MAXK : EigWork::USTAGE_DOUBLES;
     W.U.alloc(W.ustage_doubles);
     W.Ustage[0].alloc(W.ustage_doubles); W.Ustage[1].alloc(W.ustage_doubles);
@@ -888,12 +906,37 @@
     count_matvecs(W, 1);
 }
 
-inline void Solver::lz_launch_finish(EigWork& W, int k, double tol, bool use_carry) {
+inline void Solver::lz_launch_finish(EigWork& W, int k, double tol, bool use_carry, bool hand_off) {
+    const unsigned long long seq = hand_off ? ++W.rec_seq : 0ULL;
     with_nch(k + 1, [&](auto nch) {
         hipLaunchKernelGGL(dev::k_lz_finish<decltype(nch)::value>, dim3(W.nt), dim3(dev::TPB), 0, stream,
                            (const double*)W.w.p, W.n, W.V.p, W.npad, k, (const double*)lz_hpart(W, k), W.pld,
-                           (const double*)W.hsum1.p, W.alphas_p, W.betas_p, W.ctl_p, tol, use_carry ? 1 : 0, W.hred.p);
+                           (const double*)W.hsum1.p, W.alphas_p, W.betas_p, W.ctl_p, tol, use_carry ? 1 : 0, W.hred.p,
+                           hand_off ? W.rec_host : (double*)nullptr, hand_off ? W.rec_seq_host : (unsigned long long*)nullptr, seq);
     });
+}
+
+inline void Solver::wait_cycle_record(EigWork& W) {
+    const unsigned long long want = W.rec_seq;
+    for (unsigned spins = 0;; ++spins) {
+        if (__atomic_load_n(W.rec_seq_host, __ATOMIC_ACQUIRE) == want) return;
+        if ((spins & 0xfff) == 0xfff) {
+            const hipError_t e = hipStreamQuery(stream);
+            if (e != hipSuccess && e != hipErrorNotReady) PX_HIP(e);
+            if (e == hipSuccess && __atomic_load_n(W.rec_seq_host, __ATOMIC_ACQUIRE) != want)
+                throw std::logic_error("Lanczos cycle record: the stream drained without the sequence word");
+        }
+#if defined(__x86_64__)
+        _mm_pause();
+#endif
+    }
+}
+
+inline void Solver::harvest_step_events(EigWork& W) {
+    if (!W.harvest_pending) return;
+    W.ev.harvest(W.lst.symv_profiled_ms, W.lst.symv_profiled);
+    W.evo.harvest(W.lst.orth_profiled_ms, W.lst.orth_profiled);
+    W.harvest_pending = W.ev.used > 0 || W.evo.used > 0;
 }
 
 inline void Solver::lz_launch_begin(EigWork& W, const double* start, dev::LanczosCtl* ctl) {
@@ -943,7 +986,7 @@
 }
 
 inline void Solver::rotate(EigWork& W, int K, const std::vector<double>& U, int ldu, int ncols,
-                           double* out, int copy_src, int copy_dst, const double* extra, int nextra) {
+                           double* out, int copy_src, int copy_dst, const double* extra, int nextra, bool extra_is_lam) {
     if (rot_sink != nullptr) {
         RotSink::Req& q = rot_sink->slot[W.batch_slot];
         q.W = &W; q.V = W.V.p; q.out = out; q.K = K; q.ncols = ncols; q.copy_src = copy_src; q.copy_dst = copy_dst;
@@ -956,10 +999,16 @@
     }
     double* tmp = W.Ustage[W.ustage_next].p;
     W.ustage_next ^= 1;
+    const int Kp = (K + 3) & ~3;
+    const size_t lds_m = ((size_t)Kp * dev::RM_LDV + (size_t)dev::RM_CG * (Kp + 2)) * sizeof(double);
+    const bool mfma = !W.lzrun.wide && K >= 32 && ncols >= 16 && (int)lds_m <= rotate_mfma_lds_cap;
+    if (extra_is_lam && !(mfma && !W.b1_defer)) { extra_is_lam = false; extra = nullptr; nextra = 0; }
     if ((size_t)K * std::max(ncols, 1) + (size_t)std::max(nextra, 0) > W.ustage_doubles)
         throw std::logic_error("rotation staging buffer too small");
-    for (int c = 0; c < ncols; ++c)
-        for (int j = 0; j < K; ++j) tmp[(size_t)c * K + j] = U[(size_t)c * ldu + j];
+    if (W.u_staged != tmp)
+        for (int c = 0; c < ncols; ++c)
+            for (int j = 0; j < K; ++j) tmp[(size_t)c * K + j] = U[(size_t)c * ldu + j];
+    W.u_staged = nullptr;
     for (int q = 0; q < nextra; ++q) tmp[(size_t)K * ncols + q] = extra[q];
     if (W.b1_defer && nextra > 0 && K < 32 && copy_src == K && copy_dst == ncols && out == W.Z.p) {
         W.b1_rot_K = K; W.b1_rot_U = tmp;
@@ -967,21 +1016,19 @@
         return;
     }
     W.U.upload(tmp, (size_t)K * ncols + (size_t)std::max(nextra, 0), stream);
-    if (nextra > 0) W.arrow_p = W.U.p + (size_t)K * ncols;
+    if (nextra > 0 && !extra_is_lam) W.arrow_p = W.U.p + (size_t)K * ncols;
     if (W.lzrun.wide) {
         if (ncols > 0 || copy_src >= 0)
             hipLaunchKernelGGL(dev::k_lzw_rotate, dim3(W.nt, std::max(1, ceil_div(ncols, dev::LZW_RC))), dim3(dev::TPB), 0, stream,
                                (const double*)W.V.p, W.npad, K, (const double*)W.U.p, ncols, out, W.npad, copy_src, copy_dst);
         return;
     }
-    {
-        const int Kp = (K + 3) & ~3;
-        const size_t lds_m = ((size_t)Kp * dev::RM_LDV + (size_t)dev::RM_CG * (Kp + 2)) * sizeof(double);
-        if (K >= 32 && ncols >= 16 && (int)lds_m <= rotate_mfma_lds_cap) {
-            hipLaunchKernelGGL(dev::k_lz_rotate_mfma, dim3(W.nt, ceil_div(ncols, dev::RM_CG)), dim3(dev::TPB), lds_m, stream,
-                               (const double*)W.V.p, W.npad, K, (const double*)W.U.p, ncols, out, W.npad, copy_src, copy_dst);
-            return;
-        }
+    if (mfma) {
+        hipLaunchKernelGGL(dev::k_lz_rotate_mfma, dim3(W.nt, ceil_div(ncols, dev::RM_CG)), dim3(dev::TPB), lds_m, stream,
+                           (const double*)W.V.p, W.npad, K, (const double*)W.U.p, ncols, out, W.npad, copy_src, copy_dst,
+                           extra_is_lam ? W.lam.p : (double*)nullptr, extra_is_lam ? nextra : 0);
+        W.lam_on_device = extra_is_lam;
+        return;
     }
     const int vbytes = K * (dev::LZ_ROWS + 1) * 8;
     const int maxcols = std::max(1, (rotate_lds_cap - vbytes) / (8 * K));
@@ -1024,7 +1071,7 @@
     R.al.assign(R.ld, 0.0); R.be.assign(R.ld, 0.0);
     R.howmany = nev; R.numiter = 1; R.converged = 0; R.K = 0; R.kfirst = 0; R.pos_count = -1;
     R.pos_fail = false; R.presymv = false; R.betaK = 0.0;
-    R.split_ready = false; R.merge_active = false;
+    R.split_ready = false; R.merge_active = false; R.hand_off = false;
     R.splitp = &W.split;
     return true;
 }
@@ -1034,6 +1081,13 @@
     const int K = R.K;
     std::vector<int> cols(std::max(ncols, 1));
     for (int c = 0; c < ncols; ++c) cols[c] = K - 1 - c;
+    if (R.hand_off && rot_sink == nullptr && (size_t)K * std::max(ncols, 1) <= W.ustage_doubles) {
+        double* slot = W.Ustage[W.ustage_next].p;
+        if (ncols > 0) R.split_ref().M.vectors(cols.data(), ncols, slot);
+        W.u_staged = slot;
+        W.lst.host_eig_time += now_s() - t0;
+        return;
+    }
     R.U.assign((size_t)K * std::max(ncols, 1), 0.0);
     if (ncols > 0) R.split_ref().M.vectors(cols.data(), ncols, R.U.data());
     W.lst.host_eig_time += now_s() - t0;
@@ -1201,7 +1255,7 @@
     W.converged_eigs = R.converged;
     W.converged = (R.converged != 0);
     if (R.merge_active) lz_merge_vectors(W, R, howmany);
-    rotate(W, K, R.U, K, howmany, W.Z.p, -1, 0, nullptr, 0);
+    rotate(W, K, R.U, K, howmany, W.Z.p, -1, 0, R.hand_off ? W.vals.data() : nullptr, R.hand_off ? howmany : 0, R.hand_off);
 }
 
 inline void Solver::lanczos_eager(EigWork& W, const double* xp, int nev) {
@@ -1374,8 +1428,10 @@
     return true;
 }
 
-inline void Solver::lanczos(EigWork& W, const double* xp, int nev, bool positive_part) {
+inline void Solver::lanczos(EigWork& W, const double* xp, int nev, bool positive_part, bool hand_off) {
     W.ritz_ok = false;
+    W.u_staged = nullptr; W.lam_on_device = false;
+    harvest_step_events(W);
     if (opt.krylovkit_eager && opt.eigsolver != 1 && !positive_part) { lanczos_eager(W, xp, nev); return; }
     LzRun& R = W.lzrun;
     if (!lz_init(W, R, nev, positive_part)) return;
@@ -1402,6 +1458,8 @@
     const int merge_from = opt.host_eig_merge == 0 ? (1 << 30) : (opt.host_eig_merge == 1 ? 24 : 64);
     const bool blk1 = !wide && block1_plan(W, krylovdim, !R.arpack && krylovdim >= merge_from);
     const bool use_split = !wide && !blk1 && !R.arpack && krylovdim >= merge_from;
+    const bool direct = hand_off && !wide && !blk1 && !comm && opt.host_wait_spin != 0;
+    R.hand_off = direct;
     struct PoolGuard { SpinPool* p; ~PoolGuard() { if (p) p->disarm(); } } pool_guard{nullptr};
     W.split.M.par = nullptr;
     if (use_split && merge_helpers() > 0 && StreamRef::tl == nullptr) {
@@ -1425,8 +1483,10 @@
         DeferGuard(EigWork& w, bool on) : W(w) { W.b1_defer = on; }
         ~DeferGuard() { W.b1_defer = false; }
     };
+    if (debug && dbg_lz_out > 0.0) dbg_lz[7] += now_s() - dbg_lz_out;
     while (true) {
         const int kfirst = R.kfirst;
+        const double tdbge = debug ? now_s() : 0.0;
         const int k1 = (kfirst == 0) ? (18 * krylovdim) / 25 : kfirst + 1;
         const bool split_cycle = use_split && k1 >= 1 && k1 <= krylovdim - 2;
         if (wide) {
@@ -1444,7 +1504,7 @@
                     PX_HIP(hipEventRecord(W.ev_early, W.side));
                 }
             }
-            lz_launch_finish(W, krylovdim - 1, step_tol, krylovdim - 1 > kfirst);
+            lz_launch_finish(W, krylovdim - 1, step_tol, krylovdim - 1 > kfirst, direct);
         }
         const bool speculate = !blk1 && (W.prev_numiter > 1 || R.numiter > 1);
         if (speculate) {
@@ -1452,18 +1512,25 @@
             count_matvecs(W, -1);
         }
         if (wide) PX_HIP(hipMemcpyAsync(W.recw_pinned.p, W.recw.p, EigWork::RECW_DOUBLES * sizeof(double), hipMemcpyDeviceToHost, stream));
-        else PX_HIP(hipMemcpyAsync(W.rec_host, W.rec.p, EigWork::REC_DOUBLES * sizeof(double), hipMemcpyDeviceToHost, stream));
+        else if (!direct) PX_HIP(hipMemcpyAsync(W.rec_host, W.rec.p, EigWork::REC_DOUBLES * sizeof(double), hipMemcpyDeviceToHost, stream));
+        if (debug) dbg_lz[6] += now_s() - tdbge;
         if (!(split_cycle && lz_split_first(W, R, k1))) lz_prepare_arrow(R);
         const double tdbg0 = debug ? now_s() : 0.0;
-        wait_stream();
+        if (debug) dbg_lz[2] += tdbg0 - tdbge;
+        if (direct) wait_cycle_record(W);
+        else wait_stream();
         if (debug) { dbg_lz[0] += now_s() - tdbg0; dbg_lz[5] += 1.0; }
         if (W.cye_pending) {
             W.cye_pending = false;
             float ms = 0.f;
             if (hipEventElapsedTime(&ms, W.cye[0], W.cye[1]) == hipSuccess) W.lst.cycle_ms += ms;
         }
-        W.ev.harvest(W.lst.symv_profiled_ms, W.lst.symv_profiled);
-        W.evo.harvest(W.lst.orth_profiled_ms, W.lst.orth_profiled);
+        if (direct) {
+            W.harvest_pending = true;
+        } else {
+            W.ev.harvest(W.lst.symv_profiled_ms, W.lst.symv_profiled);
+            W.evo.harvest(W.lst.orth_profiled_ms, W.lst.orth_profiled);
+        }
         const double tdbg1 = debug ? now_s() : 0.0;
         bool go_on;
         {
@@ -1475,7 +1542,7 @@
     }
     const double tdbg2 = debug ? now_s() : 0.0;
     lz_finish_run(W, R);
-    if (debug) dbg_lz[3] += now_s() - tdbg2;
+    if (debug) { dbg_lz_out = now_s(); dbg_lz[3] += dbg_lz_out - tdbg2; }
 }
 
 inline void Solver::lzw_step(EigWork& W, const double* xp, int k, int kfirst, double step_tol, bool& presymv) {
```

Result: no change. 524.7 (-0.7%).
